# sibozhang/Text2Video

Hardware: AMD Instinct MI355X
Metric: frames/sec 512x512 pose->RGB (vid2vid generator) (higher is better)
Workload: dtype f32; 1 GPU; configs[1]: fadg0 openpose_only 512x512, 282-frame synthetic pose seq per GPU, generator-only inference, ngf128 n_down3 n_blocks9, flow branch + flow-warp compositor ON; frames_per_gpu=282, parallelism=sequence-chunk dp1, collectives=none (single process), world_size=1

## Files before the change

include/t2v.h:

```cpp
#ifndef T2V_H_
#define T2V_H_

#include <stddef.h>
#include <stdint.h>

#ifdef __cplusplus
extern "C" {
#endif

#define T2V_ABI_VERSION 18

typedef enum {
    T2V_OK = 0,
    T2V_ERR_INVALID = -1,
    T2V_ERR_HIP = -2,
    T2V_ERR_WORKSPACE = -3,
    T2V_ERR_HANDOVER = -4
} t2v_status;

enum { T2V_PAD_ZERO = 0, T2V_PAD_REFLECT = 1 };
enum { T2V_ACT_NONE = 0, T2V_ACT_TANH = 1, T2V_ACT_FLOW_W = 2 ,
       T2V_ACT_LRELU = 3  };

enum { T2V_ALGO_DIRECT = 0, T2V_ALGO_WINOGRAD = 1, T2V_ALGO_WINOGRAD_F4 = 2, T2V_ALGO_POLYPHASE = 3 };

typedef struct t2v_ctx t2v_ctx;

int t2v_abi_version(void);
const char* t2v_last_error(void);
int t2v_create(t2v_ctx** out, int device);
int t2v_destroy(t2v_ctx* ctx);
void t2v_reload_env(void);
int t2v_check_async_errors(void);
int t2v_fixed_grid_enabled(void);
int t2v_set_overlap_hint(int on);
void t2v_debug_async_error(int raise);

typedef struct {
    int H, W;
    int Cin, Cout;
    int kH, kW;
    int stride;
    int pad;
    int pad_mode;
    int transposed;
    int act;
    float act_scale;
    int output_padding;
    int algo;
} t2v_conv_desc;

int t2v_conv_out_dims(const t2v_conv_desc* d, int* Hout, int* Wout);
size_t t2v_conv_packed_weight_floats(const t2v_conv_desc* d, int x_cs);
int t2v_conv_pack_weight(t2v_ctx* ctx, void* stream, const t2v_conv_desc* d, int x_cs,
                         const float* w_torch_dev, float* packed_dev);
int t2v_conv_pack_weight_adjoint(t2v_ctx* ctx, void* stream, const t2v_conv_desc* d, int x_cs,
                                 const float* w_forward_torch_dev, float* packed_dev);
size_t t2v_conv_stats_floats(const t2v_conv_desc* d);
int t2v_conv2d_forward(t2v_ctx* ctx, void* stream, const t2v_conv_desc* d, const float* x, int x_cs,
                       const float* w_packed, const float* bias, float* y, int y_cs,
                       float* stats_partial);
int t2v_conv2d_forward_batch(t2v_ctx* ctx, void* stream, const t2v_conv_desc* d, int batch, const float* x, int x_cs,
                             const float* w_packed, const float* bias, float* y, int y_cs, float* stats_partial);

int t2v_conv_winograd_supported(const t2v_conv_desc* d, int x_cs);
int t2v_conv_polyphase_supported(const t2v_conv_desc* d, int x_cs);
int t2v_conv_best_algo(const t2v_conv_desc* d, int x_cs, int cap);
size_t t2v_conv_winograd_workspace_floats(const t2v_conv_desc* d, int x_cs);
size_t t2v_conv_winograd_batch_workspace_floats(const t2v_conv_desc* d, int x_cs, int nimg);
int t2v_conv_winograd_tile_rows(const t2v_conv_desc* d);
enum { T2V_GEMM_TILE_PER_BLOCK_64x64 = 0, T2V_GEMM_TILE_PER_BLOCK_128x128 = 1, T2V_GEMM_FIXED_GRID_128x128 = 2,
       T2V_GEMM_FIXED_GRID_192x64 = 3, T2V_GEMM_FIXED_GRID_160x128 = 4, T2V_GEMM_FIXED_GRID_RAGGED = 5,
       T2V_GEMM_FIXED_GRID_256x128 = 6 ,
       T2V_GEMM_FIXED_GRID_RAGGED_TALL = 7  };
int t2v_conv_winograd_gemm_form(const t2v_conv_desc* d, int nimg);
int t2v_conv2d_forward_winograd(t2v_ctx* ctx, void* stream, const t2v_conv_desc* d, const float* x, int x_cs,
                                const float* w_packed, const float* bias, float* y, int y_cs, float* stats_partial,
                                float* workspace);
int t2v_conv2d_forward_winograd_stages(t2v_ctx* ctx, void* stream, const t2v_conv_desc* d, const float* x, int x_cs,
                                       const float* w_packed, const float* bias, float* y, int y_cs,
                                       float* stats_partial, float* workspace, int stages);
int t2v_conv2d_forward_winograd_batch_stages(t2v_ctx* ctx, void* stream, const t2v_conv_desc* d, int nimg, const float* x,
                                             int x_cs, long img_stride, const float* w_packed, const float* bias, float* y,
                                             int y_cs, float* stats_partial, float* workspace, int stages,
                                             const float* mean_rstd, const float* gamma, const float* beta, int relu,
                                             const float* res, float* xout);

int t2v_instance_norm_finalize(t2v_ctx* ctx, void* stream, const t2v_conv_desc* producer,
                               const float* stats_partial, float eps, float* mean_rstd);
int t2v_batch_norm_finalize(t2v_ctx* ctx, void* stream, const t2v_conv_desc* producer, int batch,
                            const float* stats_partial, float eps, float* mean_rstd);
int t2v_batch_norm_update_running(t2v_ctx* ctx, void* stream, const float* mean_rstd, float* running_mean,
                                  float* running_var, long n, int C, float momentum, float eps);
int t2v_batch_norm_finalize_running(t2v_ctx* ctx, void* stream, const t2v_conv_desc* producer, int batch,
                                    const float* stats_partial, float eps, float* mean_rstd, float* running_mean,
                                    float* running_var, float momentum, int times);
int t2v_instance_norm_apply(t2v_ctx* ctx, void* stream, const float* x, const float* mean_rstd,
                            const float* gamma, const float* beta, const float* res1,
                            const float* res2, float* y, long npix, int C, int relu);

int t2v_flow_warp_composite(t2v_ctx* ctx, void* stream, const float* raw, const float* fw,
                            const float* prev, int prev_cs, int prev_c0, float* out, float* warp_out,
                            int H, int W);
int t2v_flow_warp_composite_backward(t2v_ctx* ctx, void* stream, const float* d_out, const float* d_warp,
                                     const float* raw, const float* fw, const float* prev, int prev_cs,
                                     int prev_c0, float* d_raw, float* d_fw, float* d_prev, int H, int W);

int t2v_avgpool3x3s2(t2v_ctx* ctx, void* stream, const float* x, float* y, int H, int W, int C);

size_t t2v_conv_backward_weight_workspace_floats(const t2v_conv_desc* d, int x_cs, int batch);
int t2v_conv2d_backward_weight(t2v_ctx* ctx, void* stream, const t2v_conv_desc* d, int batch, const float* x,
                               int x_cs, const float* dy, int dy_cs, float* dw_packed, int accumulate,
                               float* workspace );
int t2v_conv_backward_weight_strided_supported(const t2v_conv_desc* d, int x_cs, int dy_cs);
int t2v_conv2d_backward_weight_strided(t2v_ctx* ctx, void* stream, const t2v_conv_desc* d, int batch, const float* x,
                                       int x_cs, long x_img_stride, const float* dy, int dy_cs, long dy_img_stride,
                                       float* dw_packed, int accumulate, float* workspace);
int t2v_conv_backward_weight_winograd_supported(const t2v_conv_desc* d, int x_cs, int dy_cs);
size_t t2v_conv_backward_weight_winograd_workspace_floats(const t2v_conv_desc* d, int x_cs, int batch);
int t2v_conv2d_backward_weight_winograd(t2v_ctx* ctx, void* stream, const t2v_conv_desc* d, int batch, const float* x,
                                        int x_cs, const float* dy, int dy_cs, float* dw_torch, int accumulate,
                                        float* workspace);
int t2v_conv2d_backward_weight_winograd_stages(t2v_ctx* ctx, void* stream, const t2v_conv_desc* d, int batch, int b0,
                                               int nb, const float* x, int x_cs, const float* dy, int dy_cs,
                                               float* dw_torch, int accumulate, float* workspace, int stages);
int t2v_conv2d_backward_weight_winograd_dy_norm(t2v_ctx* ctx, void* stream, const t2v_conv_desc* d, int batch, int slot,
                                                int x_cs, const float* conv_out, const float* dy, const float* mean_rstd,
                                                const float* gamma, const float* beta, int relu, const float* sums,
                                                float* workspace);
int t2v_conv2d_forward_winograd_keep_v(t2v_ctx* ctx, void* stream, const t2v_conv_desc* d, const float* x, int x_cs,
                                       const float* w_packed, const float* bias, float* y, int y_cs, float* stats_partial,
                                       float* workspace, float* wgrad_workspace, int batch, int slot);

int t2v_conv_backward_data_winograd_supported(const t2v_conv_desc* d, int x_cs, int dy_cs);
size_t t2v_conv_backward_data_winograd_weight_floats(const t2v_conv_desc* d, int x_cs);
size_t t2v_conv_backward_data_winograd_scratch_floats(const t2v_conv_desc* d, int x_cs);
int t2v_conv_pack_weight_transposed(t2v_ctx* ctx, void* stream, const t2v_conv_desc* d, int x_cs, const float* w_forward_dev,
                                    float* packed_dev);
int t2v_conv2d_backward_data_winograd(t2v_ctx* ctx, void* stream, const t2v_conv_desc* d, int batch, int slot,
                                      const float* wgrad_workspace, int x_cs, const float* ut_packed, float* scratch, float* dx);
int t2v_conv_backward_data_winograd_takes_forward_weights(const t2v_conv_desc* d, int x_cs, int dy_cs);
int t2v_conv2d_backward_data_winograd_fw(t2v_ctx* ctx, void* stream, const t2v_conv_desc* d, int batch, int slot,
                                         const float* wgrad_workspace, int x_cs, const float* u_forward_packed, float* scratch,
                                         float* dx);

int t2v_conv_unpack_weight(t2v_ctx* ctx, void* stream, const t2v_conv_desc* d, int x_cs, const float* packed_dev,
                           float* w_torch_dev);
int t2v_conv_unpack_weight_into(t2v_ctx* ctx, void* stream, const t2v_conv_desc* d, int x_cs, const float* packed_dev,
                                float* w_torch_dev, int accumulate);
int t2v_accumulate(t2v_ctx* ctx, void* stream, float* dst, const float* src, long n, int overwrite);
int t2v_scale(t2v_ctx* ctx, void* stream, float* x, long n, float s);
int t2v_zero(t2v_ctx* ctx, void* stream, void* ptr, size_t bytes);
int t2v_unzip2(t2v_ctx* ctx, void* stream, const float* src, float* dst0, float* dst1, int C, int overwrite);
int t2v_channel_sum(t2v_ctx* ctx, void* stream, const float* x, long npix, int C, int cs,
                    float* scratch , float* out);
int t2v_reflect_pad_backward(t2v_ctx* ctx, void* stream, const float* dxp, float* dx, int H, int W, int C, int pad);
int t2v_instance_norm_backward(t2v_ctx* ctx, void* stream, const float* x, const float* dy, const float* mean_rstd,
                               const float* gamma, const float* beta, int relu, long npix, int C, float* scratch,
                               float* dx, float* dbeta_dgamma);
int t2v_instance_norm_backward_affine(t2v_ctx* ctx, void* stream, const float* x, const float* dy, const float* mean_rstd,
                                      const float* gamma, const float* beta, int relu, long npix, int C, float* scratch,
                                      float* dx, float* dbeta_dgamma, float* d_beta, float* d_gamma, int overwrite);
int t2v_act_backward(t2v_ctx* ctx, void* stream, const float* dy, const float* y, int act, float slope, long n,
                     float* dpre);
int t2v_avgpool3x3s2_backward(t2v_ctx* ctx, void* stream, const float* dy, float* dx, int H, int W, int C);
int t2v_maxpool2x2(t2v_ctx* ctx, void* stream, const float* x, float* y, int H, int W, int C);
int t2v_maxpool2x2_backward(t2v_ctx* ctx, void* stream, const float* x, const float* dy, float* dx, int H, int W, int C);
int t2v_sum_sq_diff_const_backward(t2v_ctx* ctx, void* stream, const float* x, float c, float scale, long n, float* dx);
int t2v_sum_abs_diff_backward(t2v_ctx* ctx, void* stream, const float* a, const float* b, float scale, long n, float* da);

int t2v_sum_sq_diff_const(t2v_ctx* ctx, void* stream, const float* x, float c, long n, float* scratch, float* out);
int t2v_sum_abs_diff(t2v_ctx* ctx, void* stream, const float* a, const float* b, long n, float* scratch, float* out);
int t2v_sum_abs_diff_masked(t2v_ctx* ctx, void* stream, const float* a, const float* b, const float* mask, long npix,
                            int c0, int C, int cs, float* scratch, float* out);
int t2v_sum_abs_diff_masked_backward(t2v_ctx* ctx, void* stream, const float* a, const float* b, const float* mask,
                                     float scale, long npix, int c0, int C, int cs, float* da);
int t2v_loss_terms(t2v_ctx* ctx, void* stream, const int64_t* term_ptrs, const int32_t* term_ints, const float* term_floats,
                   const int32_t* chunk_term, const int64_t* chunk_off, const int32_t* term_chunk0, int nterms, int nchunks,
                   int chunk, float* partials, float* out);
int t2v_adam_step(t2v_ctx* ctx, void* stream, float* param, const float* grad, float* exp_avg, float* exp_avg_sq,
                  long n, double lr, double beta1, double beta2, double eps, int step);

int t2v_adam_step_multi(t2v_ctx* ctx, void* stream, const int64_t* ptrs, const int64_t* nelem, const float* step_size,
                        const int32_t* chunk_tensor, const int64_t* chunk_off, int nchunks, int chunk, double beta1,
                        double beta2, double eps);

int t2v_nchw_to_nhwc(t2v_ctx* ctx, void* stream, const float* src, float* dst, int C, int H, int W, int dst_cs);
int t2v_nhwc_to_nchw(t2v_ctx* ctx, void* stream, const float* src, float* dst, int C, int H, int W, int src_cs);
int t2v_pose_u8_to_f32(t2v_ctx* ctx, void* stream, const uint8_t* src_hwc3, float* dst, long npix, int dst_cs, int c0);
int t2v_tensor2im_u8(t2v_ctx* ctx, void* stream, const float* x, uint8_t* y, long n);
int t2v_copy_channels(t2v_ctx* ctx, void* stream, const float* src, int src_cs, int src_c0, float* dst,
                      int dst_cs, int dst_c0, int nc, long npix);

typedef struct {
    int H, W;
    int input_nc;
    int prev_nc;
    int output_nc;
    int ngf;
    int n_downsample;
    int n_blocks;
    int no_flow;
    int norm_affine;
    int is_local;
    float flow_multiplier;
    float eps;
    int conv_algo;
} t2v_gen_desc;

typedef struct {
    const float* w;
    const float* bias;
    const float* gamma;
    const float* beta;
} t2v_layer;

// ... 44 lines not shown
```

text2video_amd/_lib.py:

```python
import ctypes
import os
from ctypes import POINTER, Structure, c_char_p, c_double, c_float, c_int, c_long, c_size_t, c_void_p

_HERE = os.path.dirname(os.path.abspath(__file__))
LIB_PATH = os.environ.get("T2V_LIBRARY") or os.path.join(_HERE, "lib", "libt2v_hip.so")

T2V_OK = 0
PAD_ZERO, PAD_REFLECT = 0, 1
ACT_NONE, ACT_TANH, ACT_FLOW_W, ACT_LRELU = 0, 1, 2, 3
ABI_VERSION = 18
MAX_BATCH = 8
ALGO_DIRECT, ALGO_WINOGRAD, ALGO_WINOGRAD_F4, ALGO_POLYPHASE = 0, 1, 2, 3


class ConvDesc(Structure):
    _fields_ = [("H", c_int), ("W", c_int), ("Cin", c_int), ("Cout", c_int), ("kH", c_int), ("kW", c_int),
                ("stride", c_int), ("pad", c_int), ("pad_mode", c_int), ("transposed", c_int), ("act", c_int),
                ("act_scale", c_float), ("output_padding", c_int), ("algo", c_int)]


class GenDesc(Structure):
    _fields_ = [("H", c_int), ("W", c_int), ("input_nc", c_int), ("prev_nc", c_int), ("output_nc", c_int),
                ("ngf", c_int), ("n_downsample", c_int), ("n_blocks", c_int), ("no_flow", c_int),
                ("norm_affine", c_int), ("is_local", c_int), ("flow_multiplier", c_float), ("eps", c_float),
                ("conv_algo", c_int)]


class Layer(Structure):
    _fields_ = [("w", c_void_p), ("bias", c_void_p), ("gamma", c_void_p), ("beta", c_void_p)]


class GenIO(Structure):
    _fields_ = [("pose", c_void_p), ("prev", c_void_p), ("coarse_img_feat", c_void_p),
                ("coarse_flow_feat", c_void_p), ("use_raw_only", c_int), ("out", c_void_p), ("raw", c_void_p),
                ("flow_w", c_void_p), ("img_feat", c_void_p), ("flow_feat", c_void_p)]


SIGNATURES = {
    "t2v_abi_version": (c_int, []),
    "t2v_last_error": (c_char_p, []),
    "t2v_create": (c_int, [POINTER(c_void_p), c_int]),
    "t2v_destroy": (c_int, [c_void_p]),
    "t2v_reload_env": (None, []),
    "t2v_set_overlap_hint": (c_int, [c_int]),
    "t2v_check_async_errors": (c_int, []),
    "t2v_fixed_grid_enabled": (c_int, []),
    "t2v_debug_async_error": (None, [c_int]),
    "t2v_conv_out_dims": (c_int, [POINTER(ConvDesc), POINTER(c_int), POINTER(c_int)]),
    "t2v_conv_packed_weight_floats": (c_size_t, [POINTER(ConvDesc), c_int]),
    "t2v_conv_pack_weight": (c_int, [c_void_p, c_void_p, POINTER(ConvDesc), c_int, c_void_p, c_void_p]),
    "t2v_conv_pack_weight_adjoint": (c_int, [c_void_p, c_void_p, POINTER(ConvDesc), c_int, c_void_p, c_void_p]),
    "t2v_conv_stats_floats": (c_size_t, [POINTER(ConvDesc)]),
    "t2v_conv2d_forward": (c_int, [c_void_p, c_void_p, POINTER(ConvDesc), c_void_p, c_int, c_void_p, c_void_p,
                                   c_void_p, c_int, c_void_p]),
    "t2v_conv2d_forward_batch": (c_int, [c_void_p, c_void_p, POINTER(ConvDesc), c_int, c_void_p, c_int, c_void_p, c_void_p,
                                         c_void_p, c_int, c_void_p]),
    "t2v_conv_winograd_supported": (c_int, [POINTER(ConvDesc), c_int]),
    "t2v_conv_polyphase_supported": (c_int, [POINTER(ConvDesc), c_int]),
    "t2v_conv_best_algo": (c_int, [POINTER(ConvDesc), c_int, c_int]),
    "t2v_conv_winograd_workspace_floats": (c_size_t, [POINTER(ConvDesc), c_int]),
    "t2v_conv_winograd_batch_workspace_floats": (c_size_t, [POINTER(ConvDesc), c_int, c_int]),
    "t2v_conv_winograd_tile_rows": (c_int, [POINTER(ConvDesc)]),
    "t2v_conv_winograd_gemm_form": (c_int, [POINTER(ConvDesc), c_int]),
    "t2v_conv2d_forward_winograd": (c_int, [c_void_p, c_void_p, POINTER(ConvDesc), c_void_p, c_int, c_void_p, c_void_p,
                                            c_void_p, c_int, c_void_p, c_void_p]),
    "t2v_conv2d_forward_winograd_stages": (c_int, [c_void_p, c_void_p, POINTER(ConvDesc), c_void_p, c_int, c_void_p,
                                                   c_void_p, c_void_p, c_int, c_void_p, c_void_p, c_int]),
    "t2v_conv2d_backward_weight_winograd_dy_norm": (c_int, [c_void_p, c_void_p, POINTER(ConvDesc), c_int, c_int, c_int, c_void_p,
                                                            c_void_p, c_void_p, c_void_p, c_void_p, c_int, c_void_p, c_void_p]),
    "t2v_conv2d_forward_winograd_batch_stages": (c_int, [c_void_p, c_void_p, POINTER(ConvDesc), c_int, c_void_p, c_int, c_long,
                                                         c_void_p, c_void_p, c_void_p, c_int, c_void_p, c_void_p, c_int,
                                                         c_void_p, c_void_p, c_void_p, c_int, c_void_p, c_void_p]),
    "t2v_conv2d_forward_winograd_keep_v": (c_int, [c_void_p, c_void_p, POINTER(ConvDesc), c_void_p, c_int, c_void_p,
                                                   c_void_p, c_void_p, c_int, c_void_p, c_void_p, c_void_p, c_int, c_int]),
    "t2v_instance_norm_finalize": (c_int, [c_void_p, c_void_p, POINTER(ConvDesc), c_void_p, c_float, c_void_p]),
    "t2v_batch_norm_finalize": (c_int, [c_void_p, c_void_p, POINTER(ConvDesc), c_int, c_void_p, c_float, c_void_p]),
    "t2v_batch_norm_finalize_running": (c_int, [c_void_p, c_void_p, POINTER(ConvDesc), c_int, c_void_p, c_float, c_void_p,
                                                c_void_p, c_void_p, c_float, c_int]),
    "t2v_conv_backward_weight_workspace_floats": (c_size_t, [POINTER(ConvDesc), c_int, c_int]),
    "t2v_conv_backward_weight_winograd_supported": (c_int, [POINTER(ConvDesc), c_int, c_int]),
    "t2v_conv_backward_weight_winograd_workspace_floats": (c_size_t, [POINTER(ConvDesc), c_int, c_int]),
    "t2v_conv2d_backward_weight_winograd": (c_int, [c_void_p, c_void_p, POINTER(ConvDesc), c_int, c_void_p, c_int,
                                                    c_void_p, c_int, c_void_p, c_int, c_void_p]),
    "t2v_conv2d_backward_weight_winograd_stages": (c_int, [c_void_p, c_void_p, POINTER(ConvDesc), c_int, c_int, c_int,
                                                           c_void_p, c_int, c_void_p, c_int, c_void_p, c_int, c_void_p,
                                                           c_int]),
    "t2v_conv2d_backward_weight": (c_int, [c_void_p, c_void_p, POINTER(ConvDesc), c_int, c_void_p, c_int, c_void_p,
                                           c_int, c_void_p, c_int, c_void_p]),
    "t2v_conv_backward_weight_strided_supported": (c_int, [POINTER(ConvDesc), c_int, c_int]),
    "t2v_conv2d_backward_weight_strided": (c_int, [c_void_p, c_void_p, POINTER(ConvDesc), c_int, c_void_p, c_int, c_long, c_void_p,
                                                   c_int, c_long, c_void_p, c_int, c_void_p]),
    "t2v_conv_unpack_weight": (c_int, [c_void_p, c_void_p, POINTER(ConvDesc), c_int, c_void_p, c_void_p]),
    "t2v_conv_backward_data_winograd_supported": (c_int, [POINTER(ConvDesc), c_int, c_int]),
    "t2v_conv_backward_data_winograd_weight_floats": (c_size_t, [POINTER(ConvDesc), c_int]),
    "t2v_conv_backward_data_winograd_scratch_floats": (c_size_t, [POINTER(ConvDesc), c_int]),
    "t2v_conv_pack_weight_transposed": (c_int, [c_void_p, c_void_p, POINTER(ConvDesc), c_int, c_void_p, c_void_p]),
    "t2v_conv2d_backward_data_winograd": (c_int, [c_void_p, c_void_p, POINTER(ConvDesc), c_int, c_int, c_void_p, c_int, c_void_p,
                                                  c_void_p, c_void_p]),
    "t2v_conv_backward_data_winograd_takes_forward_weights": (c_int, [POINTER(ConvDesc), c_int, c_int]),
    "t2v_conv2d_backward_data_winograd_fw": (c_int, [c_void_p, c_void_p, POINTER(ConvDesc), c_int, c_int, c_void_p, c_int, c_void_p,
                                                     c_void_p, c_void_p]),
    "t2v_conv_unpack_weight_into": (c_int, [c_void_p, c_void_p, POINTER(ConvDesc), c_int, c_void_p, c_void_p, c_int]),
    "t2v_accumulate": (c_int, [c_void_p, c_void_p, c_void_p, c_void_p, c_long, c_int]),
    "t2v_scale": (c_int, [c_void_p, c_void_p, c_void_p, c_long, c_float]),
    "t2v_zero": (c_int, [c_void_p, c_void_p, c_void_p, c_size_t]),
    "t2v_unzip2": (c_int, [c_void_p, c_void_p, c_void_p, c_void_p, c_void_p, c_int, c_int]),
    "t2v_channel_sum": (c_int, [c_void_p, c_void_p, c_void_p, c_long, c_int, c_int, c_void_p, c_void_p]),
    "t2v_reflect_pad_backward": (c_int, [c_void_p, c_void_p, c_void_p, c_void_p, c_int, c_int, c_int, c_int]),
    "t2v_instance_norm_backward": (c_int, [c_void_p, c_void_p, c_void_p, c_void_p, c_void_p, c_void_p, c_void_p, c_int,
                                           c_long, c_int, c_void_p, c_void_p, c_void_p]),
    "t2v_instance_norm_backward_affine": (c_int, [c_void_p, c_void_p, c_void_p, c_void_p, c_void_p, c_void_p, c_void_p, c_int,
                                           c_long, c_int, c_void_p, c_void_p, c_void_p, c_void_p, c_void_p, c_int]),
    "t2v_act_backward": (c_int, [c_void_p, c_void_p, c_void_p, c_void_p, c_int, c_float, c_long, c_void_p]),
    "t2v_avgpool3x3s2_backward": (c_int, [c_void_p, c_void_p, c_void_p, c_void_p, c_int, c_int, c_int]),
    "t2v_sum_sq_diff_const_backward": (c_int, [c_void_p, c_void_p, c_void_p, c_float, c_float, c_long, c_void_p]),
    "t2v_sum_abs_diff_backward": (c_int, [c_void_p, c_void_p, c_void_p, c_void_p, c_float, c_long, c_void_p]),
    "t2v_sum_sq_diff_const": (c_int, [c_void_p, c_void_p, c_void_p, c_float, c_long, c_void_p, c_void_p]),
    "t2v_sum_abs_diff": (c_int, [c_void_p, c_void_p, c_void_p, c_void_p, c_long, c_void_p, c_void_p]),
    "t2v_sum_abs_diff_masked": (c_int, [c_void_p, c_void_p, c_void_p, c_void_p, c_void_p, c_long, c_int, c_int, c_int,
                                        c_void_p, c_void_p]),
    "t2v_sum_abs_diff_masked_backward": (c_int, [c_void_p, c_void_p, c_void_p, c_void_p, c_void_p, c_float, c_long, c_int,
                                                 c_int, c_int, c_void_p]),
    "t2v_loss_terms": (c_int, [c_void_p, c_void_p, c_void_p, c_void_p, c_void_p, c_void_p, c_void_p, c_void_p, c_int, c_int,
                               c_int, c_void_p, c_void_p]),
    "t2v_adam_step": (c_int, [c_void_p, c_void_p, c_void_p, c_void_p, c_void_p, c_void_p, c_long, c_double, c_double,
                              c_double, c_double, c_int]),
    "t2v_adam_step_multi": (c_int, [c_void_p, c_void_p, c_void_p, c_void_p, c_void_p, c_void_p, c_void_p, c_int, c_int,
                                    c_double, c_double, c_double]),
    "t2v_batch_norm_update_running": (c_int, [c_void_p, c_void_p, c_void_p, c_void_p, c_void_p, c_long, c_int, c_float,
                                              c_float]),
    "t2v_instance_norm_apply": (c_int, [c_void_p, c_void_p, c_void_p, c_void_p, c_void_p, c_void_p, c_void_p,
                                        c_void_p, c_void_p, c_long, c_int, c_int]),
    "t2v_flow_warp_composite": (c_int, [c_void_p, c_void_p, c_void_p, c_void_p, c_void_p, c_int, c_int, c_void_p,
                                        c_void_p, c_int, c_int]),
    "t2v_flow_warp_composite_backward": (c_int, [c_void_p, c_void_p, c_void_p, c_void_p, c_void_p, c_void_p, c_void_p,
                                                 c_int, c_int, c_void_p, c_void_p, c_void_p, c_int, c_int]),
    "t2v_avgpool3x3s2": (c_int, [c_void_p, c_void_p, c_void_p, c_void_p, c_int, c_int, c_int]),
    "t2v_maxpool2x2": (c_int, [c_void_p, c_void_p, c_void_p, c_void_p, c_int, c_int, c_int]),
    "t2v_maxpool2x2_backward": (c_int, [c_void_p, c_void_p, c_void_p, c_void_p, c_void_p, c_int, c_int, c_int]),
    "t2v_nchw_to_nhwc": (c_int, [c_void_p, c_void_p, c_void_p, c_void_p, c_int, c_int, c_int, c_int]),
    "t2v_nhwc_to_nchw": (c_int, [c_void_p, c_void_p, c_void_p, c_void_p, c_int, c_int, c_int, c_int]),
    "t2v_pose_u8_to_f32": (c_int, [c_void_p, c_void_p, c_void_p, c_void_p, c_long, c_int, c_int]),
    "t2v_tensor2im_u8": (c_int, [c_void_p, c_void_p, c_void_p, c_void_p, c_long]),
    "t2v_copy_channels": (c_int, [c_void_p, c_void_p, c_void_p, c_int, c_int, c_void_p, c_int, c_int, c_int,
                                  c_long]),
    "t2v_generator_num_layers": (c_int, [POINTER(GenDesc)]),
    "t2v_generator_layer_desc": (c_int, [POINTER(GenDesc), c_int, POINTER(ConvDesc), POINTER(c_int)]),
    "t2v_generator_workspace_bytes": (c_size_t, [POINTER(GenDesc)]),
    "t2v_generator_forward": (c_int, [c_void_p, c_void_p, POINTER(GenDesc), POINTER(Layer), c_int, POINTER(GenIO),
                                      c_void_p, c_size_t]),
    "t2v_generator_workspace_bytes_batch": (c_size_t, [POINTER(GenDesc), c_int]),
    "t2v_generator_forward_batch": (c_int, [c_void_p, c_void_p, POINTER(GenDesc), POINTER(Layer), c_int, POINTER(GenIO),
                                            c_int, c_void_p, c_size_t]),
    "t2v_device_malloc": (c_int, [c_void_p, c_size_t, POINTER(c_void_p)]),
    "t2v_device_free": (c_int, [c_void_p, c_void_p]),
    "t2v_host_malloc": (c_int, [c_void_p, c_size_t, POINTER(c_void_p)]),
    "t2v_host_free": (c_int, [c_void_p, c_void_p]),
    "t2v_memcpy": (c_int, [c_void_p, c_void_p, c_void_p, c_void_p, c_size_t, c_int]),
    "t2v_stream_create": (c_int, [c_void_p, POINTER(c_void_p)]),
    "t2v_stream_destroy": (c_int, [c_void_p, c_void_p]),
    "t2v_stream_synchronize": (c_int, [c_void_p, c_void_p]),
    "t2v_event_create": (c_int, [c_void_p, POINTER(c_void_p)]),
    "t2v_event_record": (c_int, [c_void_p, c_void_p, c_void_p]),
    "t2v_event_synchronize": (c_int, [c_void_p, c_void_p]),
    "t2v_event_destroy": (c_int, [c_void_p, c_void_p]),
    "t2v_device_synchronize": (c_int, [c_void_p]),
}
COPY_H2D, COPY_D2H, COPY_D2D = 1, 2, 3

_lib = None
_load_lock = __import__("threading").RLock()


def load():
    if _lib is not None:
        return _lib
    with _load_lock:
        return _load_locked()


def _load_locked():
    global _lib
    if _lib is not None:
        return _lib
    if not os.path.exists(LIB_PATH):
        raise RuntimeError(
            "libt2v_hip.so not found at %s: the HIP extension is required (no CPU fallback). "
            "Build it with `python __graft_entry__.py` or `make -C text2video_amd/csrc`." % LIB_PATH)
    from ._xp import LEAN
    if not LEAN:
        import torch
        hip_rt = os.path.join(os.path.dirname(torch.__file__), "lib", "libamdhip64.so")
        if os.path.exists(hip_rt):
            ctypes.CDLL(hip_rt, mode=ctypes.RTLD_GLOBAL)
    elif os.environ.get("T2V_HIP_RUNTIME", "torch") != "system":
        import importlib.util
        spec = importlib.util.find_spec("torch")
        hip_rt = os.path.join(os.path.dirname(spec.origin), "lib", "libamdhip64.so") if spec and spec.origin else ""
        if os.path.exists(hip_rt):
            ctypes.CDLL(hip_rt, mode=ctypes.RTLD_GLOBAL)
    lib = ctypes.CDLL(LIB_PATH)
    for name, (res, args) in SIGNATURES.items():
        fn = getattr(lib, name)
        fn.restype = res
        fn.argtypes = args
    if lib.t2v_abi_version() != ABI_VERSION:
        raise RuntimeError("libt2v_hip.so ABI %d != binding ABI %d" % (lib.t2v_abi_version(), ABI_VERSION))
    _lib = lib
    return lib
# ... 31 lines not shown
```

text2video_amd/csrc/capi.hip:

```cpp
#include <stdarg.h>
#include <stdio.h>
#include <stdlib.h>
#include <string.h>

#include <algorithm>
#include <atomic>
#include <mutex>
#include <utility>
#include <vector>

#include "conv_plan.h"

namespace t2v {

static thread_local char g_err[512] = "";
void set_error(const char* fmt, ...) {
    va_list ap;
    va_start(ap, fmt);
    vsnprintf(g_err, sizeof(g_err), fmt, ap);
    va_end(ap);
}

static inline int round_up(int v, int m) { return (v + m - 1) / m * m; }

// ... 170 lines not shown
        k.ostride = 2;
        k.pad_mode = T2V_PAD_ZERO;
        k.nphases = 4;
        k.KW = 3;
        k.pad = 0;
        int tap0 = 0;
        long woff = 0;
        for (int p = 0; p < 4; ++p) {
            int nt, kh[4], kw[4], dy[4], dx[4], a, b;
            convT_phase_taps_host(p, d->kH, d->pad, &nt, kh, kw, dy, dx, &a, &b);
            ConvPhase& ph = k.ph[p];
            ph.ntaps = nt;
            ph.tap0 = tap0;
            ph.Kp = round_up(nt * x_cs, kBK);
            ph.nk = ph.Kp / kBK;
            ph.w_off = woff;
            ph.oy0 = a;
            ph.ox0 = b;
            for (int t = 0; t < nt; ++t) {
                k.tdy[tap0 + t] = dy[t];
                k.tdx[tap0 + t] = dx[t];
            }
            tap0 += nt;
            woff += (long)pl.Cout_p * ph.Kp;
        }
        pl.wfloats = (size_t)woff;
    }
    k.group_mtiles = 1 << 30;
    k.group_w_stride = 0;
    k.Wm = Wm;
    k.M = Hm * Wm;
    k.Wout = pl.Wout;
    k.Hout = pl.Hout;
    k.mtiles = (k.M + pl.BM - 1) / pl.BM;
    if (pl.tile == kTileL) {
        const long nb = (long)k.mtiles * k.ntiles * k.nphases;
        const double fill = (double)nb / (double)(((nb + 255) / 256) * 256);
        const long nbq = 4 * nb;
        const double fillq = (double)nbq / (double)(((nbq + 255) / 256) * 256);
        const int force = options().conv_tile;
        if (force == 2 || (force != 1 && ((fill < 0.8 && nb < 1024) || (k.nphases > 1 && nb <= 512) || (fillq - fill >= 0.1 && nb < 2048)))) {
            pl.tile = kTileQ;
            conv_tile_dims(pl.tile, &pl.BM, &pl.BN);
            k.ntiles = (d->Cout + pl.BN - 1) / pl.BN;
            k.mtiles = (k.M + pl.BM - 1) / pl.BM;
        }
    }
    if (need_stats && !d->transposed && d->kH == 7 && d->kW == 7 && d->stride == 1 && d->pad == 3 &&
        d->pad_mode == T2V_PAD_REFLECT && d->act == T2V_ACT_NONE && conv_stem7x7_supported(d->H, d->W, x_cs, d->Cout)) {
        pl.tile = kTileStem;
        pl.BM = 256;
        pl.BN = d->Cout;
        k.mtiles = ((d->H + 15) / 16) * ((d->W + 15) / 16);
        k.ntiles = 1;
    }
    pl.nparts = k.nphases * k.mtiles;
    T2V_REQUIRE((long)k.mtiles * k.ntiles * k.nphases < (1L << 31), "conv: grid too large");
    T2V_REQUIRE((long)d->H * d->W * x_cs * 4 < 0x7fff0000L, "conv: input tensor too large for 32-bit buffer offsets");
    for (int ph = 0; ph < k.nphases; ++ph)
        T2V_REQUIRE((long)pl.Cout_p * k.ph[ph].Kp * 4 < 0x7fff0000L, "conv: weight too large for 32-bit buffer offsets");
    return T2V_OK;
}

bool winograd_supported(const t2v_conv_desc* d, int x_cs, int algo) {
    if (!d || !is_winograd(algo)) return false;
    if (d->transposed || d->kH != 3 || d->kW != 3 || d->stride != 1) return false;
    if (d->pad_mode == T2V_PAD_REFLECT ? d->pad != 1 : (d->pad < 0 || d->pad > 2)) return false;
    if (wino_out_h(d) < 1 || wino_out_w(d) < 1) return false;
    if (d->Cin % 32 != 0 || x_cs != d->Cin || d->Cout % 4 != 0 || d->H < 2 || d->W < 2) return false;
    return d->act == T2V_ACT_NONE || (algo == T2V_ALGO_WINOGRAD_F4 && d->act == T2V_ACT_LRELU);
}

int best_conv_algo(const t2v_conv_desc* d, int x_cs, int cap) {
    const bool f4 = cap == 0 && winograd_supported(d, x_cs, T2V_ALGO_WINOGRAD_F4);
    const bool f2 = (cap == 0 || cap == 2) && winograd_supported(d, x_cs, T2V_ALGO_WINOGRAD);
    const long direct_rows = 9L * wino_out_h(d) * wino_out_w(d);
    if (f4 && (!f2 || wino_gemm_rows(d, T2V_ALGO_WINOGRAD_F4) <= wino_gemm_rows(d, T2V_ALGO_WINOGRAD)) &&
        wino_gemm_rows(d, T2V_ALGO_WINOGRAD_F4) < direct_rows)
        return T2V_ALGO_WINOGRAD_F4;
    if (f2 && wino_gemm_rows(d, T2V_ALGO_WINOGRAD) < direct_rows) return T2V_ALGO_WINOGRAD;
    return T2V_ALGO_DIRECT;
}

struct PositionGemm {
    int groups = 0;
    int rows = 0;
    int T = 0, K = 0, N = 0;
    int a_pitch = 0;
    bool has_scratch = true;
    bool b_kn = false;
};

static int build_position_gemm_plan(const PositionGemm& g, ConvPlan* pl) {
    t2v_conv_desc d;
    memset(&d, 0, sizeof(d));
    d.H = g.groups; d.W = g.T; d.Cin = g.K; d.Cout = g.N; d.kH = d.kW = 1; d.stride = 1; d.pad = 0;
    d.pad_mode = T2V_PAD_ZERO; d.act = T2V_ACT_NONE; d.act_scale = 1.f;
    T2V_TRY(build_conv_plan(&d, g.K,  true, pl));
    if (g.T % pl->BM != 0 && pl->tile == kTileL) {
        pl->tile = kTileQ;
        conv_tile_dims(pl->tile, &pl->BM, &pl->BN);
        pl->kp.ntiles = (d.Cout + pl->BN - 1) / pl->BN;
        pl->kp.mtiles = (pl->kp.M + pl->BM - 1) / pl->BM;
        pl->nparts = pl->kp.nphases * pl->kp.mtiles;
    }
    T2V_REQUIRE(g.T % pl->BM == 0, "position gemm: tile rows %d do not divide %d", pl->BM, g.T);
    pl->kp.group_mtiles = g.T / pl->BM;
    pl->kp.group_w_stride = (long)pl->Cout_p * g.K;
    if (g.a_pitch) {
        T2V_REQUIRE((long)g.groups * g.a_pitch * g.K * 4 < 0x7fff0000L, "position gemm: A too large for 32-bit buffer offsets");
        pl->kp.Win = g.a_pitch;
    }
    return T2V_OK;
}

static int position_gemm_form(const PositionGemm& g, ConvPlan* plan = nullptr) {
    if (g.b_kn) return T2V_GEMM_FIXED_GRID_128x128;
    if (g.has_scratch) {
        if (wino_gemm_skt_ok(g.groups, g.rows, g.T, g.K, g.N, g.N)) return T2V_GEMM_FIXED_GRID_RAGGED_TALL;
        if (wino_gemm_skr_ok(g.groups, g.rows, g.T, g.K, g.N, g.N)) return T2V_GEMM_FIXED_GRID_RAGGED;
        if (wino_gemm_sk_ok(g.groups, g.T, g.K, g.N, g.N, g.rows))
            switch (wino_gemm_sk_tall_rows(g.groups, g.rows, g.T, g.N)) {
                case 160: return T2V_GEMM_FIXED_GRID_160x128;
                case 256: return T2V_GEMM_FIXED_GRID_256x128;
                default: return g.T % 128 == 0 ? T2V_GEMM_FIXED_GRID_128x128 : T2V_GEMM_FIXED_GRID_192x64;
            }
    }
    ConvPlan local;
    ConvPlan* pl = plan ? plan : &local;
    if (build_position_gemm_plan(g, pl) != T2V_OK) return -1;
    return pl->tile == kTileL ? T2V_GEMM_TILE_PER_BLOCK_128x128 : T2V_GEMM_TILE_PER_BLOCK_64x64;
}

static int run_position_gemm(t2v_ctx* ctx, hipStream_t s, const PositionGemm& g, const float* a, const float* b, float* c,
                             float* scratch) {
    T2V_REQUIRE(a && b && c && (scratch || !g.has_scratch), "position gemm: null pointer");
    ConvPlan pl;
    const int form = position_gemm_form(g, &pl);
    if (form < 0) return T2V_ERR_INVALID;
    if (form == T2V_GEMM_TILE_PER_BLOCK_128x128 || form == T2V_GEMM_TILE_PER_BLOCK_64x64)
        return run_conv(ctx, s, pl, a, b, nullptr, c, g.N, nullptr);
    SkGemm k;
    k.a = a; k.b = b; k.c = c; k.scratch = scratch;
    k.err = async_error_word();
    k.rows = g.rows;
    k.a_group_stride = (long)(g.a_pitch ? g.a_pitch : g.T) * g.K;
    k.groups = g.groups; k.T = g.T; k.K = g.K; k.N = g.N; k.c_cs = g.N;
    k.b_kn = g.b_kn;
    if (form == T2V_GEMM_FIXED_GRID_RAGGED_TALL) return launch_wino_gemm_skt(s, k, g.rows);
    if (form == T2V_GEMM_FIXED_GRID_RAGGED) return launch_wino_gemm_skr(s, k, g.rows);
    return launch_wino_gemm_sk(s, k);
}

int run_conv_batch(t2v_ctx* ctx, hipStream_t s, const ConvPlan& pl, int batch, const float* x, long x_stride, const float* w,
                   const float* bias, float* y, int y_cs, long y_stride, float* stats, long stats_stride) {
    T2V_REQUIRE(ctx && x && w && y, "conv: null pointer");
    T2V_REQUIRE(batch >= 1 && batch <= 65535, "conv: batch %d", batch);
    T2V_REQUIRE(y_cs >= pl.kp.Cout && y_cs <= pl.Cout_p, "conv: output channel storage %d out of range [%d,%d]", y_cs,
                pl.kp.Cout, pl.Cout_p);
    T2V_REQUIRE((long)pl.Hout * pl.Wout * y_cs * 4 < 0x7fff0000L, "conv: output tensor too large for 32-bit buffer offsets");
    {
        const ConvKParams& q = pl.kp;
        if (!stats && q.nphases == 1 && q.ph[0].ntaps == 49 && q.KW == 7 && q.pad == 3 && q.stride == 1 &&
            q.pad_mode == T2V_PAD_REFLECT && q.Cout <= 3 && q.Cin_s % 16 == 0 && q.Hin >= 4 && q.Win >= 4) {
            for (int b = 0; b < batch; ++b) {
                HeadParams h;
                h.x = x + b * x_stride; h.w = w; h.bias = bias; h.y = y + b * y_stride;
                h.H = q.Hin; h.W = q.Win; h.Cin_s = q.Cin_s; h.Kp = q.ph[0].Kp; h.Cout = q.Cout; h.Cout_s = y_cs;
                h.act = q.act; h.act_scale = q.act_scale;
                T2V_TRY(launch_conv_head7x7(s, h));
            }
            return T2V_OK;
        }
    }
    {
        const ConvKParams& q = pl.kp;
        if (!stats && q.nphases == 1 && q.Cout == 1 && q.pad_mode == T2V_PAD_ZERO && q.ostride == 1 &&
            q.ph[0].ntaps == q.KW * q.KW && conv_cout1_supported(q.KW, q.Cin_s) &&
            (q.act == T2V_ACT_NONE || q.act == T2V_ACT_LRELU)) {
            for (int b = 0; b < batch; ++b) {
                Cout1Params c;
                c.x = x + b * x_stride; c.w = w; c.bias = bias; c.y = y + b * y_stride;
                c.H = q.Hin; c.W = q.Win; c.Cin_s = q.Cin_s; c.ksize = q.KW; c.stride = q.stride; c.pad = q.pad;
                c.Hout = pl.Hout; c.Wout = pl.Wout; c.Cout_s = y_cs; c.act = q.act; c.act_scale = q.act_scale;
                T2V_TRY(launch_conv_cout1(s, c));
            }
            return T2V_OK;
        }
    }
    if (pl.tile == kTileStem && stats) {
        for (int b = 0; b < batch; ++b) {
            StemParams sp;
            sp.x = x + b * x_stride; sp.w = w; sp.bias = bias; sp.y = y + b * y_stride; sp.stats = stats + b * stats_stride;
            sp.H = pl.kp.Hin; sp.W = pl.kp.Win; sp.Cin_s = pl.kp.Cin_s; sp.Kp = pl.kp.ph[0].Kp; sp.Cout = pl.kp.Cout; sp.Cout_s = y_cs;
            sp.Cin = pl.Cin;
            T2V_TRY(launch_conv_stem7x7(s, sp));
        }
        return T2V_OK;
    }
    T2V_REQUIRE(pl.tile != kTileStem, "conv: the stem plan needs a statistics buffer");
    ConvKParams k = pl.kp;
    k.x = x;
    k.w = w;
    k.bias = bias;
    k.y = y;
    k.Cout_s = y_cs;
    k.stats = stats;
    k.batch = batch;
    k.x_img_stride = batch > 1 ? x_stride : 0;
    k.y_img_stride = batch > 1 ? y_stride : 0;
    k.stats_img_stride = (batch > 1 && stats) ? stats_stride : 0;
    return launch_conv_igemm(s, k, pl.tile);
}

int run_conv(t2v_ctx* ctx, hipStream_t s, const ConvPlan& pl, const float* x, const float* w, const float* bias,
             float* y, int y_cs, float* stats) {
    return run_conv_batch(ctx, s, pl, 1, x, 0, w, bias, y, y_cs, 0, stats, 0);
}

int winograd_forward(t2v_ctx* ctx, hipStream_t s, const t2v_conv_desc* d, const float* x, const float* w_packed,
                     const float* bias, float* y, float* stats_partial, float* workspace, int stages,
                     const WinoBatch* batch) {
    const WinoBatch one;
    const WinoBatch& wb = batch ? *batch : one;
    const int nimg = wb.nimg;
    const bool f4 = d->algo == T2V_ALGO_WINOGRAD_F4;
    if (f4) T2V_TRY(check_async_errors());
    T2V_REQUIRE(nimg >= 1 && (f4 || nimg == 1), "winograd: batches are F(4x4,3x3) only");
    const size_t T = (size_t)wino_rows_batch(d, d->algo, nimg);
    const bool keep = wb.keep_v != nullptr;
    T2V_REQUIRE(!keep || (f4 && nimg == 1 && wb.keep_slot >= 0 && wb.keep_slot < wb.keep_total),
                "winograd: V is kept for the weight gradient of single F(4x4,3x3) images only");
    float* V = keep ? wb.keep_v + (size_t)wb.keep_slot * T * d->Cin : workspace;
    float* Mm = workspace + wino_pos(d->algo) * T * d->Cin;
    if (stages & 1) {
        const int reflect = d->pad_mode == T2V_PAD_REFLECT;
        if (keep) T2V_TRY(launch_winograd4_input(s, x, wb.keep_v, d->H, d->W, d->Cin, d->pad, reflect, wb.keep_total, wb.keep_slot));
        else
        T2V_TRY(f4 ? launch_winograd4_input(s, x, V, d->H, d->W, d->Cin, d->pad, reflect, nimg, 0, nimg, wb.img_stride_x)
                   : launch_winograd_input(s, x, V, d->H, d->W, d->Cin, d->pad, reflect));
    }
    if (stages & 2) {
        PositionGemm g;
        g.has_scratch = f4;
        g.groups = wino_pos(d->algo);
        g.rows = nimg * wino_tiles_real(d, d->algo);
        g.T = (int)T; g.K = d->Cin; g.N = d->Cout;
        if (keep) g.a_pitch = wb.keep_total * (int)T;
        T2V_TRY(run_position_gemm(ctx, s, g, V, w_packed, Mm, f4 ? workspace + winograd_vm_floats(d, nimg) : nullptr));
    }
    if (stages & 4) {
        T2V_REQUIRE(d->act == T2V_ACT_NONE || !stats_partial, "winograd: an activation and norm statistics do not combine");
        if (f4)
            T2V_TRY(launch_winograd4_output(s, Mm, bias, y, stats_partial, wino_out_h(d), wino_out_w(d), d->Cout,
                                            d->act == T2V_ACT_LRELU, d->act_scale, nimg));
        else
            T2V_TRY(launch_winograd_output(s, Mm, bias, y, stats_partial, wino_out_h(d), wino_out_w(d), d->Cout));
    }
    return T2V_OK;
}

bool polyphase_supported(const t2v_conv_desc* d, int x_cs) {
    if (!d || d->kH != 3 || d->kW != 3 || d->stride != 2 || d->pad != 1 || d->pad_mode != T2V_PAD_ZERO) return false;
    if (d->act != T2V_ACT_NONE || d->Cin % 32 != 0 || x_cs != d->Cin || d->Cout % 128 != 0) return false;
    if (d->transposed) return d->output_padding == 1 && d->H >= 2 && d->W >= 2;
    return d->H >= 4 && d->W >= 4 && d->H % 2 == 0 && d->W % 2 == 0;
}

bool polyphase_pays(const t2v_conv_desc* d, int x_cs) {
    return polyphase_supported(d, x_cs) && d->Cin >= 256 && d->Cout >= 256 && poly_tiles_real(d) >= 128;
}

int polyphase_forward(t2v_ctx* ctx, hipStream_t s, const t2v_conv_desc* d, const float* x, const float* w_packed,
                      const float* bias, float* y, float* stats_partial, float* workspace, int stages,
                      const LazyNorm* lazy) {
    T2V_TRY(check_async_errors());
    const int up = d->transposed ? 1 : 0;
    const int T = poly_tiles_padded(d), rows = poly_tiles_real(d);
    float* V = workspace;
    float* Mm = workspace + (size_t)81 * T * d->Cin;
    if (stages & 1) T2V_TRY(launch_polyphase_input(s, x, V, d->H, d->W, d->Cin, up, T, lazy));
    if (stages & 2) {
        PositionGemm g;
        g.groups = 81; g.rows = rows; g.T = T; g.K = d->Cin; g.N = d->Cout;
        T2V_TRY(run_position_gemm(ctx, s, g, V, w_packed, Mm, workspace + (size_t)81 * T * ((size_t)d->Cin + d->Cout)));
    }
    if (stages & 4)
        T2V_TRY(launch_polyphase_output(s, Mm, bias, y, stats_partial, poly_out_h(d), poly_out_w(d), d->Cout, up, T));
    return T2V_OK;
}

}

using namespace t2v;

extern "C" {

int t2v_abi_version(void) { return T2V_ABI_VERSION; }
const char* t2v_last_error(void) { return g_err; }

int t2v_create(t2v_ctx** out, int device) {
    T2V_REQUIRE(out, "t2v_create: null out");
    int n = 0;
    T2V_HIP_CHECK(hipGetDeviceCount(&n));
    T2V_REQUIRE(device >= 0 && device < n, "t2v_create: device %d out of range (%d visible)", device, n);
    T2V_HIP_CHECK(hipSetDevice(device));
    hipDeviceProp_t prop;
    T2V_HIP_CHECK(hipGetDeviceProperties(&prop, device));
    T2V_REQUIRE(strncmp(prop.gcnArchName, "gfx950", 6) == 0,
                "libt2v_hip is built for gfx950 (MI355X) only; device %d is %s", device, prop.gcnArchName);
    t2v_ctx* c = new t2v_ctx();
    c->device = device;
    c->side = nullptr;
    c->ev_fork = c->ev_join = nullptr;
    if (hipStreamCreateWithFlags(&c->side, hipStreamNonBlocking) != hipSuccess ||
        hipEventCreateWithFlags(&c->ev_fork, hipEventDisableTiming) != hipSuccess ||
        hipEventCreateWithFlags(&c->ev_join, hipEventDisableTiming) != hipSuccess) {
        t2v_destroy(c);
        set_error("t2v_create: cannot create the side stream / events");
        return T2V_ERR_HIP;
    }
    (void)options();
    {
        static std::once_flag once;
        int st = T2V_OK;
        std::call_once(once, [&]() {
            void* w = nullptr;
            if (hipHostMalloc(&w, 64, hipHostMallocMapped | hipHostMallocPortable) != hipSuccess) {
                fixed_grid_disable("no pinned error word");
                return;
            }
            memset(w, 0, 64);
            g_err_word = static_cast<unsigned*>(w);
            st = fixed_grid_selftest();
        });
        if (st != T2V_OK) {
            t2v_destroy(c);
            return st;
        }
    }
    *out = c;
    return T2V_OK;
}

void t2v_reload_env(void) { options_reload(); }
int t2v_set_overlap_hint(int on) { return set_overlap_hint(on); }
int t2v_check_async_errors(void) { return check_async_errors(); }
int t2v_fixed_grid_enabled(void) { return fixed_grid_enabled() ? 1 : 0; }
void t2v_debug_async_error(int raise) {
    if (!g_err_word) return;
    if (raise) {
        *reinterpret_cast<volatile unsigned*>(g_err_word) = 1u;
    } else {
        *reinterpret_cast<volatile unsigned*>(g_err_word) = 0u;
        g_fixed_grid_on.store(1);
    }
}

int t2v_destroy(t2v_ctx* ctx) {
    if (!ctx) return T2V_OK;
    if (ctx->ev_fork) (void)hipEventDestroy(ctx->ev_fork);
    if (ctx->ev_join) (void)hipEventDestroy(ctx->ev_join);
    if (ctx->side) (void)hipStreamDestroy(ctx->side);
    delete ctx;
    return T2V_OK;
}

int t2v_conv_out_dims(const t2v_conv_desc* d, int* Hout, int* Wout) {
    ConvPlan pl;
    T2V_TRY(build_conv_plan(d, round_up(d ? d->Cin : 0, 4), false, &pl));
    if (Hout) *Hout = pl.Hout;
    if (Wout) *Wout = pl.Wout;
    return T2V_OK;
}

size_t t2v_conv_packed_weight_floats(const t2v_conv_desc* d, int x_cs) {
    ConvPlan pl;
    if (build_conv_plan(d, x_cs, false, &pl) != T2V_OK) return 0;
    if (is_winograd(d->algo)) return winograd_supported(d, x_cs, d->algo) ? (size_t)wino_pos(d->algo) * pl.Cout_p * x_cs : 0;
    if (d->algo == T2V_ALGO_POLYPHASE) return polyphase_supported(d, x_cs) ? (size_t)81 * pl.Cout_p * x_cs : 0;
    return pl.wfloats;
}
int t2v_conv_polyphase_supported(const t2v_conv_desc* d, int x_cs) {
    return (polyphase_supported(d, x_cs) ? 1 : 0) | (polyphase_pays(d, x_cs) ? 2 : 0);
}

int t2v_conv_winograd_supported(const t2v_conv_desc* d, int x_cs) {
    return (winograd_supported(d, x_cs, T2V_ALGO_WINOGRAD) ? 1 : 0) | (winograd_supported(d, x_cs, T2V_ALGO_WINOGRAD_F4) ? 2 : 0);
}

int t2v_conv_best_algo(const t2v_conv_desc* d, int x_cs, int cap) { return d ? best_conv_algo(d, x_cs, cap) : T2V_ALGO_DIRECT; }

size_t t2v_conv_winograd_workspace_floats(const t2v_conv_desc* d, int x_cs) {
    if (d && d->algo == T2V_ALGO_POLYPHASE) return polyphase_supported(d, x_cs) ? polyphase_workspace_floats(d) : 0;
    if (!d || !winograd_supported(d, x_cs, d->algo)) return 0;
    return winograd_workspace_floats(d);
}

size_t t2v_conv_winograd_batch_workspace_floats(const t2v_conv_desc* d, int x_cs, int nimg) {
    if (!d || nimg < 1) return 0;
    if (d->algo == T2V_ALGO_POLYPHASE) return nimg == 1 && polyphase_supported(d, x_cs) ? polyphase_workspace_floats(d) : 0;
    if (!winograd_supported(d, x_cs, d->algo) || (nimg > 1 && d->algo != T2V_ALGO_WINOGRAD_F4)) return 0;
    return winograd_workspace_floats(d, nimg);
}

int t2v_conv2d_forward_winograd_stages(t2v_ctx* ctx, void* stream, const t2v_conv_desc* d, const float* x, int x_cs,
                                       const float* w_packed, const float* bias, float* y, int y_cs,
                                       float* stats_partial, float* workspace, int stages) {
    T2V_REQUIRE(ctx && d && x && w_packed && y && workspace, "winograd forward: null pointer");
    if (d->algo == T2V_ALGO_POLYPHASE) {
        T2V_REQUIRE(polyphase_supported(d, x_cs), "polyphase forward: shape not supported (t2v_conv_polyphase_supported)");
        T2V_REQUIRE(y_cs == d->Cout, "polyphase forward: output channel storage must equal Cout");
        return polyphase_forward(ctx, (hipStream_t)stream, d, x, w_packed, bias, y, stats_partial, workspace, stages);
    }
    T2V_REQUIRE(winograd_supported(d, x_cs, d->algo),
                "winograd forward: shape/algo not supported (t2v_conv_winograd_supported)");
    T2V_REQUIRE(y_cs == d->Cout, "winograd forward: output channel storage must equal Cout");
    return winograd_forward(ctx, (hipStream_t)stream, d, x, w_packed, bias, y, stats_partial, workspace, stages);
}

int t2v_conv2d_forward_winograd_batch_stages(t2v_ctx* ctx, void* stream, const t2v_conv_desc* d, int nimg, const float* x,
                                             int x_cs, long img_stride, const float* w_packed, const float* bias, float* y,
                                             int y_cs, float* stats_partial, float* workspace, int stages,
                                             const float* mean_rstd, const float* gamma, const float* beta, int relu,
                                             const float* res, float* xout) {
    T2V_REQUIRE(ctx && d && x && w_packed && y && workspace, "winograd batch forward: null pointer");
    T2V_REQUIRE(stages >= 0 && stages <= 7, "winograd batch forward: stages mask %d", stages);
    T2V_REQUIRE(nimg >= 1 && nimg <= 65535, "winograd batch forward: nimg %d", nimg);
    T2V_REQUIRE(nimg == 1 || img_stride >= (long)d->H * d->W * x_cs, "winograd batch forward: image stride %ld below one map",
                img_stride);
    T2V_REQUIRE(mean_rstd || (!gamma && !beta && !res && !xout && relu == 0),
                "winograd batch forward: gamma, beta, relu, res and xout need mean_rstd");
    hipStream_t s = (hipStream_t)stream;
    if (d->algo == T2V_ALGO_POLYPHASE) {
        T2V_REQUIRE(polyphase_supported(d, x_cs), "polyphase forward: shape not supported (t2v_conv_polyphase_supported)");
        T2V_REQUIRE(y_cs == d->Cout, "polyphase forward: output channel storage must equal Cout");
        T2V_REQUIRE(nimg == 1 && !res && !xout, "polyphase batch forward: one image, no residual");
        const LazyNorm ln{mean_rstd, gamma, beta, relu};
        return polyphase_forward(ctx, s, d, x, w_packed, bias, y, stats_partial, workspace, stages, mean_rstd ? &ln : nullptr);
    }
    T2V_REQUIRE(winograd_supported(d, x_cs, d->algo), "winograd forward: shape/algo not supported (t2v_conv_winograd_supported)");
    T2V_REQUIRE(y_cs == d->Cout, "winograd forward: output channel storage must equal Cout");
    T2V_REQUIRE(d->algo == T2V_ALGO_WINOGRAD_F4 || (nimg == 1 && !mean_rstd),
                "winograd batch forward: batches and the lazy norm are F(4x4,3x3) only");
    if (mean_rstd && (stages & 1)) {
        T2V_REQUIRE(relu == 0 || relu == 1, "winograd batch forward: relu %d", relu);
        const LazyNorm ln{mean_rstd, gamma, beta, relu, res, xout};
        T2V_TRY(launch_winograd4_input(s, x, workspace, d->H, d->W, d->Cin, d->pad, d->pad_mode == T2V_PAD_REFLECT, nimg, 0, nimg,
                                       img_stride, &ln));
        stages &= ~1;
    }
    WinoBatch wb;
    wb.nimg = nimg;
    wb.img_stride_x = img_stride;
    return winograd_forward(ctx, s, d, x, w_packed, bias, y, stats_partial, workspace, stages, &wb);
}

static bool wgrad_winograd_ok(const t2v_conv_desc* d, int x_cs, int dy_cs);
int t2v_conv2d_forward_winograd_keep_v(t2v_ctx* ctx, void* stream, const t2v_conv_desc* d, const float* x, int x_cs,
                                       const float* w_packed, const float* bias, float* y, int y_cs, float* stats_partial,
                                       float* workspace, float* wgrad_workspace, int batch, int slot) {
    T2V_REQUIRE(ctx && d && x && w_packed && y && workspace && wgrad_workspace, "winograd forward (V kept): null pointer");
    T2V_REQUIRE(d->algo == T2V_ALGO_WINOGRAD_F4 && winograd_supported(d, x_cs, d->algo) && x_cs == d->Cin &&
                    wgrad_winograd_ok(d, x_cs, d->Cout),
                "winograd forward (V kept): F(4x4,3x3) layers with a Winograd-domain weight gradient only "
                "(t2v_conv_backward_weight_winograd_supported)");
    T2V_REQUIRE(y_cs == d->Cout, "winograd forward: output channel storage must equal Cout");
    T2V_REQUIRE(batch >= 1 && slot >= 0 && slot < batch, "winograd forward (V kept): slot %d of %d", slot, batch);
    T2V_REQUIRE((long)36 * batch * wino_tiles_padded(d, d->algo) * x_cs * 4 < 0x7fff0000L,
                "winograd forward (V kept): batch-wide V too large for 32-bit buffer offsets");
    WinoBatch wb;
    wb.keep_v = wgrad_workspace;
    wb.keep_total = batch;
    wb.keep_slot = slot;
    return winograd_forward(ctx, (hipStream_t)stream, d, x, w_packed, bias, y, stats_partial, workspace, 7, &wb);
}

int t2v_conv2d_forward_winograd(t2v_ctx* ctx, void* stream, const t2v_conv_desc* d, const float* x, int x_cs,
                                const float* w_packed, const float* bias, float* y, int y_cs, float* stats_partial,
                                float* workspace) {
    return t2v_conv2d_forward_winograd_stages(ctx, stream, d, x, x_cs, w_packed, bias, y, y_cs, stats_partial, workspace, 7);
}

static int pack_weight(t2v_ctx* ctx, void* stream, const t2v_conv_desc* d, int x_cs, const float* w_torch_dev,
                       float* packed_dev, int adjoint) {
    T2V_REQUIRE(ctx && w_torch_dev && packed_dev, "pack_weight: null pointer");
    ConvPlan pl;
    T2V_TRY(build_conv_plan(d, x_cs, false, &pl));
    hipStream_t s = (hipStream_t)stream;
    if (d->algo == T2V_ALGO_POLYPHASE) {
        T2V_REQUIRE(polyphase_supported(d, x_cs) && !adjoint, "pack_weight: polyphase form not supported for this shape");
        return launch_polyphase_weight(s, w_torch_dev, packed_dev, d->Cout, d->Cin, pl.Cout_p, x_cs, d->transposed ? 1 : 0);
    }
    if (is_winograd(d->algo)) {
        T2V_REQUIRE(winograd_supported(d, x_cs, d->algo), "pack_weight: Winograd not supported for this shape");
        return (d->algo == T2V_ALGO_WINOGRAD_F4 ? launch_winograd4_weight : launch_winograd_weight)(
            s, w_torch_dev, packed_dev, d->Cout, d->Cin, pl.Cout_p, x_cs, adjoint);
    }
    if (!d->transposed)
        return launch_pack_conv_weight(s, w_torch_dev, packed_dev, d->Cout, d->Cin, d->kH, d->kW, x_cs, pl.kp.ph[0].Kp,
                                       pl.Cout_p, adjoint);
    T2V_REQUIRE(!adjoint, "pack_weight_adjoint: stride-1 convolutions only (a transposed conv's data gradient reuses its weight)");
    return launch_pack_convT_weight(s, w_torch_dev, packed_dev, d->Cin, d->Cout, x_cs, pl.Cout_p, d->kH, d->pad);
}
int t2v_conv_pack_weight(t2v_ctx* ctx, void* stream, const t2v_conv_desc* d, int x_cs, const float* w_torch_dev,
                         float* packed_dev) {
    return pack_weight(ctx, stream, d, x_cs, w_torch_dev, packed_dev, 0);
}
int t2v_conv_pack_weight_adjoint(t2v_ctx* ctx, void* stream, const t2v_conv_desc* d, int x_cs, const float* w_forward_dev,
                                 float* packed_dev) {
    T2V_REQUIRE(d && !d->transposed && d->stride == 1, "pack_weight_adjoint: `d` must be a stride-1 (data-gradient) conv");
    return pack_weight(ctx, stream, d, x_cs, w_forward_dev, packed_dev, 1);
}

size_t t2v_conv_stats_floats(const t2v_conv_desc* d) {
    if (d && is_winograd(d->algo))
        return (size_t)(wino_tiles_padded(d, d->algo) * wino_m(d->algo) * wino_m(d->algo) / 128) * d->Cout * 2;
    if (d && d->algo == T2V_ALGO_POLYPHASE) return (size_t)(poly_tiles_padded(d) * poly_m(d) * poly_m(d) / 128) * d->Cout * 2;
    ConvPlan pl;
    if (!d || build_conv_plan(d, round_up(d->Cin, 4), true, &pl) != T2V_OK) return 0;
    return (size_t)pl.nparts * d->Cout * 2;
}

int t2v_conv2d_forward(t2v_ctx* ctx, void* stream, const t2v_conv_desc* d, const float* x, int x_cs,
                       const float* w_packed, const float* bias, float* y, int y_cs, float* stats_partial) {
    T2V_REQUIRE(d && d->algo == T2V_ALGO_DIRECT, "conv2d_forward: use t2v_conv2d_forward_winograd for algo=WINOGRAD");
    ConvPlan pl;
    T2V_TRY(build_conv_plan(d, x_cs, stats_partial != nullptr, &pl));
    return run_conv(ctx, (hipStream_t)stream, pl, x, w_packed, bias, y, y_cs, stats_partial);
}

int t2v_conv2d_forward_batch(t2v_ctx* ctx, void* stream, const t2v_conv_desc* d, int batch, const float* x, int x_cs,
                             const float* w_packed, const float* bias, float* y, int y_cs, float* stats_partial) {
    T2V_REQUIRE(d && d->algo == T2V_ALGO_DIRECT, "conv2d_forward_batch: direct convolutions only");
    T2V_REQUIRE(batch >= 1, "conv2d_forward_batch: batch %d", batch);
    ConvPlan pl;
    T2V_TRY(build_conv_plan(d, x_cs, stats_partial != nullptr, &pl));
    return run_conv_batch(ctx, (hipStream_t)stream, pl, batch, x, (long)d->H * d->W * x_cs, w_packed, bias, y, y_cs,
                          (long)pl.Hout * pl.Wout * y_cs, stats_partial, (long)t2v_conv_stats_floats(d));
}

int t2v_instance_norm_finalize(t2v_ctx* ctx, void* stream, const t2v_conv_desc* producer, const float* stats_partial,
                               float eps, float* mean_rstd) {
    T2V_REQUIRE(ctx && stats_partial && mean_rstd, "inorm_finalize: null pointer");
    if (producer && is_winograd(producer->algo)) {
        return launch_inorm_finalize_winograd((hipStream_t)stream, stats_partial, wino_m(producer->algo),
                                              wino_out_h(producer), wino_out_w(producer), producer->Cout, eps, mean_rstd, 1);
    }
    if (producer && producer->algo == T2V_ALGO_POLYPHASE)
        return launch_inorm_finalize_winograd((hipStream_t)stream, stats_partial, poly_m(producer), poly_out_h(producer),
                                              poly_out_w(producer), producer->Cout, eps, mean_rstd, 1);
    ConvPlan pl;
    T2V_TRY(build_conv_plan(producer, round_up(producer ? producer->Cin : 0, 4), true, &pl));
    if (pl.tile == kTileStem)
        return launch_inorm_finalize_tiles((hipStream_t)stream, stats_partial, 16, producer->H, producer->W, producer->Cout, eps,
                                           mean_rstd, 1);
    return launch_inorm_finalize((hipStream_t)stream, stats_partial, pl.nparts, pl.kp.mtiles, pl.BM, pl.kp.M,
                                 producer->Cout, eps, mean_rstd);
}

static int batch_norm_finalize(hipStream_t s, const t2v_conv_desc* producer, int batch, const float* stats_partial, float eps,
                               float* mean_rstd, const RunningUpdate* ru) {
    if (producer && is_winograd(producer->algo))
        return launch_inorm_finalize_winograd(s, stats_partial, wino_m(producer->algo), wino_out_h(producer),
                                              wino_out_w(producer), producer->Cout, eps, mean_rstd, batch, nullptr, ru);
    if (producer && producer->algo == T2V_ALGO_POLYPHASE)
        return launch_inorm_finalize_winograd(s, stats_partial, poly_m(producer), poly_out_h(producer), poly_out_w(producer),
                                              producer->Cout, eps, mean_rstd, batch, nullptr, ru);
    ConvPlan pl;
    T2V_TRY(build_conv_plan(producer, round_up(producer ? producer->Cin : 0, 4), true, &pl));
    if (pl.tile == kTileStem)
        return launch_inorm_finalize_tiles(s, stats_partial, 16, producer->H, producer->W, producer->Cout, eps, mean_rstd, batch,
                                           nullptr, ru);
    return launch_inorm_finalize(s, stats_partial, batch * pl.nparts, pl.kp.mtiles, pl.BM, pl.kp.M, producer->Cout, eps,
                                 mean_rstd, nullptr, ru);
}
int t2v_batch_norm_finalize(t2v_ctx* ctx, void* stream, const t2v_conv_desc* producer, int batch,
                            const float* stats_partial, float eps, float* mean_rstd) {
    T2V_REQUIRE(ctx && stats_partial && mean_rstd && batch >= 1, "batch_norm_finalize: bad arguments");
    return batch_norm_finalize((hipStream_t)stream, producer, batch, stats_partial, eps, mean_rstd, nullptr);
}
int t2v_batch_norm_finalize_running(t2v_ctx* ctx, void* stream, const t2v_conv_desc* producer, int batch,
                                    const float* stats_partial, float eps, float* mean_rstd, float* running_mean,
                                    float* running_var, float momentum, int times) {
    T2V_REQUIRE(ctx && producer && stats_partial && mean_rstd && running_mean && running_var && batch >= 1 && times >= 1,
                "batch_norm_finalize_running: bad arguments");
    int ho = 0, wo = 0;
    T2V_TRY(t2v_conv_out_dims(producer, &ho, &wo));
    const long n = (long)batch * ho * wo;
    T2V_REQUIRE(n >= 2, "batch_norm_finalize_running: the unbiased variance needs at least two values per channel");
    const RunningUpdate ru{running_mean, running_var, (float)n, momentum, times};
    return batch_norm_finalize((hipStream_t)stream, producer, batch, stats_partial, eps, mean_rstd, &ru);
}

static bool wgrad_fold(const t2v_conv_desc* d, int x_cs) {
    return !d->transposed && x_cs < 64 && d->kH * d->kW > 1;
}

static bool wgrad_fold_n(const t2v_conv_desc* d, int x_cs, int dy_cs) {
    return !d->transposed && d->stride == 1 && dy_cs <= 16 && x_cs >= 64 && d->kH * d->kW > 1 &&
           d->kH * d->kW <= kMaxTaps;
}
static size_t wgrad_padded_floats(const t2v_conv_desc* d, int x_cs, int batch) {
    return (size_t)batch * (d->H + 2 * d->pad) * (d->W + 2 * d->pad) * x_cs;
}

static int wgrad_splits(const t2v_conv_desc* d, int x_cs, int batch, const ConvPlan& pl) {
    int ntaps = 0;
    for (int ph = 0; ph < pl.kp.nphases; ++ph) ntaps += pl.kp.ph[ph].ntaps;
    const long blocks = wgrad_fold(d, x_cs) ? (long)((d->Cout + 127) / 128) * ((ntaps * x_cs + 127) / 128)
                                            : (long)ntaps * ((d->Cout + 127) / 128) * ((x_cs + 127) / 128);
    const long nk = ((long)batch * pl.kp.M + 31) / 32;
    long smax = nk / 8;
    if (smax > 256) smax = 256;
    if (smax < 1) smax = 1;
    long s = 1, best = -1;
    const long slots = 2 * 256;
    for (long c = 1; c <= smax; ++c) {
        const long rounds = (blocks * c + slots - 1) / slots;
        const long cost = rounds * ((nk + c - 1) / c + 3) + (c > 1 ? c * (long)pl.wfloats * 12 / 15000000 : 0);
        if (best < 0 || cost < best) { best = cost; s = c; }
        if (blocks * c >= 4096) break;
    }
    return s < 1 ? 1 : (int)s;
}

static size_t wgrad_ticket_floats(const t2v_conv_desc* d, int x_cs, const ConvPlan& pl) {
    int ntaps = 0;
    for (int ph = 0; ph < pl.kp.nphases; ++ph) ntaps += pl.kp.ph[ph].ntaps;
    const size_t tiles = wgrad_fold(d, x_cs) ? (size_t)((d->Cout + 127) / 128) * ((ntaps * x_cs + 127) / 128)
                                            : (size_t)ntaps * ((d->Cout + 127) / 128) * ((x_cs + 127) / 128);
    return (tiles + 255) / 256 * 256;
}
static int wgrad_combine_max_splits() { return options().wgrad_combine_max; }
static bool wgrad_combine_on() { return options().wgrad_combine != 0; }

size_t t2v_conv_backward_weight_workspace_floats(const t2v_conv_desc* d, int x_cs, int batch) {
    ConvPlan pl;
    if (!d || build_conv_plan(d, x_cs, true, &pl) != T2V_OK) return 0;
    const int dy_cs = round_up(d->Cout, 4);
    if (wgrad_fold_n(d, x_cs, dy_cs)) {
        const long nk = ((long)batch * (d->H + 2 * d->pad) * (d->W + 2 * d->pad) + 31) / 32;
        long s = nk / 16;
        if (s > 256) s = 256;
        if (s < 1) s = 1;
        return wgrad_padded_floats(d, x_cs, batch) + (size_t)s * d->Cout * pl.kp.ph[0].Kp;
    }
    const int s = wgrad_splits(d, x_cs, batch, pl);
    return s > 1 ? (size_t)s * pl.wfloats + wgrad_ticket_floats(d, x_cs, pl) : 0;
}

static int backward_weight_impl(t2v_ctx* ctx, void* stream, const t2v_conv_desc* d, int batch, const float* x,
                                int x_cs, long x_stride, const float* dy, int dy_cs, long dy_stride, float* dw_packed,
                                int accumulate, float* workspace) {
    T2V_REQUIRE(ctx && x && dy && dw_packed && batch >= 1, "backward_weight: bad arguments");
    ConvPlan pl;
    T2V_TRY(build_conv_plan(d, x_cs, true, &pl));
    T2V_REQUIRE(dy_cs >= d->Cout && dy_cs % 4 == 0, "backward_weight: dy channel storage %d", dy_cs);
    const ConvKParams& k = pl.kp;
    WgradParams w;
    memset(&w, 0, sizeof(w));
    w.x = x; w.dy = dy; w.dw = dw_packed;
    w.batch = batch; w.Hin = d->H; w.Win = d->W; w.Cin_s = x_cs;
    w.Wm = k.Wm; w.M = k.M;
    w.Hout = pl.Hout; w.Wout = pl.Wout; w.Cout = d->Cout; w.Cout_s = dy_cs;
    w.stride = k.stride; w.ostride = k.ostride;
    w.reflect = k.pad_mode == T2V_PAD_REFLECT; w.accumulate = accumulate;
    w.ntiles = (d->Cout + 127) / 128; w.ctiles = (x_cs + 127) / 128;
    int nt = 0;
    for (int ph = 0; ph < k.nphases; ++ph)
        for (int t = 0; t < k.ph[ph].ntaps; ++t, ++nt) {
            w.tdy[nt] = k.tdy[k.ph[ph].tap0 + t]; w.tdx[nt] = k.tdx[k.ph[ph].tap0 + t];
            w.toy[nt] = k.ph[ph].oy0; w.tox[nt] = k.ph[ph].ox0;
            w.tap_woff[nt] = k.ph[ph].w_off; w.tap_Kp[nt] = k.ph[ph].Kp; w.tap_kidx[nt] = t;
        }
    w.ntaps = nt;
    w.x_img_stride = (long)d->H * d->W * x_cs;
    w.dy_img_stride = (long)pl.Hout * pl.Wout * dy_cs;
    if (x_stride || dy_stride) {
        T2V_REQUIRE(!(wgrad_fold_n(d, x_cs, dy_cs) && dy_cs == round_up(d->Cout, 4)) && !wgrad_fold(d, x_cs) && conv_wgrad_strided_ok(w),
                    "backward_weight_strided: this shape keeps its images contiguous (t2v_conv_backward_weight_strided_supported)");
        if (x_stride) w.x_img_stride = x_stride;
// ... 529 lines not shown
```

text2video_amd/csrc/conv_head.hip:

```cpp
#include <stdlib.h>

#include "t2v_internal.h"

namespace t2v {

__device__ __forceinline__ void hd_dma16(const float* base, int nbytes, char* lds_dst, int voff, int soff) {
#if defined(__HIP_DEVICE_COMPILE__)
    const __amdgpu_buffer_rsrc_t srd = __builtin_amdgcn_make_buffer_rsrc(const_cast<float*>(base), 0, nbytes, 0x00020000);
    __builtin_amdgcn_raw_ptr_buffer_load_lds(srd, (__attribute__((address_space(3))) void*)lds_dst, 16, voff, soff, 0, 0);
#endif
}

constexpr int kHdTile = 16;
constexpr int kHdHalo = kHdTile + 6;
constexpr int kHsPitch = 23;
constexpr int kHsPlane = 512 * 16;
template <int CIN>
__global__ __launch_bounds__(256) void conv_head7x7_strip_kernel(const HeadParams p) {
    extern __shared__ __attribute__((aligned(16))) char smem[];
    const int tid = threadIdx.x, lane = tid & 63;
    const int wave = __builtin_amdgcn_readfirstlane(tid >> 6);
    const int cin_s = CIN ? CIN : p.Cin_s;
    int tile;
    {
        const int nb = gridDim.x, b = blockIdx.x;
        const int xcd = b & 7, idx = b >> 3;
        const int q = nb >> 3, r = nb & 7;
        tile = (xcd < r ? xcd * (q + 1) : r * (q + 1) + (xcd - r) * q) + idx;
    }
    const int tiles_x = (p.W + kHdTile - 1) / kHdTile;
    const int x0 = (tile % tiles_x) * kHdTile, y0 = (tile / tiles_x) * kHdTile;
    int voff[8];
#pragma unroll
    for (int i = 0; i < 8; ++i) {
        const int hp = i * 64 + lane;
        const int hy = hp / kHsPitch, hx = hp - hy * kHsPitch;
        int gy = y0 - 3 + hy, gx = x0 - 3 + hx;
        gy = gy < 0 ? -gy : gy;
        gx = gx < 0 ? -gx : gx;
        gy = min(gy, 2 * p.H - 2 - gy);
        gx = min(gx, 2 * p.W - 2 - gx);
        gy = max(gy, 0);
        gx = max(gx, 0);
        voff[i] = (hy < kHdHalo && hx < kHdHalo) ? (gy * p.W + gx) * cin_s * 4 : 0x7fff0000;
    }
    const int x_bytes = p.H * p.W * cin_s * 4;
    char* plane = smem + wave * kHsPlane;
    const int lq = (lane & 31) >> 2;
    const int ty = ((lq >> 1) << 2) | (lane & 3), sx = ((lane >> 5) << 1) | ((0x96 >> lq) & 1);
    const char* sb = plane + (ty * kHsPitch + sx * 4) * 16;

    typedef float f32x2 __attribute__((ext_vector_type(2)));
    f32x2 acc[3][4];
#pragma unroll
    for (int o = 0; o < 3; ++o)
#pragma unroll
        for (int q = 0; q < 4; ++q) acc[o][q] = (f32x2){0.f, 0.f};
    const float* __restrict__ w0 = p.w;
    const float* __restrict__ w1 = p.w + p.Kp;
    const float* __restrict__ w2 = p.w + 2 * p.Kp;
    auto stage = [&](int c) {
#pragma unroll
        for (int i = 0; i < 8; ++i) hd_dma16(p.x, x_bytes, plane + i * 1024, voff[i], c * 4);
    };
    for (int c0 = wave * 4; c0 < cin_s; c0 += 16) {
        stage(c0);
        asm volatile("s_waitcnt vmcnt(0)" ::: "memory");
        typedef float f32x4 __attribute__((ext_vector_type(4)));
        typedef const __attribute__((address_space(4))) f32x4* cf4;
        f32x4 wa[3][3], wb[2][3], wc[2][3];
        float4 xv[2][10];
        const float* __restrict__ b0 = w0 + c0;
        const float* __restrict__ b1 = w1 + c0;
        const float* __restrict__ b2 = w2 + c0;
        auto load_w = [&](int kh, int kw, f32x4(&w)[3]) {
            const int kofs = (kh * 7 + kw) * cin_s;
            w[0] = *(cf4)(b0 + kofs);
            w[1] = *(cf4)(b1 + kofs);
            w[2] = *(cf4)(b2 + kofs);
        };
        auto load_x = [&](int kh, float4(&x)[10]) {
#pragma unroll
            for (int j = 0; j < 10; ++j) x[j] = *reinterpret_cast<const float4*>(sb + (kh * kHsPitch + j) * 16);
        };
        auto taps = [&](const float4(&x)[10], int kw, const f32x4(&w)[3]) {
#pragma unroll
            for (int q = 0; q < 4; ++q) {
                const f32x2 xlo = {x[q + kw].x, x[q + kw].y}, xhi = {x[q + kw].z, x[q + kw].w};
#pragma unroll
                for (int o = 0; o < 3; ++o) acc[o][q] = __builtin_elementwise_fma(xlo, (f32x2){w[o].x, w[o].y}, acc[o][q]);
#pragma unroll
                for (int o = 0; o < 3; ++o) acc[o][q] = __builtin_elementwise_fma(xhi, (f32x2){w[o].z, w[o].w}, acc[o][q]);
            }
        };
        if constexpr (CIN == 0) {
#pragma unroll 1
            for (int kh = 0; kh < 7; ++kh) {
                load_x(kh, xv[0]);
#pragma unroll
                for (int kw = 0; kw < 7; ++kw) {
                    load_w(kh, kw, wa[0]);
                    taps(xv[0], kw, wa[0]);
                }
            }
        } else {
        load_x(0, xv[0]);
#pragma unroll
        for (int t = 0; t < 3; ++t) load_w(0, t, wa[t]);
#pragma unroll
        for (int kh = 0; kh < 7; ++kh) {
            __builtin_amdgcn_sched_barrier(0);
#pragma unroll
            for (int t = 0; t < 2; ++t) load_w(kh, 3 + t, wb[t]);
            __builtin_amdgcn_sched_barrier(0);
#pragma unroll
            for (int t = 0; t < 3; ++t) taps(xv[kh & 1], t, wa[t]);
            __builtin_amdgcn_sched_barrier(0);
#pragma unroll
            for (int t = 0; t < 2; ++t) load_w(kh, 5 + t, wc[t]);
            __builtin_amdgcn_sched_barrier(0);
#pragma unroll
            for (int t = 0; t < 2; ++t) taps(xv[kh & 1], 3 + t, wb[t]);
            __builtin_amdgcn_sched_barrier(0);
            if (kh < 6) {
                load_x(kh + 1, xv[(kh + 1) & 1]);
#pragma unroll
                for (int t = 0; t < 3; ++t) load_w(kh + 1, t, wa[t]);
            }
            __builtin_amdgcn_sched_barrier(0);
#pragma unroll
            for (int t = 0; t < 2; ++t) taps(xv[kh & 1], 5 + t, wc[t]);
        }
        }
        __builtin_amdgcn_sched_barrier(0);
        asm volatile("s_waitcnt lgkmcnt(0)" ::: "memory");
    }
    float* red = reinterpret_cast<float*>(plane);
#pragma unroll
    for (int o = 0; o < 3; ++o)
#pragma unroll
        for (int q = 0; q < 4; ++q) red[(o * 4 + q) * 64 + lane] = acc[o][q].x + acc[o][q].y;
    __syncthreads();
    const int prow = tid >> 4, pcol = tid & 15;
    const int pq = pcol & 3, psx = pcol >> 2;
    const int src = ((psx >> 1) << 5) | ((((psx & 1) ? 0x7421 : 0x6530) >> (4 * (prow >> 2))) & 7) << 2 | (prow & 3);
    float v[3];
#pragma unroll
    for (int o = 0; o < 3; ++o) {
        float sum = 0.f;
#pragma unroll
        for (int w = 0; w < 4; ++w) sum += reinterpret_cast<const float*>(smem + w * kHsPlane)[(o * 4 + pq) * 64 + src];
        v[o] = sum;
    }
    const int oy = y0 + prow, ox = x0 + pcol;
    if (oy < p.H && ox < p.W) {
        float v0 = v[0] + (p.bias ? p.bias[0] : 0.f);
        float v1 = v[1] + (p.bias && p.Cout > 1 ? p.bias[1] : 0.f);
        float v2 = v[2] + (p.bias && p.Cout > 2 ? p.bias[2] : 0.f);
        if (p.act == T2V_ACT_TANH) {
            v0 = tanhf(v0); v1 = tanhf(v1); v2 = tanhf(v2);
        } else if (p.act == T2V_ACT_FLOW_W) {
            v0 *= p.act_scale; v1 *= p.act_scale; v2 = 1.f / (1.f + expf(-v2));
        } else if (p.act == T2V_ACT_LRELU) {
            v0 = v0 > 0.f ? v0 : v0 * p.act_scale; v1 = v1 > 0.f ? v1 : v1 * p.act_scale; v2 = v2 > 0.f ? v2 : v2 * p.act_scale;
        }
        if (p.Cout < 2) v1 = 0.f;
        if (p.Cout < 3) v2 = 0.f;
        float* dst = p.y + (size_t)(oy * p.W + ox) * p.Cout_s;
        if (p.Cout_s == 4) {
            *reinterpret_cast<float4*>(dst) = make_float4(v0, v1, v2, 0.f);
        } else {
            dst[0] = v0;
            if (p.Cout_s > 1) dst[1] = v1;
            if (p.Cout_s > 2) dst[2] = v2;
            for (int c = 3; c < p.Cout_s; ++c) dst[c] = 0.f;
        }
    }
}

int launch_conv_head7x7(hipStream_t s, const HeadParams& p) {
    constexpr int lds = 4 * kHsPlane;
    const dim3 grid(((p.W + kHdTile - 1) / kHdTile) * ((p.H + kHdTile - 1) / kHdTile));
    if (p.Cin_s == 128) hipLaunchKernelGGL(conv_head7x7_strip_kernel<128>, grid, dim3(256), lds, s, p);
    else if (p.Cin_s == 64) hipLaunchKernelGGL(conv_head7x7_strip_kernel<64>, grid, dim3(256), lds, s, p);
    else hipLaunchKernelGGL(conv_head7x7_strip_kernel<0>, grid, dim3(256), lds, s, p);
    T2V_HIP_CHECK(hipGetLastError());
    return T2V_OK;
}

constexpr int kC1Pix = 4;
template <int KS, int CPL>
__global__ __launch_bounds__(256) void conv_cout1_kernel(const Cout1Params p) {
    const int lane = threadIdx.x & 63;
    const int wave = blockIdx.x * 4 + (threadIdx.x >> 6);
    const int C4 = p.Cin_s >> 2;
    const float4* __restrict__ x4 = reinterpret_cast<const float4*>(p.x);
    const float4* __restrict__ w4 = reinterpret_cast<const float4*>(p.w);
    float4 wv[KS * KS][CPL];
#pragma unroll
    for (int t = 0; t < KS * KS; ++t)
#pragma unroll
        for (int h = 0; h < CPL; ++h) wv[t][h] = w4[t * C4 + h * 64 + lane];
    const float bv = p.bias ? p.bias[0] : 0.f;
    const int P = p.Hout * p.Wout;
    for (int i = 0; i < kC1Pix; ++i) {
        const int pix = wave * kC1Pix + i;
        if (pix >= P) return;
        const int oy = pix / p.Wout, ox = pix - oy * p.Wout;
        float4 acc = make_float4(0.f, 0.f, 0.f, 0.f);
#pragma unroll
        for (int kh = 0; kh < KS; ++kh)
#pragma unroll
            for (int kw = 0; kw < KS; ++kw) {
                const int iy = oy * p.stride - p.pad + kh, ix = ox * p.stride - p.pad + kw;
                const bool ok = (unsigned)iy < (unsigned)p.H && (unsigned)ix < (unsigned)p.W;
                const long base = ok ? ((long)iy * p.W + ix) * C4 : 0;
#pragma unroll
                for (int h = 0; h < CPL; ++h) {
                    float4 xv = x4[base + h * 64 + lane];
                    if (!ok) xv = make_float4(0.f, 0.f, 0.f, 0.f);
                    const float4 wq = wv[kh * KS + kw][h];
                    acc.x = fmaf(xv.x, wq.x, acc.x);
                    acc.y = fmaf(xv.y, wq.y, acc.y);
                    acc.z = fmaf(xv.z, wq.z, acc.z);
                    acc.w = fmaf(xv.w, wq.w, acc.w);
                }
            }
        float s = (acc.x + acc.y) + (acc.z + acc.w);
#pragma unroll
        for (int m = 32; m >= 1; m >>= 1) s += __shfl_xor(s, m);
        if (lane == 0) {
            float v = s + bv;
            if (p.act == T2V_ACT_LRELU) v = v > 0.f ? v : v * p.act_scale;
            float* dst = p.y + (size_t)pix * p.Cout_s;
            dst[0] = v;
            for (int c = 1; c < p.Cout_s; ++c) dst[c] = 0.f;
        }
    }
}
bool conv_cout1_supported(int ksize, int Cin_s) { return ksize == 4 && (Cin_s == 256 || Cin_s == 512); }
int launch_conv_cout1(hipStream_t s, const Cout1Params& p) {
    T2V_REQUIRE(conv_cout1_supported(p.ksize, p.Cin_s), "conv_cout1: k=%d Cin_s=%d not supported", p.ksize, p.Cin_s);
    const int P = p.Hout * p.Wout;
    const int blocks = (P + 4 * kC1Pix - 1) / (4 * kC1Pix);
    if (p.Cin_s == 512)
        hipLaunchKernelGGL((conv_cout1_kernel<4, 2>), dim3(blocks), dim3(256), 0, s, p);
    else
        hipLaunchKernelGGL((conv_cout1_kernel<4, 1>), dim3(blocks), dim3(256), 0, s, p);
    T2V_HIP_CHECK(hipGetLastError());
    return T2V_OK;
}

}
```

text2video_amd/csrc/conv_plan.h:

```cpp
#pragma once
#include "t2v_internal.h"

namespace t2v {

struct ConvPlan {
    ConvKParams kp;
    int tile;
    int BM, BN;
    int Hout, Wout;
    int Cout_p;
    int Cin;
    int nparts;
    size_t wfloats;
};

int build_conv_plan(const t2v_conv_desc* d, int x_cs, bool need_stats, ConvPlan* out);
inline bool is_winograd(int algo) { return algo == T2V_ALGO_WINOGRAD || algo == T2V_ALGO_WINOGRAD_F4; }
inline int wino_m(int algo) { return algo == T2V_ALGO_WINOGRAD_F4 ? 4 : 2; }
inline int wino_pos(int algo) { return (wino_m(algo) + 2) * (wino_m(algo) + 2); }
inline int wino_out_h(const t2v_conv_desc* d) { return d->H + 2 * d->pad - 2; }
inline int wino_out_w(const t2v_conv_desc* d) { return d->W + 2 * d->pad - 2; }
inline TileGrid wino_tile_grid(const t2v_conv_desc* d, int algo) { return tile_grid(wino_out_h(d), wino_out_w(d), wino_m(algo)); }
inline int wino_tiles_padded(const t2v_conv_desc* d, int algo) { return wino_tile_grid(d, algo).Tp; }
inline int wino_tiles_real(const t2v_conv_desc* d, int algo) { return wino_tile_grid(d, algo).T; }
inline int wino_rows_batch(const t2v_conv_desc* d, int algo, int nimg) {
    return (nimg > 1 && algo == T2V_ALGO_WINOGRAD_F4) ? wino_pad_tiles(nimg * wino_tiles_real(d, algo)) : wino_tiles_padded(d, algo);
}
inline size_t winograd_vm_floats(const t2v_conv_desc* d, int nimg = 1) {
    return (size_t)wino_pos(d->algo) * wino_rows_batch(d, d->algo, nimg) * ((size_t)d->Cin + d->Cout);
}
inline size_t winograd_workspace_floats(const t2v_conv_desc* d, int nimg = 1) {
    return winograd_vm_floats(d, nimg) + (d->algo == T2V_ALGO_WINOGRAD_F4 ? wino_gemm_sk_scratch_floats() : 0);
}
inline long wino_gemm_rows(const t2v_conv_desc* d, int algo) { return (long)wino_pos(algo) * wino_tiles_padded(d, algo); }
bool winograd_supported(const t2v_conv_desc* d, int x_cs, int algo);
bool polyphase_supported(const t2v_conv_desc* d, int x_cs);
bool polyphase_pays(const t2v_conv_desc* d, int x_cs);
inline TileGrid poly_tile_grid(const t2v_conv_desc* d) {
    return d->transposed ? tile_grid(d->H, d->W, 4) : tile_grid(d->H / 2, d->W / 2, 4);
}
inline int poly_tiles_real(const t2v_conv_desc* d) { return poly_tile_grid(d).T; }
inline int poly_tiles_padded(const t2v_conv_desc* d) { return poly_tile_grid(d).Tp; }
inline int poly_out_h(const t2v_conv_desc* d) { return d->transposed ? 2 * d->H : d->H / 2; }
inline int poly_out_w(const t2v_conv_desc* d) { return d->transposed ? 2 * d->W : d->W / 2; }
inline int poly_m(const t2v_conv_desc* d) { return d->transposed ? 8 : 4; }
inline size_t polyphase_workspace_floats(const t2v_conv_desc* d) {
    return (size_t)81 * poly_tiles_padded(d) * ((size_t)d->Cin + d->Cout) + wino_gemm_sk_scratch_floats();
}
int polyphase_forward(t2v_ctx* ctx, hipStream_t s, const t2v_conv_desc* d, const float* x, const float* w_packed,
                      const float* bias, float* y, float* stats_partial, float* workspace, int stages,
                      const LazyNorm* lazy = nullptr);
int best_conv_algo(const t2v_conv_desc* d, int x_cs, int cap);
struct WinoBatch {
    int nimg = 1;
    long img_stride_x = 0;
    float* keep_v = nullptr;
    int keep_total = 1, keep_slot = 0;
};
int winograd_forward(t2v_ctx* ctx, hipStream_t s, const t2v_conv_desc* d, const float* x, const float* w_packed,
                     const float* bias, float* y, float* stats_partial, float* workspace, int stages,
                     const WinoBatch* batch = nullptr);
int run_conv(t2v_ctx* ctx, hipStream_t s, const ConvPlan& pl, const float* x, const float* w, const float* bias,
             float* y, int y_cs, float* stats);
int run_conv_batch(t2v_ctx* ctx, hipStream_t s, const ConvPlan& pl, int batch, const float* x, long x_stride, const float* w,
                   const float* bias, float* y, int y_cs, long y_stride, float* stats, long stats_stride);

}
```

text2video_amd/csrc/elementwise.hip:

```cpp
#include <math.h>
#include <stdint.h>
#include <stdlib.h>

#include <algorithm>

#include "t2v_internal.h"
#include "norm_pool.h"
#include "transform_common.h"

namespace t2v {

static inline long gcd_l(long a, long b) {
    while (b) { const long t = a % b; a = b; b = t; }
    return a;
}
static inline int grid_for(long n, int block) {
    long g = (n + block - 1) / block;
    if (g > 2048) g = 2048;
    if (g < 1) g = 1;
    return (int)g;
}

__device__ __forceinline__ void running_update(const RunningUpdate& ru, int c, float2 mr, float eps) {
    if (ru.mean == nullptr) return;
    const float var = fmaxf(1.0f / (mr.y * mr.y) - eps, 0.f);
    const float unbiased = var * (ru.n / (ru.n - 1.0f));
    float rm = ru.mean[c], rv = ru.var[c];
    for (int t = 0; t < ru.times; ++t) {
        rm = (1.0f - ru.momentum) * rm + ru.momentum * mr.x;
        rv = (1.0f - ru.momentum) * rv + ru.momentum * unbiased;
    }
    ru.mean[c] = rm;
    ru.var[c] = rv;
}

__global__ __launch_bounds__(16 * kFinSlices) void inorm_finalize_kernel(const float2* __restrict__ stats, int nparts, int mtiles,
                                                             int BM, int M, int C, float eps,
                                                             float2* __restrict__ mean_rstd, int wm, int H, int W,
                                                             double* __restrict__ scratch, RunningUpdate ru) {
    __shared__ double sh[4][kFinSlices][17];
    const int cc = threadIdx.x & 15, sl = threadIdx.x >> 4;
    const int c = blockIdx.x * 16 + cc;
    double s0 = 0.0, s1 = 0.0, s2 = 0.0, sm2 = 0.0;
    float ref = 0.f;
    if (c < C) {
        ref = stats[c].x;
        const bool uniform = wm == 0 && M % BM == 0;
#pragma unroll 4
        for (int part = blockIdx.y * kFinSlices + sl; part < nparts; part += kFinSlices * gridDim.y) {
            const int nb = uniform ? BM : partial_pixels(part, mtiles, BM, M, wm, H, W);
            if (nb == 0) continue;
            const float2 v = stats[(size_t)part * C + c];
            const double d = (double)(v.x - ref), n = (double)nb;
            s0 += n;
            s1 += n * d;
            s2 += n * d * d;
            sm2 += (double)v.y;
        }
    }
    sh[0][sl][cc] = s0;
    sh[1][sl][cc] = s1;
    sh[2][sl][cc] = s2;
    sh[3][sl][cc] = sm2;
    __syncthreads();
    if (sl == 0 && c < C) {
        for (int s = 1; s < kFinSlices; ++s) {
            s0 += sh[0][s][cc];
            s1 += sh[1][s][cc];
            s2 += sh[2][s][cc];
            sm2 += sh[3][s][cc];
        }
        if (scratch != nullptr) {
            double* o = scratch + ((size_t)blockIdx.y * C + c) * 4;
            o[0] = s0; o[1] = s1; o[2] = s2; o[3] = sm2;
            return;
        }
        const double mean_d = s1 / s0;
        double m2 = sm2 + s2 - s1 * mean_d;
        m2 = m2 > 0.0 ? m2 : 0.0;
        const float var = (float)(m2 / s0);
        const float2 mr = make_float2(ref + (float)mean_d, 1.0f / sqrtf(var + eps));
        mean_rstd[c] = mr;
        running_update(ru, c, mr, eps);
    }
}

__global__ void inorm_finalize_merge_kernel(const float2* __restrict__ stats, const double* __restrict__ scratch, int groups,
                                            int C, float eps, float2* __restrict__ mean_rstd, RunningUpdate ru) {
    const int c = blockIdx.x * blockDim.x + threadIdx.x;
    if (c >= C) return;
    double s0 = 0.0, s1 = 0.0, s2 = 0.0, sm2 = 0.0;
    for (int g = 0; g < groups; ++g) {
        const double* o = scratch + ((size_t)g * C + c) * 4;
        s0 += o[0]; s1 += o[1]; s2 += o[2]; sm2 += o[3];
    }
    const double mean_d = s1 / s0;
    double m2 = sm2 + s2 - s1 * mean_d;
    m2 = m2 > 0.0 ? m2 : 0.0;
    const float2 mr = make_float2(stats[c].x + (float)mean_d, 1.0f / sqrtf((float)(m2 / s0) + eps));
    mean_rstd[c] = mr;
    running_update(ru, c, mr, eps);
}

static int finalize_groups(int nparts, int C, const double* scratch) {
    if (scratch == nullptr || nparts < 2048) return 1;
    int g = nparts / 512;
    const int want = 512 / ((C + 15) / 16);
    if (g > want) g = want;
    if (g > kFinalizeMaxGroups) g = kFinalizeMaxGroups;
    return g < 1 ? 1 : g;
}
static int run_finalize(hipStream_t s, const float* stats, int nparts, int mtiles, int BM, int M, int C, float eps,
                        float* mean_rstd, int wm, int H, int W, double* scratch, const RunningUpdate* ru) {
    const int groups = finalize_groups(nparts, C, scratch);
    const RunningUpdate none{nullptr, nullptr, 0.f, 0.f, 0};
    const RunningUpdate upd = ru ? *ru : none;
    hipLaunchKernelGGL(inorm_finalize_kernel, dim3((C + 15) / 16, groups), dim3(16 * kFinSlices), 0, s,
                       reinterpret_cast<const float2*>(stats), nparts, mtiles, BM, M, C, eps,
                       reinterpret_cast<float2*>(mean_rstd), wm, H, W, groups > 1 ? scratch : nullptr, groups > 1 ? none : upd);
    T2V_HIP_CHECK(hipGetLastError());
    if (groups > 1) {
        hipLaunchKernelGGL(inorm_finalize_merge_kernel, dim3((C + 255) / 256), dim3(256), 0, s,
                           reinterpret_cast<const float2*>(stats), scratch, groups, C, eps,
                           reinterpret_cast<float2*>(mean_rstd), upd);
        T2V_HIP_CHECK(hipGetLastError());
    }
    return T2V_OK;
}

int launch_inorm_finalize(hipStream_t s, const float* stats, int nparts, int mtiles, int BM, int M, int C,
                          float eps, float* mean_rstd, double* scratch, const RunningUpdate* ru) {
    return run_finalize(s, stats, nparts, mtiles, BM, M, C, eps, mean_rstd, 0, 0, 0, scratch, ru);
}
int launch_inorm_finalize_tiles(hipStream_t s, const float* stats, int edge, int H, int W, int C, float eps,
                                float* mean_rstd, int batch, double* scratch, const RunningUpdate* ru) {
    const int nparts = ((H + edge - 1) / edge) * ((W + edge - 1) / edge);
    return run_finalize(s, stats, batch * nparts, nparts, edge * edge, H * W, C, eps, mean_rstd, -edge, H, W, scratch, ru);
}

int launch_inorm_finalize_winograd(hipStream_t s, const float* stats, int wm, int H, int W, int C, float eps,
                                   float* mean_rstd, int batch, double* scratch, const RunningUpdate* ru) {
    const int T = ((H + wm - 1) / wm) * ((W + wm - 1) / wm), Tp = wino_pad_tiles(T);
    const int nparts = Tp / (128 / (wm * wm));
    return run_finalize(s, stats, batch * nparts, nparts, 0, H * W, C, eps, mean_rstd, wm, H, W, scratch, ru);
}

__global__ void bn_running_update_kernel(const float2* __restrict__ mean_rstd, float* __restrict__ running_mean,
                                         float* __restrict__ running_var, float n, float momentum, float eps, int C) {
    const int c = blockIdx.x * blockDim.x + threadIdx.x;
    if (c >= C) return;
    const float2 mr = mean_rstd[c];
    const float var = fmaxf(1.0f / (mr.y * mr.y) - eps, 0.f);
    const float unbiased = var * (n / (n - 1.0f));
    running_mean[c] = (1.0f - momentum) * running_mean[c] + momentum * mr.x;
    running_var[c] = (1.0f - momentum) * running_var[c] + momentum * unbiased;
}
int launch_bn_running_update(hipStream_t s, const float* mean_rstd, float* running_mean, float* running_var, long n,
                             float momentum, float eps, int C) {
    hipLaunchKernelGGL(bn_running_update_kernel, dim3((C + 255) / 256), dim3(256), 0, s,
                       reinterpret_cast<const float2*>(mean_rstd), running_mean, running_var, (float)n, momentum, eps, C);
    T2V_HIP_CHECK(hipGetLastError());
    return T2V_OK;
}

__global__ __launch_bounds__(256) void inorm_apply_kernel(const float4* __restrict__ x,
                                                          const float4* __restrict__ mean_rstd,
                                                          const float4* __restrict__ gamma,
                                                          const float4* __restrict__ beta,
                                                          const float4* __restrict__ res1,
                                                          const float4* __restrict__ res2, float4* __restrict__ y,
                                                          long n4, int C4, int relu) {
    {
        const long im = blockIdx.y;
        x += im * n4;
        y += im * n4;
        mean_rstd += im * 2 * C4;
        if (res1) res1 += im * n4;
        if (res2) res2 += im * n4;
    }
    const long stride = (long)gridDim.x * blockDim.x;
    for (long i = (long)blockIdx.x * blockDim.x + threadIdx.x; i < n4; i += stride) {
        const int c4 = (int)(i % C4);
        const float4 a = mean_rstd[2 * c4], b = mean_rstd[2 * c4 + 1];
        float4 v = x[i];
        v.x = norm_scale(v.x, a.x, a.y);
        v.y = norm_scale(v.y, a.z, a.w);
        v.z = norm_scale(v.z, b.x, b.y);
        v.w = norm_scale(v.w, b.z, b.w);
        if (gamma) {
            const float4 gm = gamma[c4], bt = beta[c4];
            v.x = norm_affine(v.x, gm.x, bt.x);
            v.y = norm_affine(v.y, gm.y, bt.y);
            v.z = norm_affine(v.z, gm.z, bt.z);
            v.w = norm_affine(v.w, gm.w, bt.w);
        }
        if (relu == 1) {
            v.x = norm_act(v.x, 1);
            v.y = norm_act(v.y, 1);
            v.z = norm_act(v.z, 1);
            v.w = norm_act(v.w, 1);
        } else if (relu == 2) {
            v.x = norm_act(v.x, 2);
            v.y = norm_act(v.y, 2);
            v.z = norm_act(v.z, 2);
            v.w = norm_act(v.w, 2);
        }
        if (res1) {
            const float4 r = res1[i];
            v.x += r.x; v.y += r.y; v.z += r.z; v.w += r.w;
        }
        if (res2) {
            const float4 r = res2[i];
            v.x += r.x; v.y += r.y; v.z += r.z; v.w += r.w;
        }
        y[i] = v;
    }
}

int launch_inorm_apply(hipStream_t s, const float* x, const float* mean_rstd, const float* gamma,
                       const float* beta, const float* res1, const float* res2, float* y, long npix, int C,
                       int relu, int nimg) {
    T2V_REQUIRE(C % 4 == 0, "inorm_apply: C=%d must be a multiple of 4", C);
    const long n4 = npix * (C / 4);
    hipLaunchKernelGGL(inorm_apply_kernel, dim3(grid_for(n4, 256), nimg), dim3(256), 0, s,
                       reinterpret_cast<const float4*>(x), reinterpret_cast<const float4*>(mean_rstd),
                       reinterpret_cast<const float4*>(gamma), reinterpret_cast<const float4*>(beta),
                       reinterpret_cast<const float4*>(res1), reinterpret_cast<const float4*>(res2),
                       reinterpret_cast<float4*>(y), n4, C / 4, relu);
    T2V_HIP_CHECK(hipGetLastError());
    return T2V_OK;
}

__global__ void add_kernel(const float4* __restrict__ a, const float4* __restrict__ b, float4* __restrict__ y,
                           long n4) {
    const long stride = (long)gridDim.x * blockDim.x;
    for (long i = (long)blockIdx.x * blockDim.x + threadIdx.x; i < n4; i += stride) {
        float4 u = a[i];
        const float4 v = b[i];
        u.x += v.x; u.y += v.y; u.z += v.z; u.w += v.w;
        y[i] = u;
    }
}
int launch_add(hipStream_t s, const float* a, const float* b, float* y, long n) {
    T2V_REQUIRE(n % 4 == 0, "add: n must be a multiple of 4");
    hipLaunchKernelGGL(add_kernel, dim3(grid_for(n / 4, 256)), dim3(256), 0, s,
                       reinterpret_cast<const float4*>(a), reinterpret_cast<const float4*>(b),
                       reinterpret_cast<float4*>(y), n / 4);
    T2V_HIP_CHECK(hipGetLastError());
    return T2V_OK;
}

__device__ __forceinline__ float block_sum(float v, float* sh) {
#pragma unroll
    for (int o = 32; o >= 1; o >>= 1) v += __shfl_xor(v, o);
    const int w = threadIdx.x >> 6, l = threadIdx.x & 63;
    if (l == 0) sh[w] = v;
    __syncthreads();
    float t = 0.f;
    if (threadIdx.x == 0)
        for (int i = 0; i < (int)(blockDim.x >> 6); ++i) t += sh[i];
    return t;
}
template <int OP>
__global__ __launch_bounds__(256) void reduce_partial_kernel(const float* __restrict__ a, const float* __restrict__ b,
                                                             float c, long n, float* __restrict__ part) {
    __shared__ float sh[4];
    float s = 0.f;
    const long stride = (long)gridDim.x * blockDim.x;
    for (long i = (long)blockIdx.x * blockDim.x + threadIdx.x; i < n; i += stride) {
        if (OP == 0) {
            const float d = a[i] - c;
            s += d * d;
        } else {
            s += fabsf(a[i] - b[i]);
        }
    }
    const float t = block_sum(s, sh);
    if (threadIdx.x == 0) part[blockIdx.x] = t;
}
__global__ __launch_bounds__(256) void reduce_final_kernel(const float* __restrict__ part, int np, float* out) {
    __shared__ float sh[4];
    float s = 0.f;
    for (int i = threadIdx.x; i < np; i += blockDim.x) s += part[i];
    const float t = block_sum(s, sh);
    if (threadIdx.x == 0) out[0] = t;
}
__global__ __launch_bounds__(256) void reduce_masked_l1_kernel(const float* __restrict__ a, const float* __restrict__ b,
                                                               const float* __restrict__ mask, long npix, int c0, int C,
                                                               int cs, float* __restrict__ part) {
    __shared__ float sh[4];
    float s = 0.f;
    const long n = npix * cs, stride = (long)gridDim.x * blockDim.x;
    for (long i = (long)blockIdx.x * blockDim.x + threadIdx.x; i < n; i += stride) {
        const long pix = i / cs;
        if ((unsigned)((int)(i - pix * cs) - c0) < (unsigned)C) {
            const float d = fabsf(a[i] - (b ? b[i] : 0.f));
            s += mask ? mask[pix] * d : d;
        }
    }
    const float t = block_sum(s, sh);
    if (threadIdx.x == 0) part[blockIdx.x] = t;
}
__global__ void masked_l1_backward_kernel(const float* __restrict__ a, const float* __restrict__ b,
                                          const float* __restrict__ mask, float scale, long npix, int c0, int C,
                                          int cs, float* __restrict__ da) {
    const long n = npix * cs, stride = (long)gridDim.x * blockDim.x;
    for (long i = (long)blockIdx.x * blockDim.x + threadIdx.x; i < n; i += stride) {
        const long pix = i / cs;
        float g = 0.f;
        if ((unsigned)((int)(i - pix * cs) - c0) < (unsigned)C) {
            const float d = a[i] - (b ? b[i] : 0.f);
            g = (d > 0.f ? scale : (d < 0.f ? -scale : 0.f)) * (mask ? mask[pix] : 1.f);
        }
        da[i] = g;
    }
}
int launch_masked_l1(hipStream_t s, const float* a, const float* b, const float* mask, long npix, int c0, int C, int cs,
                     float* scratch, float* out) {
    const int g = grid_for(npix * cs, 256);
    hipLaunchKernelGGL(reduce_masked_l1_kernel, dim3(g), dim3(256), 0, s, a, b, mask, npix, c0, C, cs, scratch);
    hipLaunchKernelGGL(reduce_final_kernel, dim3(1), dim3(256), 0, s, scratch, g, out);
    T2V_HIP_CHECK(hipGetLastError());
    return T2V_OK;
}
int launch_masked_l1_backward(hipStream_t s, const float* a, const float* b, const float* mask, float scale, long npix,
                              int c0, int C, int cs, float* da) {
    hipLaunchKernelGGL(masked_l1_backward_kernel, dim3(grid_for(npix * cs, 256)), dim3(256), 0, s, a, b, mask, scale,
                       npix, c0, C, cs, da);
    T2V_HIP_CHECK(hipGetLastError());
    return T2V_OK;
}
int launch_reduce(hipStream_t s, int op, const float* a, const float* b, float c, long n, float* scratch, float* out) {
    const int g = grid_for(n, 256);
    if (op == 0)
        hipLaunchKernelGGL(reduce_partial_kernel<0>, dim3(g), dim3(256), 0, s, a, b, c, n, scratch);
    else
        hipLaunchKernelGGL(reduce_partial_kernel<1>, dim3(g), dim3(256), 0, s, a, b, c, n, scratch);
    hipLaunchKernelGGL(reduce_final_kernel, dim3(1), dim3(256), 0, s, scratch, g, out);
    T2V_HIP_CHECK(hipGetLastError());
    return T2V_OK;
}

__global__ __launch_bounds__(256) void loss_terms_kernel(const long long* __restrict__ tp, const int* __restrict__ ti,
                                                         const float* __restrict__ tf, const int* __restrict__ chunk_term,
                                                         const long long* __restrict__ chunk_off, int chunk,
                                                         float* __restrict__ part) {
    __shared__ float sh[4];
    const int t = chunk_term[blockIdx.x];
    const long long off = chunk_off[blockIdx.x];
    const float* __restrict__ a = reinterpret_cast<const float*>(tp[4 * t]);
    const float* __restrict__ b = reinterpret_cast<const float*>(tp[4 * t + 1]);
    float* __restrict__ seed = reinterpret_cast<float*>(tp[4 * t + 2]);
    const long long end = min(tp[4 * t + 3], off + (long long)chunk);
    const int op = ti[2 * t], cs = ti[2 * t + 1];
    const float c = tf[3 * t], ss = tf[3 * t + 1];
    float s = 0.f;
    if (op == 0) {
        for (long long i = off + threadIdx.x; i < end; i += blockDim.x) {
            const float d = a[i * cs] - c;
            s += d * d;
            if (seed) {
                seed[i * cs] = 2.f * ss * d;
                for (int k = 1; k < cs; ++k) seed[i * cs + k] = 0.f;
            }
        }
    } else if (op == 1) {
        long long body = off;
        if ((((uintptr_t)a | (uintptr_t)b | (uintptr_t)seed) & 15) == 0) {
            const long long n4 = (end - off) >> 2;
            const float4* a4 = reinterpret_cast<const float4*>(a + off);
            const float4* b4 = reinterpret_cast<const float4*>(b + off);
            float4* s4 = seed ? reinterpret_cast<float4*>(seed + off) : nullptr;
            auto sg = [&](float d) { return d > 0.f ? ss : (d < 0.f ? -ss : 0.f); };
            for (long long i = threadIdx.x; i < n4; i += blockDim.x) {
                const float4 av = a4[i], bv = b4[i];
                const float d0 = av.x - bv.x, d1 = av.y - bv.y, d2 = av.z - bv.z, d3 = av.w - bv.w;
                s += (fabsf(d0) + fabsf(d1)) + (fabsf(d2) + fabsf(d3));
                if (s4) s4[i] = make_float4(sg(d0), sg(d1), sg(d2), sg(d3));
            }
            body = off + (n4 << 2);
        }
// ... 928 lines not shown
```

text2video_amd/csrc/generator.hip:

```cpp
#include <vector>

#include "conv_plan.h"

namespace t2v {
namespace {

inline int round_up(int v, int m) { return (v + m - 1) / m * m; }

struct Arena {
    char* base;
    size_t cap;
    size_t off = 0;
    bool overflow = false;
    float* alloc(size_t floats) {
        const size_t bytes = (floats * sizeof(float) + 255) / 256 * 256;
        float* p = reinterpret_cast<float*>(base + off);
        off += bytes;
        if (base && off > cap) overflow = true;
        return p;
    }
};

t2v_conv_desc mk_conv(int H, int W, int Cin, int Cout, int k, int stride, int pad, int pad_mode, int transposed,
                      int act = T2V_ACT_NONE, float act_scale = 1.f) {
    t2v_conv_desc d;
    d.H = H; d.W = W; d.Cin = Cin; d.Cout = Cout; d.kH = k; d.kW = k; d.stride = stride; d.pad = pad;
    d.pad_mode = pad_mode; d.transposed = transposed; d.act = act; d.act_scale = act_scale;
    d.output_padding = transposed ? 1 : 0;
    d.algo = T2V_ALGO_DIRECT;
    return d;
}

struct LayerSpec {
    t2v_conv_desc cd;
    int x_cs;
    bool has_norm;
};

void enumerate_layers(const t2v_gen_desc& g, std::vector<LayerSpec>& out) {
    const int G = g.ngf, n = g.is_local ? 1 : g.n_downsample;
    const int H = g.H, W = g.W;
    auto enc = [&](int in_nc) {
        out.push_back({mk_conv(H, W, in_nc, G, 7, 1, 3, T2V_PAD_REFLECT, 0), round_up(in_nc, 4), true});
        for (int i = 0; i < n; ++i) {
            t2v_conv_desc cd = mk_conv(H >> i, W >> i, G << i, G << (i + 1), 3, 2, 1, T2V_PAD_ZERO, 0);
            if (g.conv_algo == 0 && polyphase_pays(&cd, G << i)) cd.algo = T2V_ALGO_POLYPHASE;
            out.push_back({cd, G << i, true});
        }
    };
    auto rbs = [&](int count) {
        const int C = G << n;
        t2v_conv_desc cd = mk_conv(H >> n, W >> n, C, C, 3, 1, 1, T2V_PAD_REFLECT, 0);
        cd.algo = best_conv_algo(&cd, C, g.conv_algo);
        for (int i = 0; i < 2 * count; ++i) out.push_back({cd, C, true});
    };
    auto ups = [&]() {
        for (int i = 0; i < n; ++i) {
            const int l = n - i;
            t2v_conv_desc cd = mk_conv(H >> l, W >> l, G << l, G << (l - 1), 3, 2, 1, T2V_PAD_ZERO, 1);
            if (g.conv_algo == 0 && polyphase_pays(&cd, G << l)) cd.algo = T2V_ALGO_POLYPHASE;
            out.push_back({cd, G << l, true});
        }
    };
    const int nb_enc = g.is_local ? 0 : g.n_blocks - g.n_blocks / 2;
    const int nb_res = g.is_local ? g.n_blocks : g.n_blocks / 2;
    enc(g.input_nc); rbs(nb_enc);
    enc(g.prev_nc);  rbs(nb_enc);
    rbs(nb_res); ups();
    out.push_back({mk_conv(H, W, G, g.output_nc, 7, 1, 3, T2V_PAD_REFLECT, 0, T2V_ACT_TANH), G, false});
    if (!g.no_flow) {
        rbs(nb_res); ups();
        out.push_back({mk_conv(H, W, G, 3, 7, 1, 3, T2V_PAD_REFLECT, 0, T2V_ACT_FLOW_W, g.flow_multiplier), G, false});
    }
}

int check_desc(const t2v_gen_desc* g) {
    T2V_REQUIRE(g, "null generator descriptor");
    const int n = g->is_local ? 1 : g->n_downsample;
    T2V_REQUIRE(g->ngf > 0 && g->ngf % 4 == 0, "ngf=%d must be a positive multiple of 4", g->ngf);
    T2V_REQUIRE(n >= 1 && n <= 6, "n_downsample=%d out of range", n);
    T2V_REQUIRE(g->H > 0 && g->W > 0 && g->H % (1 << n) == 0 && g->W % (1 << n) == 0,
                "H=%d W=%d must be positive multiples of %d", g->H, g->W, 1 << n);
    T2V_REQUIRE((g->H >> n) >= 2 && (g->W >> n) >= 2, "bottleneck %dx%d too small for reflection pad 1", g->H >> n,
                g->W >> n);
    T2V_REQUIRE(g->output_nc == 3, "output_nc=%d: only RGB output is on the path", g->output_nc);
    T2V_REQUIRE(g->input_nc > 0 && g->prev_nc >= 3, "bad input_nc/prev_nc");
    T2V_REQUIRE(g->n_blocks >= 0, "bad n_blocks");
    return T2V_OK;
}

constexpr int kMaxBatch = T2V_MAX_BATCH;

struct Buffers {
    float *encA[8], *encB[8];
    float* bt[4];
    float* bt2[4];
    float* d;
    float *dimg, *dflow;
    float *decI[8], *decF[8];
    float *raw, *fw;
    size_t lvl[8];
    size_t bott;
    float* stats[2];
    float* mean_rstd[2];
    float* wino[2];
    double* fin[2];
    size_t stats_stride, mr_stride, fin_stride;
};

void plan_buffers(const t2v_gen_desc& g, const std::vector<LayerSpec>& layers, int nimg, Arena& a, Buffers& b) {
    const int G = g.ngf, n = g.is_local ? 1 : g.n_downsample;
    auto lvl = [&](int l) { return (size_t)(g.H >> l) * (g.W >> l) * (G << l); };
    const size_t N = (size_t)nimg;
    for (int l = 0; l <= n; ++l) {
        b.lvl[l] = lvl(l);
        b.encA[l] = a.alloc(N * lvl(l));
        b.encB[l] = a.alloc(N * lvl(l));
    }
    b.bott = lvl(n);
    for (int i = 0; i < 4; ++i) b.bt[i] = a.alloc(N * lvl(n));
    for (int i = 0; i < 4; ++i) b.bt2[i] = a.alloc(N * lvl(n));
    b.d = a.alloc(N * lvl(n));
    b.dimg = a.alloc(N * lvl(n));
    b.dflow = a.alloc(N * lvl(n));
    for (int l = 0; l < n; ++l) {
        b.decI[l] = a.alloc(N * lvl(l));
        b.decF[l] = g.no_flow ? nullptr : a.alloc(N * lvl(l));
    }
    b.raw = a.alloc(N * g.H * g.W * 4);
    b.fw = a.alloc(N * g.H * g.W * 4);
    size_t max_stats = 0;
    int max_c = 4;
    for (const LayerSpec& L : layers) {
        ConvPlan pl;
        if (L.has_norm && is_winograd(L.cd.algo)) {
            const int m = wino_m(L.cd.algo);
            const size_t s = (size_t)(wino_tiles_padded(&L.cd, L.cd.algo) * m * m / 128) * L.cd.Cout * 2;
            if (s > max_stats) max_stats = s;
        } else if (L.has_norm && L.cd.algo == T2V_ALGO_POLYPHASE) {
            const size_t s = (size_t)(poly_tiles_padded(&L.cd) * poly_m(&L.cd) * poly_m(&L.cd) / 128) * L.cd.Cout * 2;
            if (s > max_stats) max_stats = s;
        } else if (L.has_norm && build_conv_plan(&L.cd, L.x_cs, true, &pl) == T2V_OK) {
            const size_t s = (size_t)pl.nparts * L.cd.Cout * 2;
            if (s > max_stats) max_stats = s;
        }
        if (L.cd.Cout > max_c) max_c = L.cd.Cout;
    }
    b.stats_stride = (max_stats + 63) / 64 * 64;
    b.mr_stride = (size_t)max_c * 2;
    b.fin_stride = (size_t)kFinalizeMaxGroups * max_c * 4;
    for (int k = 0; k < 2; ++k) {
        b.stats[k] = a.alloc(N * b.stats_stride);
        b.mean_rstd[k] = a.alloc(N * b.mr_stride);
        b.fin[k] = reinterpret_cast<double*>(a.alloc(N * b.fin_stride * 2));
    }
    size_t max_wino = 0;
    for (const LayerSpec& L : layers)
        if (is_winograd(L.cd.algo)) {
            const size_t w = winograd_workspace_floats(&L.cd, L.cd.algo == T2V_ALGO_WINOGRAD_F4 ? nimg : 1);
            if (w > max_wino) max_wino = w;
        } else if (L.cd.algo == T2V_ALGO_POLYPHASE) {
            const size_t w = polyphase_workspace_floats(&L.cd);
            if (w > max_wino) max_wino = w;
        }
    for (int k = 0; k < 2; ++k) b.wino[k] = max_wino ? a.alloc(max_wino) : nullptr;
}

struct Ptrs {
    const float* p[kMaxBatch];
};
struct MutPtrs {
    float* p[kMaxBatch];
    operator Ptrs() const {
        Ptrs q;
        for (int i = 0; i < kMaxBatch; ++i) q.p[i] = p[i];
        return q;
    }
};

struct Runner {
    t2v_ctx* ctx;
    hipStream_t s;
    const t2v_gen_desc& g;
    const std::vector<LayerSpec>& specs;
    const t2v_layer* layers;
    Buffers& b;
    int nimg;
    int li = 0;
    int sc = 0;

    Ptrs at(const float* base, size_t stride) const {
        Ptrs q{};
        for (int i = 0; i < nimg; ++i) q.p[i] = base ? base + (size_t)i * stride : nullptr;
        return q;
    }
    MutPtrs at(float* base, size_t stride) const {
        MutPtrs q{};
        for (int i = 0; i < nimg; ++i) q.p[i] = base ? base + (size_t)i * stride : nullptr;
        return q;
    }
    float* stats_of(int im) const { return b.stats[sc] + (size_t)im * b.stats_stride; }
    float* mr_of(int im) const { return b.mean_rstd[sc] + (size_t)im * b.mr_stride; }
    double* fin_of(int im) const { return b.fin[sc] + (size_t)im * b.fin_stride; }
    int conv_norm_one(int l, int im, const float* x, float* y, int relu, const float* res1, const float* res2,
                      bool lazy_in = false, bool lazy_out = false) {
        const LayerSpec& L = specs[l];
        const t2v_layer& w = layers[l];
        ConvPlan pl;
        const int Cout = L.cd.Cout;
        float* stats = stats_of(im);
        float* mr = mr_of(im);
        const float* gam = g.norm_affine ? w.gamma : nullptr;
        const float* bet = g.norm_affine ? w.beta : nullptr;
        if (g.norm_affine) T2V_REQUIRE(gam && bet, "layer %d: norm_affine=1 but gamma/beta missing", l);
        if (is_winograd(L.cd.algo)) {
            const int M = L.cd.H * L.cd.W;
            const int wm = wino_m(L.cd.algo);
            WinoBatch wb;
            T2V_TRY(winograd_forward(ctx, s, &L.cd, x, w.w, w.bias, y, stats, b.wino[sc], 7, &wb));
            T2V_TRY(launch_inorm_finalize_winograd(s, stats, wm, L.cd.H, L.cd.W, Cout, g.eps, mr, 1, fin_of(im)));
            return launch_inorm_apply(s, y, mr, gam, bet, res1, res2, y, (long)M, Cout, relu);
        }
        T2V_REQUIRE(!lazy_out || (relu == 1 && !res1 && !res2), "internal: a lazy output carries a plain norm + ReLU");
        if (L.cd.algo == T2V_ALGO_POLYPHASE) {
            const int Ho = poly_out_h(&L.cd), Wo = poly_out_w(&L.cd);
            const LazyNorm ln{mr, g.norm_affine ? layers[l - 1].gamma : nullptr, g.norm_affine ? layers[l - 1].beta : nullptr, 1};
            T2V_TRY(polyphase_forward(ctx, s, &L.cd, x, w.w, w.bias, y, stats, b.wino[sc], 7, lazy_in ? &ln : nullptr));
            T2V_TRY(launch_inorm_finalize_winograd(s, stats, poly_m(&L.cd), Ho, Wo, Cout, g.eps, mr, 1, fin_of(im)));
            if (lazy_out) return T2V_OK;
            return launch_inorm_apply(s, y, mr, gam, bet, res1, res2, y, (long)Ho * Wo, Cout, relu);
        }
        T2V_REQUIRE(!lazy_in, "internal: only the polyphase input transform applies a pending norm");
        T2V_TRY(build_conv_plan(&L.cd, L.x_cs, true, &pl));
        T2V_TRY(run_conv(ctx, s, pl, x, w.w, w.bias, y, Cout, stats));
        if (pl.tile == kTileStem)
            T2V_TRY(launch_inorm_finalize_tiles(s, stats, 16, L.cd.H, L.cd.W, Cout, g.eps, mr, 1, fin_of(im)));
        else
            T2V_TRY(launch_inorm_finalize(s, stats, pl.nparts, pl.kp.mtiles, pl.BM, pl.kp.M, Cout, g.eps, mr, fin_of(im)));
        if (lazy_out) return T2V_OK;
        return launch_inorm_apply(s, y, mr, gam, bet, res1, res2, y, (long)pl.Hout * pl.Wout, Cout, relu);
    }
    int conv_norm(const Ptrs& x, const MutPtrs& y, int relu, const Ptrs& res1, bool lazy_in = false, bool lazy_out = false) {
        for (int im = 0; im < nimg; ++im)
            T2V_TRY(conv_norm_one(li, im, x.p[im], y.p[im], relu, res1.p[im], nullptr, lazy_in, lazy_out));
        ++li;
        return T2V_OK;
    }
    bool next_takes_raw() const { return options().chain_lazy && specs[li + 1].cd.algo == T2V_ALGO_POLYPHASE; }

    int head(const Ptrs& x, const MutPtrs& y) {
        const LayerSpec& L = specs[li];
        const t2v_layer& w = layers[li];
        ++li;
        ConvPlan pl;
        T2V_TRY(build_conv_plan(&L.cd, L.x_cs, false, &pl));
        for (int im = 0; im < nimg; ++im) T2V_TRY(run_conv(ctx, s, pl, x.p[im], w.w, w.bias, y.p[im], 4, nullptr));
        return T2V_OK;
    }

    int resblock(const Ptrs& x, const MutPtrs& t, const MutPtrs& y) {
        T2V_TRY(conv_norm(x, t, 1, Ptrs{}));
        return conv_norm(t, y, 0, x);
    }

    struct LazyIn {
        const t2v_layer* norm;
        int relu;
        const float* res;
        float* xout;
    };
    int wino4_conv_stats(const float* x, const LazyIn* lz, float* y_raw) {
        const LayerSpec& L = specs[li];
        const t2v_layer& w = layers[li];
        ++li;
        const t2v_conv_desc& cd = L.cd;
        if (g.norm_affine) T2V_REQUIRE(w.gamma && w.beta, "layer %d: norm_affine=1 but gamma/beta missing", li - 1);
        T2V_REQUIRE(b.mr_stride == (size_t)2 * cd.Cout, "internal: chain scratch layout");
        if (lz) {
            const LazyNorm ln{b.mean_rstd[sc], g.norm_affine ? lz->norm->gamma : nullptr, g.norm_affine ? lz->norm->beta : nullptr,
                              lz->relu, lz->res, lz->xout};
            T2V_TRY(launch_winograd4_input(s, x, b.wino[sc], cd.H, cd.W, cd.Cin, cd.pad, cd.pad_mode == T2V_PAD_REFLECT, nimg, 0,
                                           nimg, (long)b.bott, &ln));
        }
        WinoBatch wb;
        wb.nimg = nimg;
        wb.img_stride_x = (long)b.bott;
        T2V_TRY(winograd_forward(ctx, s, &cd, x, w.w, w.bias, y_raw, b.stats[sc], b.wino[sc], lz ? 6 : 7, &wb));
        const size_t per_img = (size_t)(wino_tiles_padded(&cd, cd.algo) / 8) * cd.Cout * 2;
        for (int im = 0; im < nimg; ++im)
            T2V_TRY(launch_inorm_finalize_winograd(s, b.stats[sc] + im * per_img, 4, cd.H, cd.W, cd.Cout, g.eps, mr_of(im), 1,
                                                   fin_of(im)));
        return T2V_OK;
    }

    int res_chain_lazy(const float* x, int count, float* tmp[4], const float** out) {
        const float* cur = x;
        const t2v_layer* pend = nullptr;
        for (int i = 0; i < count; ++i) {
            if (i == 0) {
                T2V_TRY(wino4_conv_stats(x, nullptr, tmp[0]));
            } else {
                float* xi = tmp[2 + (i & 1)];
                const LazyIn in{pend, 0, cur, xi};
                T2V_TRY(wino4_conv_stats(tmp[1], &in, tmp[0]));
                cur = xi;
            }
            const LazyIn mid{&layers[li - 1], 1, nullptr, nullptr};
            T2V_TRY(wino4_conv_stats(tmp[0], &mid, tmp[1]));
            pend = &layers[li - 1];
        }
        const LayerSpec& L = specs[li - 1];
        T2V_TRY(launch_inorm_apply(s, tmp[1], b.mean_rstd[sc], g.norm_affine ? pend->gamma : nullptr,
                                   g.norm_affine ? pend->beta : nullptr, cur, nullptr, tmp[1], (long)L.cd.H * L.cd.W,
                                   L.cd.Cout, 0, nimg));
        *out = tmp[1];
        return T2V_OK;
    }

    int res_chain(const float* x, int count, float* tmp[4], const float** out) {
        if (options().chain_lazy && count > 0 && specs[li].cd.algo == T2V_ALGO_WINOGRAD_F4 && b.mr_stride == (size_t)2 * specs[li].cd.Cout)
            return res_chain_lazy(x, count, tmp, out);
        const float* cur = x;
        for (int i = 0; i < count; ++i) {
            float* t = tmp[0];
            float* y = (cur == tmp[1]) ? tmp[2] : tmp[1];
            T2V_TRY(resblock(at(cur, b.bott), at(t, b.bott), at(y, b.bott)));
            cur = y;
        }
        *out = cur;
        return T2V_OK;
    }

    int encoder(const Ptrs& x, float** act, int nb, float* tmp[4], const float** out) {
        const int n = g.is_local ? 1 : g.n_downsample;
        bool raw = n > 0 && next_takes_raw();
        T2V_TRY(conv_norm(x, at(act[0], b.lvl[0]), 1, Ptrs{}, false, raw));
        for (int i = 0; i < n; ++i) {
            const bool raw_out = i + 1 < n && next_takes_raw();
            T2V_TRY(conv_norm(at(act[i], b.lvl[i]), at(act[i + 1], b.lvl[i + 1]), 1, Ptrs{}, raw, raw_out));
            raw = raw_out;
        }
        if (nb == 0) {
            *out = act[n];
            return T2V_OK;
        }
        return res_chain(act[n], nb, tmp, out);
    }

    int decoder(const float* x, float** dec, const float** out) {
        const int n = g.is_local ? 1 : g.n_downsample;
        const float* cur = x;
        size_t cur_stride = b.bott;
        bool raw = false;
        for (int i = 0; i < n; ++i) {
            const int l = n - 1 - i;
            float* y = dec[l];
            const bool raw_out = i + 1 < n && next_takes_raw();
            T2V_TRY(conv_norm(at(cur, cur_stride), at(y, b.lvl[l]), 1, Ptrs{}, raw, raw_out));
            raw = raw_out;
            cur = y;
            cur_stride = b.lvl[l];
        }
        *out = cur;
        return T2V_OK;
    }
};

}
}

using namespace t2v;

extern "C" {

int t2v_generator_num_layers(const t2v_gen_desc* d) {
    if (check_desc(d) != T2V_OK) return -1;
    std::vector<LayerSpec> L;
    enumerate_layers(*d, L);
    return (int)L.size();
}

int t2v_generator_layer_desc(const t2v_gen_desc* d, int i, t2v_conv_desc* out, int* x_cs) {
    T2V_TRY(check_desc(d));
    std::vector<LayerSpec> L;
    enumerate_layers(*d, L);
    T2V_REQUIRE(i >= 0 && i < (int)L.size() && out, "layer index %d out of range", i);
    *out = L[i].cd;
    if (x_cs) *x_cs = L[i].x_cs;
    return T2V_OK;
}

size_t t2v_generator_workspace_bytes_batch(const t2v_gen_desc* d, int batch) {
    if (check_desc(d) != T2V_OK || batch < 1 || batch > kMaxBatch) return 0;
    std::vector<LayerSpec> L;
    enumerate_layers(*d, L);
    Arena a{nullptr, 0};
    Buffers b;
    plan_buffers(*d, L, batch, a, b);
    return a.off;
}
size_t t2v_generator_workspace_bytes(const t2v_gen_desc* d) { return t2v_generator_workspace_bytes_batch(d, 1); }

int t2v_generator_forward_batch(t2v_ctx* ctx, void* stream, const t2v_gen_desc* d, const t2v_layer* layers, int n_layers,
                                const t2v_gen_io* ios, int batch, void* workspace, size_t ws_bytes) {
    T2V_REQUIRE(ctx && layers && ios && workspace, "generator_forward: null pointer");
    T2V_REQUIRE(batch >= 1 && batch <= kMaxBatch, "generator_forward: batch %d out of range [1,%d]", batch, kMaxBatch);
    T2V_TRY(check_desc(d));
    T2V_TRY(check_async_errors());
    std::vector<LayerSpec> specs;
    enumerate_layers(*d, specs);
    T2V_REQUIRE(n_layers == (int)specs.size(), "generator_forward: expected %d layers, got %d", (int)specs.size(),
                n_layers);
    T2V_REQUIRE(((uintptr_t)workspace & 255) == 0, "workspace must be 256-byte aligned");
    for (int im = 0; im < batch; ++im) {
        const t2v_gen_io* io = ios + im;
        T2V_REQUIRE(io->pose && io->prev && io->out, "generator_forward: pose/prev/out must be set (image %d)", im);
        if (d->is_local) {
            T2V_REQUIRE(io->coarse_img_feat, "local generator needs coarse_img_feat");
            T2V_REQUIRE(d->no_flow || io->coarse_flow_feat, "local generator with flow needs coarse_flow_feat");
        }
    }
    for (int i = 0; i < n_layers; ++i)
        T2V_REQUIRE(layers[i].w && layers[i].bias, "layer %d: weight/bias pointer missing", i);
    Arena a{reinterpret_cast<char*>(workspace), ws_bytes};
    Buffers b;
    plan_buffers(*d, specs, batch, a, b);
    if (a.overflow) {
        set_error("generator_forward: workspace %zu bytes < required %zu", ws_bytes, a.off);
        return T2V_ERR_WORKSPACE;
    }
    hipStream_t s = (hipStream_t)stream;
    const int bott_tiles = ((d->H >> d->n_downsample) + 3) / 4 * (((d->W >> d->n_downsample) + 3) / 4);
    const bool two_streams = options().streams == 2 || (options().streams == 0 && (d->is_local || bott_tiles < 1024));
    const OverlapScope overlap(two_streams);
    hipStream_t s2 = two_streams ? ctx->side : s;
    auto fork = [&]() -> int {
        if (!two_streams) return T2V_OK;
        T2V_HIP_CHECK(hipEventRecord(ctx->ev_fork, s));
        T2V_HIP_CHECK(hipStreamWaitEvent(s2, ctx->ev_fork, 0));
        return T2V_OK;
    };
    auto join = [&]() -> int {
        if (!two_streams) return T2V_OK;
        T2V_HIP_CHECK(hipEventRecord(ctx->ev_join, s2));
        T2V_HIP_CHECK(hipStreamWaitEvent(s, ctx->ev_join, 0));
        return T2V_OK;
    };
    const int n = d->is_local ? 1 : d->n_downsample;
    const int G = d->ngf;
    const size_t bott = b.bott;
    const int nb_enc = d->is_local ? 0 : d->n_blocks - d->n_blocks / 2;
    const int nb_res = d->is_local ? d->n_blocks : d->n_blocks / 2;
    const int enc_layers = 1 + n + 2 * nb_enc;
    const int branch_layers = 2 * nb_res + n + 1;
    Runner r{ctx, s, *d, specs, layers, b, batch};
    Runner r2{ctx, s2, *d, specs, layers, b, batch};
    r2.sc = two_streams ? 1 : 0;

    Ptrs pose{}, prevp{};
    for (int im = 0; im < batch; ++im) {
        pose.p[im] = ios[im].pose;
        prevp.p[im] = ios[im].prev;
    }
    float* tmpA[4] = {b.bt[0], b.bt[1], b.bt[2], b.bt[3]};
    float* tmpB[4] = {b.bt2[0], b.bt2[1], b.bt2[2], b.bt2[3]};
    const float *segout, *imgout;
    T2V_TRY(fork());
    r2.li = enc_layers;
    T2V_TRY(r2.encoder(prevp, b.encB, nb_enc, tmpB, &imgout));
    T2V_TRY(r.encoder(pose, b.encA, nb_enc, tmpA, &segout));
    T2V_TRY(join());
    T2V_TRY(launch_add(s, imgout, segout, b.d, (long)(batch * bott)));
    const float* dsum = b.d;
    r.li = 2 * enc_layers;

    const float* img_in = dsum;
    const float* flow_in = dsum;
    if (d->is_local) {
        for (int im = 0; im < batch; ++im) {
            T2V_TRY(launch_add(s, dsum + im * bott, ios[im].coarse_img_feat, b.dimg + im * bott, (long)bott));
            if (!d->no_flow)
                T2V_TRY(launch_add(s, dsum + im * bott, ios[im].coarse_flow_feat, b.dflow + im * bott, (long)bott));
        }
        img_in = b.dimg;
        if (!d->no_flow) flow_in = b.dflow;
    }
    const size_t px4 = (size_t)d->H * d->W * 4, feat = (size_t)d->H * d->W * G;
    MutPtrs raw{}, fw{};
    bool blend[kMaxBatch];
    for (int im = 0; im < batch; ++im) {
        blend[im] = !(d->no_flow || ios[im].use_raw_only);
        raw.p[im] = ios[im].raw ? ios[im].raw : (blend[im] ? b.raw + im * px4 : ios[im].out);
        fw.p[im] = ios[im].flow_w ? ios[im].flow_w : b.fw + im * px4;
    }
    if (!d->no_flow) {
        T2V_TRY(fork());
        r2.li = 2 * enc_layers + branch_layers;
        const float *res_flow, *flow_feat;
        T2V_TRY(r2.res_chain(flow_in, nb_res, tmpB, &res_flow));
        T2V_TRY(r2.decoder(res_flow, b.decF, &flow_feat));
        T2V_TRY(r2.head(r2.at(flow_feat, feat), fw));
        for (int im = 0; im < batch; ++im)
            if (ios[im].flow_feat)
                T2V_HIP_CHECK(hipMemcpyAsync(ios[im].flow_feat, flow_feat + im * feat, feat * sizeof(float),
                                             hipMemcpyDeviceToDevice, s2));
    }
    const float *res_img, *img_feat;
    T2V_TRY(r.res_chain(img_in, nb_res, tmpA, &res_img));
    T2V_TRY(r.decoder(res_img, b.decI, &img_feat));
    T2V_TRY(r.head(r.at(img_feat, feat), raw));
    for (int im = 0; im < batch; ++im)
        if (ios[im].img_feat)
            T2V_HIP_CHECK(hipMemcpyAsync(ios[im].img_feat, img_feat + im * feat, feat * sizeof(float), hipMemcpyDeviceToDevice,
                                         s));
    if (!d->no_flow) {
        T2V_TRY(join());
        r.li += branch_layers;
        T2V_REQUIRE(r2.li == n_layers, "internal: flow branch consumed up to layer %d of %d", r2.li, n_layers);
        const int prev_cs = round_up(d->prev_nc, 4);
        for (int im = 0; im < batch; ++im)
            if (blend[im])
                T2V_TRY(launch_warp_composite(s, raw.p[im], fw.p[im], ios[im].prev, prev_cs, d->prev_nc - 3, ios[im].out,
                                              nullptr, d->H, d->W));
    }
    for (int im = 0; im < batch; ++im)
        if (!blend[im] && raw.p[im] != ios[im].out)
            T2V_HIP_CHECK(hipMemcpyAsync(ios[im].out, raw.p[im], px4 * sizeof(float), hipMemcpyDeviceToDevice, s));
    T2V_REQUIRE(r.li == n_layers, "internal: consumed %d of %d layers", r.li, n_layers);
    return T2V_OK;
}

int t2v_generator_forward(t2v_ctx* ctx, void* stream, const t2v_gen_desc* d, const t2v_layer* layers, int n_layers,
                          const t2v_gen_io* io, void* workspace, size_t ws_bytes) {
    return t2v_generator_forward_batch(ctx, stream, d, layers, n_layers, io, 1, workspace, ws_bytes);
}

}
```

text2video_amd/csrc/polyphase.hip:

```cpp
#include "t2v_internal.h"
#include "norm_pool.h"
#include "polyphase_consts.h"
#include "transform_common.h"

namespace t2v {

static inline int pp_grid(long n, int block) { return capped_grid(n, block, 65535L * 16); }


template <bool UP>
__global__ void polyphase_weight_kernel(const float* __restrict__ w, float* __restrict__ U, int Cout, int Cin, int Cout_p,
                                        int Cin_s) {
    const long total = (long)Cout_p * Cin_s;
    const long stride = (long)gridDim.x * blockDim.x;
    for (long i = (long)blockIdx.x * blockDim.x + threadIdx.x; i < total; i += stride) {
        const int n = (int)(i / Cin_s), c = (int)(i - (long)n * Cin_s);
        double g[3][3];
#pragma unroll
        for (int a = 0; a < 3; ++a)
#pragma unroll
            for (int b = 0; b < 3; ++b) {
                const size_t at = UP ? (((size_t)c * Cout + n) * 3 + a) * 3 + b : (((size_t)n * Cin + c) * 3 + a) * 3 + b;
                g[a][b] = (n < Cout && c < Cin) ? (double)w[at] : 0.0;
            }
        double t[9][3];
#pragma unroll
        for (int p = 0; p < 9; ++p)
#pragma unroll
            for (int b = 0; b < 3; ++b) {
                const double(&G)[9][3] = UP ? pp::kGU : pp::kGD;
                t[p][b] = G[p][0] * g[0][b] + G[p][1] * g[1][b] + G[p][2] * g[2][b];
            }
#pragma unroll
        for (int p = 0; p < 9; ++p)
#pragma unroll
            for (int q = 0; q < 9; ++q) {
                const double(&G)[9][3] = UP ? pp::kGU : pp::kGD;
                const double u = t[p][0] * G[q][0] + t[p][1] * G[q][1] + t[p][2] * G[q][2];
                U[(size_t)(p * 9 + q) * Cout_p * Cin_s + (size_t)n * Cin_s + c] = (float)u;
            }
    }
}
int launch_polyphase_weight(hipStream_t s, const float* w, float* U, int Cout, int Cin, int Cout_p, int Cin_s, int up) {
    const int grid = pp_grid((long)Cout_p * Cin_s, 256);
    if (up)
        hipLaunchKernelGGL(polyphase_weight_kernel<true>, dim3(grid), dim3(256), 0, s, w, U, Cout, Cin, Cout_p, Cin_s);
    else
        hipLaunchKernelGGL(polyphase_weight_kernel<false>, dim3(grid), dim3(256), 0, s, w, U, Cout, Cin, Cout_p, Cin_s);
    T2V_HIP_CHECK(hipGetLastError());
    return T2V_OK;
}

template <bool UP, bool NORM>
__global__ __launch_bounds__(256) void polyphase_input_kernel(const float2* __restrict__ x, float2* __restrict__ V, int H, int W,
                                                             int C2, int TW, int T, int Tt,
                                                             const float2* __restrict__ mean_rstd,
                                                             const float2* __restrict__ gamma,
                                                             const float2* __restrict__ beta, int relu) {
    const long total = (long)Tt * C2;
    const long stride = (long)gridDim.x * blockDim.x;
    for (long i = (long)blockIdx.x * blockDim.x + threadIdx.x; i < total; i += stride) {
        const long tile = i / C2;
        const int c2 = (int)(i - tile * C2);
        if (tile >= T) {
#pragma unroll 1
            for (int pos = 0; pos < 81; ++pos) V[((long)pos * Tt + tile) * C2 + c2] = make_float2(0.f, 0.f);
            continue;
        }
        const int ty = (int)(tile / TW), tx = (int)(tile - (long)ty * TW);
        auto wrow = [&](int k, int t) { return UP ? 4 * t + k : 8 * t - 1 + 2 * k; };
        auto prow = [&](int k, int t) { return UP ? 4 * t + k : 8 * t + 2 * k; };
        float2 mr0 = make_float2(0.f, 1.f), mr1 = make_float2(0.f, 1.f), gm = make_float2(1.f, 1.f), bt = make_float2(0.f, 0.f);
        if (NORM) {
            mr0 = mean_rstd[2 * c2];
            mr1 = mean_rstd[2 * c2 + 1];
            if (gamma) {
                gm = gamma[c2];
                bt = beta[c2];
            }
        }
        auto load = [&](int yy, int xx) {
            if (!((unsigned)yy < (unsigned)H && (unsigned)xx < (unsigned)W)) return make_float2(0.f, 0.f);
            float2 v = x[((long)yy * W + xx) * C2 + c2];
            if (NORM) {
                v.x = norm_apply(v.x, mr0.x, mr0.y, gamma != nullptr, gm.x, bt.x, relu == 1);
                v.y = norm_apply(v.y, mr1.x, mr1.y, gamma != nullptr, gm.y, bt.y, relu == 1);
            }
            return v;
        };
        auto store = [&](int pr, int pc, float vx, float vy) { V[((long)(pr * 9 + pc) * Tt + tile) * C2 + c2] = make_float2(vx, vy); };
        {
            float rx[5][5], ry[5][5];
#pragma unroll
            for (int a = 0; a < 5; ++a) {
                float dx[5], dy[5];
#pragma unroll
                for (int b = 0; b < 5; ++b) {
                    const float2 v = load(wrow(a, ty), wrow(b, tx));
                    dx[b] = v.x;
                    dy[b] = v.y;
                }
#pragma unroll
                for (int q = 0; q < 5; ++q) {
                    rx[a][q] = cdot<5>(pp::kBU[q], dx);
                    ry[a][q] = cdot<5>(pp::kBU[q], dy);
                }
            }
#pragma unroll
            for (int q = 0; q < 5; ++q) {
                float cx[5], cy[5];
#pragma unroll
                for (int a = 0; a < 5; ++a) {
                    cx[a] = rx[a][q];
                    cy[a] = ry[a][q];
                }
#pragma unroll
                for (int p = 0; p < 5; ++p) store(p, q, cdot<5>(pp::kBU[p], cx), cdot<5>(pp::kBU[p], cy));
            }
        }
#pragma unroll
        for (int b = 0; b < 4; ++b) {
            float cx[5], cy[5];
#pragma unroll
            for (int a = 0; a < 5; ++a) {
                const float2 v = load(wrow(a, ty), prow(b, tx));
                cx[a] = v.x;
                cy[a] = v.y;
            }
#pragma unroll
            for (int p = 0; p < 5; ++p) store(p, 5 + b, cdot<5>(pp::kBU[p], cx), cdot<5>(pp::kBU[p], cy));
        }
#pragma unroll
        for (int a = 0; a < 4; ++a) {
            float dx[5], dy[5];
#pragma unroll
            for (int b = 0; b < 5; ++b) {
                const float2 v = load(prow(a, ty), wrow(b, tx));
                dx[b] = v.x;
                dy[b] = v.y;
            }
#pragma unroll
            for (int q = 0; q < 5; ++q) store(5 + a, q, cdot<5>(pp::kBU[q], dx), cdot<5>(pp::kBU[q], dy));
        }
#pragma unroll
        for (int a = 0; a < 4; ++a)
#pragma unroll
            for (int b = 0; b < 4; ++b) {
                const float2 v = load(prow(a, ty), prow(b, tx));
                store(5 + a, 5 + b, v.x, v.y);
            }
    }
}
int launch_polyphase_input(hipStream_t s, const float* x, float* V, int H, int W, int C, int up, int Tt, const LazyNorm* lazy) {
    const LazyNorm none{};
    const LazyNorm& ln = lazy ? *lazy : none;
    T2V_REQUIRE((ln.gamma == nullptr) == (ln.beta == nullptr) && (ln.relu == 0 || ln.relu == 1) && !ln.res && !ln.xout,
                "polyphase_input: bad norm arguments");
    const TileGrid tg = up ? tile_grid(H, W, 4) : tile_grid(H / 2, W / 2, 4);
    const int grid = pp_grid((long)Tt * (C / 2), 256);
    auto kern = up ? (ln.mean_rstd ? polyphase_input_kernel<true, true> : polyphase_input_kernel<true, false>)
                   : (ln.mean_rstd ? polyphase_input_kernel<false, true> : polyphase_input_kernel<false, false>);
    hipLaunchKernelGGL(kern, dim3(grid), dim3(256), 0, s, reinterpret_cast<const float2*>(x), reinterpret_cast<float2*>(V), H, W,
                       C / 2, tg.TW, tg.T, Tt, reinterpret_cast<const float2*>(ln.mean_rstd),
                       reinterpret_cast<const float2*>(ln.gamma), reinterpret_cast<const float2*>(ln.beta), ln.relu);
    T2V_HIP_CHECK(hipGetLastError());
    return T2V_OK;
}

__global__ __launch_bounds__(256) void polyphase_output_down_kernel(const float* __restrict__ Mm, const float* __restrict__ bias,
                                                                    float* __restrict__ y, float2* __restrict__ stats, int Ho,
                                                                    int Wo, int N, int TW, int T, int Tt) {
    __shared__ float sh[4][64];
    output_transform_4x4<9>(pp::kAD, Mm, bias, y, stats, Ho, Wo, N, TW, T, Tt, sh, [](float v) { return v; });
}

__global__ __launch_bounds__(256) void polyphase_output_up_kernel(const float* __restrict__ Mm, const float* __restrict__ bias,
                                                                  float* __restrict__ y, float2* __restrict__ stats, int Ho,
                                                                  int Wo, int N, int TW, int T, int Tt) {
    __shared__ float sh[4][64];
    const int cl = threadIdx.x & 63, tl = threadIdx.x >> 6;
    const int n = blockIdx.y * 64 + cl;
    const bool ok = n < N;
    const float bv = (ok && bias) ? bias[n] : 0.f;
    const long tile = (long)blockIdx.x * 2 + (tl >> 1);
    const int half = tl & 1;
    const bool tv = tile < T;
    float r[4][9];
#pragma unroll
    for (int pc = 0; pc < 9; ++pc) {
        float m[5];
#pragma unroll
        for (int pr = 0; pr < 5; ++pr) m[pr] = (ok && tv) ? Mm[((long)(pr * 9 + pc) * Tt + tile) * N + n] : 0.f;
#pragma unroll
        for (int k = 0; k < 2; ++k) {
            const int q = 2 * half + k;
            r[2 * k][pc] = (ok && tv) ? Mm[((long)((5 + q) * 9 + pc) * Tt + tile) * N + n] : 0.f;
            r[2 * k + 1][pc] = half ? (k ? cdot<5>(pp::kAD[3], m) : cdot<5>(pp::kAD[2], m)) : (k ? cdot<5>(pp::kAD[1], m) : cdot<5>(pp::kAD[0], m));
        }
    }
    const int ty = (int)(tile / TW), tx = (int)(tile - (long)ty * TW);
    float out[32];
    unsigned mask = 0;
#pragma unroll
    for (int i2 = 0; i2 < 4; ++i2)
#pragma unroll
        for (int j2 = 0; j2 < 8; ++j2) {
            const float v = cdot<9>(pp::kAU[j2], r[i2]) + bv;
            out[i2 * 8 + j2] = v;
            const int oy = 8 * ty + 4 * half + i2, ox = 8 * tx + j2;
            if (tv && oy < Ho && ox < Wo) {
                mask |= 1u << (i2 * 8 + j2);
                if (ok) y[((long)oy * Wo + ox) * N + n] = v;
            }
        }
    block_stats_128(out, mask, sh, tl, cl, ok, stats, N, n);
}
int launch_polyphase_output(hipStream_t s, const float* Mm, const float* bias, float* y, float* stats, int Ho, int Wo, int N,
                            int up, int Tt) {
    const TileGrid tg = tile_grid(Ho, Wo, up ? 8 : 4);
    const int TW = tg.TW, T = tg.T, Tp = tg.Tp;
    if (up)
        hipLaunchKernelGGL(polyphase_output_up_kernel, dim3(Tp / 2, (N + 63) / 64), dim3(256), 0, s, Mm, bias, y,
                           reinterpret_cast<float2*>(stats), Ho, Wo, N, TW, T, Tt);
    else
        hipLaunchKernelGGL(polyphase_output_down_kernel, dim3(Tp / 8, (N + 63) / 64), dim3(256), 0, s, Mm, bias, y,
                           reinterpret_cast<float2*>(stats), Ho, Wo, N, TW, T, Tt);
    T2V_HIP_CHECK(hipGetLastError());
    return T2V_OK;
}

}
```

text2video_amd/csrc/t2v_internal.h:

```cpp
#pragma once
#include <hip/hip_runtime.h>
#include <stddef.h>
#include <stdint.h>
#include "../../include/t2v.h"

namespace t2v {

void set_error(const char* fmt, ...);
#define T2V_HIP_CHECK(expr)                                                            \
    do {                                                                               \
        hipError_t _e = (expr);                                                        \
        if (_e != hipSuccess) {                                                        \
            ::t2v::set_error("%s:%d: %s -> %s", __FILE__, __LINE__, #expr,             \
                             hipGetErrorString(_e));                                   \
            return T2V_ERR_HIP;                                                        \
        }                                                                              \
    } while (0)
#define T2V_REQUIRE(cond, ...)                                                         \
    do {                                                                               \
        if (!(cond)) {                                                                 \
            ::t2v::set_error(__VA_ARGS__);                                             \
            return T2V_ERR_INVALID;                                                    \
        }                                                                              \
    } while (0)
// ... 11 lines not shown
    int wgrad_sk;
    int wgrad_combine;
    int wgrad_combine_max;
    int chain_lazy;
    int conv_tile;
    int streams;
    int sk_blocks_per_cu;
    int xcd_slices;
};
const Options& options();
bool overlap_hint();
int set_overlap_hint(int on);
struct OverlapScope {
    int prev;
    explicit OverlapScope(bool on) : prev(set_overlap_hint(on ? 1 : 0)) {}
    ~OverlapScope() { set_overlap_hint(prev); }
};
void options_reload();

unsigned* async_error_word();
bool fixed_grid_enabled();
void fixed_grid_disable(const char* why);
int check_async_errors();

constexpr int kMaxTaps = 52;
constexpr int kMaxPhases = 4;
constexpr int kBK = 32;

struct ConvPhase {
    int ntaps;
    int tap0;
    int nk;
    int Kp;
    long w_off;
    int oy0, ox0;
};

struct ConvKParams {
    const float* x;
    const float* w;
    const float* bias;
    float* y;
    float* stats;
    int Hin, Win, Cin_s;
    int Wm, M;
    int Cout, Cout_s, Wout, Hout;
    int stride, ostride;
    int pad_mode, act;
    float act_scale;
    int mtiles, ntiles, nphases;
    int group_mtiles;
    long group_w_stride;
    int KW, pad;
    int batch;
    long x_img_stride, y_img_stride, stats_img_stride;
    ConvPhase ph[kMaxPhases];
    int tdy[kMaxTaps];
    int tdx[kMaxTaps];
};

struct WgradParams {
    const float* x;
    const float* dy;
    float* dw;
    int batch, Hin, Win, Cin_s;
    long x_img_stride, dy_img_stride;
    int Wm, M;
    int Hout, Wout, Cout, Cout_s;
    int stride, ostride;
    int ntaps, ntiles, ctiles;
    int reflect, accumulate;
    int fold, fold_taps, KW, pad;
    int splits;
    long dw_floats;
    float* dw_final;
    int* tickets;
    int tdy[kMaxTaps], tdx[kMaxTaps];
    int toy[kMaxTaps], tox[kMaxTaps];
    long tap_woff[kMaxTaps];
    int tap_Kp[kMaxTaps];
    int tap_kidx[kMaxTaps];
};
int launch_conv_wgrad(hipStream_t s, const WgradParams& p);
bool conv_wgrad_strided_ok(const WgradParams& p);
int launch_wgrad_reduce(hipStream_t s, const float* partial, int splits, long n, float* dw, int accumulate);
int launch_unpack_conv_weight(hipStream_t s, const float* packed, float* w, int Cout, int Cin, int KH, int KW, int Cin_s,
                              int Kp, int accumulate = 0);
int launch_unpack_convT_weight(hipStream_t s, const float* packed, float* w, int Cin, int Cout, int Cin_s, int Cout_p,
                               int K, int pad, int accumulate = 0);
int launch_accumulate(hipStream_t s, float* dst, const float* src, long n, int overwrite);
int launch_scale(hipStream_t s, float* x, long n, float sc);
int launch_unzip2(hipStream_t s, const float* src, float* dst0, float* dst1, int C, int overwrite);
int launch_pad_copy(hipStream_t s, const float* x, float* xp, int batch, int H, int W, int C, int pad, int reflect);
int launch_reflect_pad_backward(hipStream_t s, const float* dxp, float* dx, int H, int W, int C, int p);
int launch_inorm_backward(hipStream_t s, const float* x, const float* dy, const float* mean_rstd, const float* gamma,
                          const float* beta, int relu, long npix, int C, float* scratch, float* dx, float* sums,
                          float* d_beta = nullptr, float* d_gamma = nullptr, int overwrite = 0);
int launch_act_backward(hipStream_t s, const float* dy, const float* y, int mode, float slope, long n, float* dpre);
int launch_avgpool3s2_backward(hipStream_t s, const float* dy, float* dx, int H, int W, int C);
int launch_maxpool2x2(hipStream_t s, const float* x, float* y, int H, int W, int C);
int launch_maxpool2x2_backward(hipStream_t s, const float* x, const float* dy, float* dx, int H, int W, int C);
int launch_loss_backward(hipStream_t s, int op, const float* a, const float* b, float c, float scale, long n, float* da);
inline int wino_pad_tiles(int T) {
    const int a = (T + 63) / 64 * 64, b = (T + 127) / 128 * 128;
    return (b - a) * 8 >= b ? a : b;
}
struct TileGrid {
    int TW, T, Tp;
};
inline TileGrid tile_grid(int Ho, int Wo, int edge) {
    const int TW = (Wo + edge - 1) / edge, T = ((Ho + edge - 1) / edge) * TW;
    return {TW, T, wino_pad_tiles(T)};
}
inline int capped_grid(long n, int block, long cap) {
    const long g = (n + block - 1) / block;
    return (int)(g > cap ? cap : g < 1 ? 1 : g);
}
struct LazyNorm {
    const float* mean_rstd = nullptr;
    const float* gamma = nullptr;
    const float* beta = nullptr;
    int relu = 0;
    const float* res = nullptr;
    float* xout = nullptr;
};
int launch_winograd_weight(hipStream_t s, const float* w, float* U, int Cout, int Cin, int Cout_p, int Cin_s, int adjoint = 0);
int launch_winograd_input(hipStream_t s, const float* x, float* V, int H, int W, int C, int pad, int reflect);
int launch_winograd_output(hipStream_t s, const float* Mm, const float* bias, float* y, float* stats, int H, int W, int N);
int launch_winograd4_weight(hipStream_t s, const float* w, float* U, int Cout, int Cin, int Cout_p, int Cin_s, int adjoint = 0);
int launch_winograd4_input(hipStream_t s, const float* x, float* V, int H, int W, int C, int pad, int reflect, int batch = 1,
                           int image = 0, int nimg = 0, long img_stride = 0, const LazyNorm* lazy = nullptr);
int launch_winograd4_dgrad_output(hipStream_t s, const float* dV, float* dxp, int H, int W, int C);
int launch_polyphase_weight(hipStream_t s, const float* w, float* U, int Cout, int Cin, int Cout_p, int Cin_s, int up);
int launch_polyphase_input(hipStream_t s, const float* x, float* V, int H, int W, int C, int up, int Tt,
                           const LazyNorm* lazy = nullptr);
int launch_polyphase_output(hipStream_t s, const float* Mm, const float* bias, float* y, float* stats, int Ho, int Wo, int N,
                            int up, int Tt);
int launch_winograd4_dy(hipStream_t s, const float* dy, float* Md, int Ho, int Wo, int N, int dy_cs, int batch, int image);
int launch_winograd4_dy_norm(hipStream_t s, const float* dy, const float* x, const float* mean_rstd, const float* gamma,
                             const float* beta, int relu, const float* sums, float* Md, int Ho, int Wo, int N, int batch,
                             int image);
int launch_winograd4_dw(hipStream_t s, const float* dU, float* dw, int Cout, int Cin, int Cout_p, int Kp, int accumulate);
int launch_winograd4_output(hipStream_t s, const float* Mm, const float* bias, float* y, float* stats, int H, int W, int N,
                            int lrelu, float slope, int nimg = 1);
int launch_channel_sum(hipStream_t s, const float* x, long npix, int C, int cs, float* scratch, float* out);

struct HeadParams {
    const float* x;
    const float* w;
    const float* bias;
    float* y;
    int H, W, Cin_s, Kp, Cout, Cout_s, act;
    float act_scale;
};
int launch_conv_head7x7(hipStream_t s, const HeadParams& p);

struct Cout1Params {
    const float* x;
    const float* w;
    const float* bias;
    float* y;
    int H, W, Cin_s, ksize, stride, pad, Hout, Wout, Cout_s, act;
    float act_scale;
};
bool conv_cout1_supported(int ksize, int Cin_s);
int launch_conv_cout1(hipStream_t s, const Cout1Params& p);

struct StemParams {
    const float* x;
    const float* w;
    const float* bias;
    float* y;
    float* stats;
    int H, W, Cin_s, Kp, Cout, Cout_s;
    int Cin;
};
bool conv_stem7x7_supported(int H, int W, int Cin_s, int Cout);
int launch_conv_stem7x7(hipStream_t s, const StemParams& p);

enum ConvTile { kTileL = 0 , kTileS = 1 , kTileQ = 2 ,
                kTileStem = 3  };
int conv_tile_for(int Cout);
void conv_tile_dims(int tile, int* BM, int* BN);
int launch_conv_igemm(hipStream_t s, const ConvKParams& p, int tile);

struct SkGemm {
    const float* a;
    const float* b;
    float* c;
    float* scratch;
    unsigned* err;
    int rows = 0;
    long a_group_stride;
    int groups, T, K, N, c_cs;
    bool b_kn = false;
};
size_t wino_gemm_sk_scratch_floats();
bool wino_gemm_sk_ok(int groups, int T, int K, int N, int c_cs, int rows = 0);
bool wino_gemm_sk_bkn_ok(int groups, int T, int K, int N, int c_cs);
int wino_gemm_sk_tall_rows(int groups, int rows, int T, int N);
int launch_wino_gemm_sk(hipStream_t s, const SkGemm& g);
bool wino_gemm_skr_ok(int groups, int rows, int Tp, int K, int N, int c_cs);
int launch_wino_gemm_skr(hipStream_t s, const SkGemm& g, int rows);
bool wino_gemm_skt_ok(int groups, int rows, int Tp, int K, int N, int c_cs);
int launch_wino_gemm_skt(hipStream_t s, const SkGemm& g, int rows);
int wino_gemm_sk_grid_blocks();
int sk_launch_blocks();
constexpr int kSkExclusiveLds = 96 * 1024;
int sk_exclusive_lds(int own_bytes);
unsigned long long wino_gemm_sk_next_tag();
bool wino_wgrad_sk_ok(int Tt, int Cin, int Cout);
int launch_wino_wgrad_sk(hipStream_t s, const float* V, const float* Md, float* dU, float* scratch, int Tt, int Cin, int Cout,
                         int Cout_p, int Kp);

constexpr int kFinalizeMaxGroups = 64;
struct RunningUpdate {
    float* mean;
    float* var;
    float n;
    float momentum;
    int times;
};
int launch_inorm_finalize_winograd(hipStream_t s, const float* stats, int wm, int H, int W, int C, float eps,
                                   float* mean_rstd, int batch, double* scratch = nullptr, const RunningUpdate* ru = nullptr);
int launch_inorm_finalize_tiles(hipStream_t s, const float* stats, int edge, int H, int W, int C, float eps,
                                float* mean_rstd, int batch, double* scratch = nullptr, const RunningUpdate* ru = nullptr);
int launch_inorm_finalize(hipStream_t s, const float* stats, int nparts, int mtiles, int BM, int M, int C,
                          float eps, float* mean_rstd, double* scratch = nullptr, const RunningUpdate* ru = nullptr);
int launch_inorm_apply(hipStream_t s, const float* x, const float* mean_rstd, const float* gamma,
                       const float* beta, const float* res1, const float* res2, float* y, long npix, int C,
                       int relu, int nimg = 1);
int launch_bn_running_update(hipStream_t s, const float* mean_rstd, float* running_mean, float* running_var, long n,
                             float momentum, float eps, int C);
int launch_pack_conv_weight(hipStream_t s, const float* w, float* packed, int Cout, int Cin, int KH, int KW,
                            int Cin_s, int Kp, int Cout_p, int adjoint = 0);
int launch_pack_convT_weight(hipStream_t s, const float* w, float* packed, int Cin, int Cout, int Cin_s, int Cout_p,
                             int K, int pad);
void convT_phase_taps_host(int phase, int k, int pad, int* ntaps, int kh[4], int kw[4], int dy[4], int dx[4], int* a,
                           int* b);
int launch_nchw_to_nhwc(hipStream_t s, const float* src, float* dst, int C, int H, int W, int Cs);
int launch_nhwc_to_nchw(hipStream_t s, const float* src, float* dst, int C, int H, int W, int Cs);
int launch_reduce(hipStream_t s, int op, const float* a, const float* b, float c, long n, float* scratch, float* out);
int launch_loss_terms(hipStream_t s, const long long* tp, const int* ti, const float* tf, const int* chunk_term,
                      const long long* chunk_off, const int* term_chunk0, int nterms, int nchunks, int chunk, float* part,
                      float* out);
int launch_adam(hipStream_t s, float* p, const float* g, float* m, float* v, long n, double lr, double b1, double b2,
                double eps, int step);
int launch_adam_multi(hipStream_t s, const long long* ptrs, const long long* nelem, const float* step_size,
                      const int* chunk_tensor, const long long* chunk_off, int nchunks, int chunk, double b1, double b2,
                      double eps);
int launch_masked_l1(hipStream_t s, const float* a, const float* b, const float* mask, long npix, int c0, int C, int cs,
                     float* scratch, float* out);
int launch_masked_l1_backward(hipStream_t s, const float* a, const float* b, const float* mask, float scale, long npix,
                              int c0, int C, int cs, float* da);
int launch_add(hipStream_t s, const float* a, const float* b, float* y, long n);
int launch_warp_composite(hipStream_t s, const float* raw, const float* fw, const float* prev, int prev_cs,
                          int prev_c0, float* out, float* warp_out, int H, int W);
int launch_warp_composite_backward(hipStream_t s, const float* d_out, const float* d_warp, const float* raw,
                                   const float* fw, const float* prev, int prev_cs, int prev_c0, float* d_raw,
                                   float* d_fw, float* d_prev, int H, int W);
int launch_avgpool3s2(hipStream_t s, const float* x, float* y, int H, int W, int C);
int launch_to_u8(hipStream_t s, const float* x, uint8_t* y, long n);
int launch_u8_pose_to_f32(hipStream_t s, const uint8_t* src, float* dst, long npix, int Cs, int c0);
int launch_copy_channels(hipStream_t s, const float* src, int src_cs, int src_c0, float* dst, int dst_cs,
                         int dst_c0, int nc, long npix);

}

struct t2v_ctx {
    int device;
    hipStream_t side;
    hipEvent_t ev_fork, ev_join;
};
```

text2video_amd/ops.py:

```python
import ctypes

from ._xp import torch

from . import _lib
from ._lib import (ACT_FLOW_W, ACT_LRELU, ACT_NONE, ACT_TANH, ALGO_DIRECT, ALGO_WINOGRAD,
                   ALGO_POLYPHASE, ALGO_WINOGRAD_F4, PAD_REFLECT, PAD_ZERO, ConvDesc, check)

_contexts = {}


def context(device=None):
    if not torch.cuda.is_available():
        raise RuntimeError("text2video_amd: no HIP device visible; the frame-synthesis path has no CPU fallback")
    dev = torch.cuda.current_device() if device is None else torch.device(device).index or 0
    c = _contexts.get(dev)
    if c is None:
        with torch.cuda.device(dev):
            c = _lib.Context(dev)
        _contexts[dev] = c
    return c


def reload_env():
    _lib.load().t2v_reload_env()
# ... 21 lines not shown

def _chk(t, name):
    if not (t.is_cuda and t.dtype == torch.float32 and t.is_contiguous()):
        raise ValueError("%s must be a contiguous fp32 device tensor" % name)


def round_up(v, m):
    return (v + m - 1) // m * m


def conv_desc(H, W, Cin, Cout, k, stride=1, pad=0, pad_mode=PAD_ZERO, transposed=False, act=ACT_NONE,
              act_scale=1.0, output_padding=None, algo=0):
    if output_padding is None:
        output_padding = 1 if transposed else 0
    return ConvDesc(H, W, Cin, Cout, k, k, stride, pad, pad_mode, int(transposed), act, act_scale, output_padding,
                    algo)


def winograd_supported(desc, x_cs=None, algo=None):
    x_cs = round_up(desc.Cin, 4) if x_cs is None else x_cs
    algo = (desc.algo or ALGO_WINOGRAD) if algo is None else algo
    mask = _lib.load().t2v_conv_winograd_supported(ctypes.byref(desc), x_cs)
    return bool(mask & (2 if algo == ALGO_WINOGRAD_F4 else 1))


def polyphase_supported(desc, x_cs=None):
    x_cs = round_up(desc.Cin, 4) if x_cs is None else x_cs
    return bool(_lib.load().t2v_conv_polyphase_supported(ctypes.byref(desc), x_cs) & 1)


def polyphase_pays(desc, x_cs=None):
    x_cs = round_up(desc.Cin, 4) if x_cs is None else x_cs
    return bool(_lib.load().t2v_conv_polyphase_supported(ctypes.byref(desc), x_cs) & 2)


def best_conv_algo(desc, x_cs=None, cap=0):
    x_cs = round_up(desc.Cin, 4) if x_cs is None else x_cs
    return _lib.load().t2v_conv_best_algo(ctypes.byref(desc), x_cs, cap)


def conv2d_auto(x, packed_w, bias, desc, y_cs=None, stats=None, out=None):
    if desc.algo in (ALGO_WINOGRAD, ALGO_WINOGRAD_F4, ALGO_POLYPHASE):
        assert y_cs is None or y_cs == desc.Cout
        return conv2d_winograd(x, packed_w, bias, desc, stats=stats, out=out)
    return conv2d(x, packed_w, bias, desc, y_cs=y_cs, stats=stats, out=out)


def with_algo(desc, algo):
    return ConvDesc(desc.H, desc.W, desc.Cin, desc.Cout, desc.kH, desc.kW, desc.stride, desc.pad, desc.pad_mode,
                    desc.transposed, desc.act, desc.act_scale, desc.output_padding, algo)


GEMM_FORMS = {0: "conv_igemm_kernel<64x64 tiles, one block per tile>", 1: "conv_igemm_kernel<128x128 tiles, one block per tile>",
              2: "wino_gemm_sk_kernel<128x128 tiles on a fixed grid of 2 blocks per CU>",
              3: "wino_gemm_sk_kernel<192x64 tiles on a fixed grid of 2 blocks per CU>",
              4: "wino_gemm_sk_kernel<160x128 tiles on a fixed grid of 1 block per CU>",
              5: "wino_gemm_skr_kernel<ragged 128/96/64/32 x 128 tiles on a fixed grid of 2 blocks per CU>",
              6: "wino_gemm_sk_kernel<256x128 tiles on a fixed grid of 1 block per CU>",
              7: "wino_gemm_skt_kernel<ragged 96..192 x 128 tiles on a fixed grid of 1 block per CU>"}


def winograd_gemm_form(desc, nimg=1):
    return GEMM_FORMS.get(_lib.load().t2v_conv_winograd_gemm_form(ctypes.byref(desc), nimg), "?")


def winograd_tile_rows(desc):
    return _lib.load().t2v_conv_winograd_tile_rows(ctypes.byref(desc))


def winograd_workspace(desc, x_cs, device):
    n = _lib.load().t2v_conv_winograd_workspace_floats(ctypes.byref(desc), x_cs)
    if n == 0:
        raise RuntimeError("winograd_workspace: shape not supported")
    return torch.empty(n, dtype=torch.float32, device=device)


def conv2d_winograd(x, packed_u, bias, desc, stats=None, out=None, workspace=None, stages=7, keep_v=None):
    c = context()
    _chk(x, "x")
    x_cs = x.shape[-1]
    ws = workspace if workspace is not None else winograd_workspace(desc, x_cs, x.device)
    ho, wo = conv_out_dims(desc)
    y = out if out is not None else torch.empty(ho, wo, desc.Cout, dtype=torch.float32, device=x.device)
    if keep_v is not None:
        assert stages == 7
        wg, batch, slot = keep_v
        check(c.lib.t2v_conv2d_forward_winograd_keep_v(c.handle, _stream(), ctypes.byref(desc), _p(x), x_cs, _p(packed_u), _p(bias),
                                                       _p(y), desc.Cout, _p(stats), _p(ws), _p(wg), batch, slot),
              "conv2d_forward_winograd_keep_v")
        return y
    check(c.lib.t2v_conv2d_forward_winograd_stages(c.handle, _stream(), ctypes.byref(desc), _p(x), x_cs, _p(packed_u),
                                                   _p(bias), _p(y), desc.Cout, _p(stats), _p(ws), stages),
          "conv2d_forward_winograd")
    return y


def winograd_batch_workspace(desc, x_cs, nimg, device):
    n = _lib.load().t2v_conv_winograd_batch_workspace_floats(ctypes.byref(desc), x_cs, nimg)
    if n == 0:
        raise RuntimeError("winograd_batch_workspace: shape not supported")
    return torch.empty(n, dtype=torch.float32, device=device)


def conv2d_winograd_batch(x, packed_u, bias, desc, workspace, stats=None, out=None, stages=7, mean_rstd=None, gamma=None,
                          beta=None, relu=0, res=None, xout=None):
    c = context()
    if x.dim() == 3:
        x = x.unsqueeze(0)
    _chk(x, "x")
    nimg, x_cs = x.shape[0], x.shape[-1]
    ho, wo = conv_out_dims(desc)
    y = out if out is not None else torch.empty(nimg, ho, wo, desc.Cout, dtype=torch.float32, device=x.device)
    check(c.lib.t2v_conv2d_forward_winograd_batch_stages(c.handle, _stream(), ctypes.byref(desc), nimg, _p(x), x_cs,
                                                         x[0].numel(), _p(packed_u), _p(bias), _p(y), desc.Cout, _p(stats),
                                                         _p(workspace), stages, _p(mean_rstd), _p(gamma), _p(beta), int(relu),
                                                         _p(res), _p(xout)),
          "conv2d_forward_winograd_batch_stages")
    return y


def conv_out_dims(desc):
    h, w = ctypes.c_int(), ctypes.c_int()
    check(_lib.load().t2v_conv_out_dims(ctypes.byref(desc), ctypes.byref(h), ctypes.byref(w)), "conv_out_dims")
    return h.value, w.value


def pack_conv_weight(weight, desc, x_cs=None, adjoint=False):
    c = context()
    _chk(weight, "weight")
    x_cs = round_up(desc.Cin, 4) if x_cs is None else x_cs
    n = c.lib.t2v_conv_packed_weight_floats(ctypes.byref(desc), x_cs)
    if n == 0:
        raise RuntimeError("pack_conv_weight: %s" % c.lib.t2v_last_error().decode())
    packed = torch.empty(n, dtype=torch.float32, device=weight.device)
    fn = c.lib.t2v_conv_pack_weight_adjoint if adjoint else c.lib.t2v_conv_pack_weight
    check(fn(c.handle, _stream(), ctypes.byref(desc), x_cs, _p(weight), _p(packed)), "conv_pack_weight")
    return packed


def conv_stats_buffer(desc, device):
    n = _lib.load().t2v_conv_stats_floats(ctypes.byref(desc))
    return torch.empty(max(n, 1), dtype=torch.float32, device=device)


def conv2d(x, packed_w, bias, desc, y_cs=None, stats=None, out=None):
    c = context()
    _chk(x, "x")
    x_cs = x.shape[-1]
    ho, wo = conv_out_dims(desc)
    y_cs = round_up(desc.Cout, 4) if y_cs is None else y_cs
    y = out if out is not None else torch.empty(ho, wo, y_cs, dtype=torch.float32, device=x.device)
    check(c.lib.t2v_conv2d_forward(c.handle, _stream(), ctypes.byref(desc), _p(x), x_cs, _p(packed_w), _p(bias),
                                   _p(y), y_cs, _p(stats)), "conv2d_forward")
    return y


def conv2d_batch(x, packed_w, bias, desc, y_cs=None, stats=None, out=None):
    c = context()
    _chk(x, "x")
    B, x_cs = x.shape[0], x.shape[-1]
    ho, wo = conv_out_dims(desc)
    y_cs = round_up(desc.Cout, 4) if y_cs is None else y_cs
    y = out if out is not None else torch.empty(B, ho, wo, y_cs, dtype=torch.float32, device=x.device)
    if out is not None:
        _chk(out, "out")
    check(c.lib.t2v_conv2d_forward_batch(c.handle, _stream(), ctypes.byref(desc), B, _p(x), x_cs, _p(packed_w), _p(bias),
                                         _p(y), y_cs, _p(stats)), "conv2d_forward_batch")
    return y


def conv2d_auto_batch(x, packed_w, bias, desc, y_cs=None, stats=None, out=None):
    B = x.shape[0]
    if out is None:
        ho, wo = conv_out_dims(desc)
        out = torch.empty(B, ho, wo, round_up(desc.Cout, 4) if y_cs is None else y_cs, dtype=torch.float32, device=x.device)
    if desc.algo == ALGO_DIRECT and B > 1 and x.is_contiguous() and out.is_contiguous() and \
            (stats is None or stats.is_contiguous()):
        return conv2d_batch(x, packed_w, bias, desc, y_cs=y_cs, stats=stats, out=out)
    n = stats.numel() // B if stats is not None else 0
    for i in range(B):
        conv2d_auto(x[i], packed_w, bias, desc, y_cs=y_cs, stats=stats[i * n:(i + 1) * n] if stats is not None else None, out=out[i])
    return out


def instance_norm_finalize(stats, desc, eps=1e-5, out=None, running=None):
    c = context()
    mr = out if out is not None else torch.empty(desc.Cout, 2, dtype=torch.float32, device=stats.device)
    if running is not None:
        rm, rv, momentum, times = running
        check(c.lib.t2v_batch_norm_finalize_running(c.handle, _stream(), ctypes.byref(desc), 1, _p(stats), eps, _p(mr), _p(rm), _p(rv),
                                                    momentum, int(times)), "batch_norm_finalize_running")
        return mr
    check(c.lib.t2v_instance_norm_finalize(c.handle, _stream(), ctypes.byref(desc), _p(stats), eps, _p(mr)),
          "instance_norm_finalize")
    return mr


def instance_norm_apply(x, mean_rstd, gamma=None, beta=None, res1=None, res2=None, relu=False, out=None):
    c = context()
    _chk(x, "x")
    C = x.shape[-1]
    npix = x.numel() // C
    y = out if out is not None else torch.empty_like(x)
    check(c.lib.t2v_instance_norm_apply(c.handle, _stream(), _p(x), _p(mean_rstd), _p(gamma), _p(beta), _p(res1),
                                        _p(res2), _p(y), npix, C, int(relu)), "instance_norm_apply")
    return y


def conv_norm_act(x, packed_w, bias, desc, gamma=None, beta=None, relu=True, res1=None, res2=None, eps=1e-5):
    stats = conv_stats_buffer(desc, x.device)
    y = conv2d(x, packed_w, bias, desc, y_cs=desc.Cout, stats=stats)
    mr = instance_norm_finalize(stats, desc, eps)
    return instance_norm_apply(y, mr, gamma, beta, res1, res2, relu, out=y)


def flow_warp_composite(raw, fw, prev, prev_c0, want_warp=False, out=None):
    c = context()
    H, W = raw.shape[0], raw.shape[1]
    out = torch.empty_like(raw) if out is None else out
    warp = torch.empty_like(raw) if want_warp else None
    check(c.lib.t2v_flow_warp_composite(c.handle, _stream(), _p(raw), _p(fw), _p(prev), prev.shape[-1], prev_c0,
                                        _p(out), _p(warp), H, W), "flow_warp_composite")
    return (out, warp) if want_warp else out


def flow_warp(fw, img, c0=0, out=None):
    c = context()
    H, W = fw.shape[0], fw.shape[1]
    out = torch.empty(H, W, 4, dtype=torch.float32, device=fw.device) if out is None else out
    check(c.lib.t2v_flow_warp_composite(c.handle, _stream(), None, _p(fw), _p(img), img.shape[-1], c0, None, _p(out),
                                        H, W), "flow_warp")
    return out


def flow_warp_composite_backward(d_out, d_warp, raw, fw, prev, prev_c0, want_d_prev=False):
    c = context()
    H, W = fw.shape[0], fw.shape[1]
    d_raw = torch.empty_like(fw) if d_out is not None else None
    d_fw = torch.empty_like(fw)
    d_prev = torch.zeros_like(prev) if want_d_prev else None
    check(c.lib.t2v_flow_warp_composite_backward(c.handle, _stream(), _p(d_out), _p(d_warp), _p(raw), _p(fw), _p(prev),
                                                 prev.shape[-1], prev_c0, _p(d_raw), _p(d_fw), _p(d_prev), H, W),
          "flow_warp_composite_backward")
    return d_raw, d_fw, d_prev


def avgpool3x3s2(x):
    c = context()
    _chk(x, "x")
    H, W, C = x.shape
    y = torch.empty((H + 2 - 3) // 2 + 1, (W + 2 - 3) // 2 + 1, C, dtype=torch.float32, device=x.device)
    check(c.lib.t2v_avgpool3x3s2(c.handle, _stream(), _p(x), _p(y), H, W, C), "avgpool3x3s2")
    return y


def nchw_to_nhwc(x, cs=None, out=None):
    c = context()
    _chk(x, "x")
    C, H, W = x.shape
    cs = round_up(C, 4) if cs is None else cs
    y = out if out is not None else torch.empty(H, W, cs, dtype=torch.float32, device=x.device)
    check(c.lib.t2v_nchw_to_nhwc(c.handle, _stream(), _p(x), _p(y), C, H, W, cs), "nchw_to_nhwc")
    return y


def nhwc_to_nchw(x, C=None):
    c = context()
    _chk(x, "x")
    H, W, cs = x.shape
    C = cs if C is None else C
    y = torch.empty(C, H, W, dtype=torch.float32, device=x.device)
    check(c.lib.t2v_nhwc_to_nchw(c.handle, _stream(), _p(x), _p(y), C, H, W, cs), "nhwc_to_nchw")
    return y


def pose_u8_to_f32(src_u8, dst, c0):
    c = context()
    H, W, _ = src_u8.shape
    check(c.lib.t2v_pose_u8_to_f32(c.handle, _stream(), _p(src_u8), _p(dst), H * W, dst.shape[-1], c0),
          "pose_u8_to_f32")
    return dst


def tensor2im_u8(x):
    c = context()
    _chk(x, "x")
    y = torch.empty(x.shape, dtype=torch.uint8, device=x.device)
    check(c.lib.t2v_tensor2im_u8(c.handle, _stream(), _p(x), _p(y), x.numel()), "tensor2im_u8")
    return y


def copy_channels(src, src_c0, dst, dst_c0, nc):
    c = context()
    npix = src.numel() // src.shape[-1]
    check(c.lib.t2v_copy_channels(c.handle, _stream(), _p(src), src.shape[-1], src_c0, _p(dst), dst.shape[-1],
                                  dst_c0, nc, npix), "copy_channels")
    return dst


def batch_norm_finalize(stats, desc, batch, eps=1e-5, running=None):
    c = context()
    mr = torch.empty(desc.Cout, 2, dtype=torch.float32, device=stats.device)
    if running is not None:
        rm, rv, momentum, times = running
        check(c.lib.t2v_batch_norm_finalize_running(c.handle, _stream(), ctypes.byref(desc), batch, _p(stats), eps, _p(mr), _p(rm),
                                                    _p(rv), momentum, int(times)), "batch_norm_finalize_running")
# ... 368 lines not shown
```

Baseline: 96.52 frames/s.

## Fuse pending norm into 7x7 head, share Winograd V across branches, join-norm bottleneck

Lets the 7x7 output head apply the decoder's last pending instance norm + ReLU on its LDS input plane, so the separate norm-apply pass over the full-resolution feature map is skipped. When the image and flow residual chains start from the same input, one F(4x4,3x3) Winograd input transform is computed once and reused by both branches. The two encoder outputs are normalized and summed in a single join kernel, and the polyphase input transform spreads its four sub-blocks across more threads. This adds coupling between layers and more parameters in the generator scheduler, and it risks more register and LDS pressure in the head kernel.

Result: faster. 98.11 frames/s, median of 6 (+1.6%).

```diff
diff --git a/include/t2v.h b/include/t2v.h
--- a/include/t2v.h
+++ b/include/t2v.h
@@ -8,7 +8,7 @@
 extern "C" {
 #endif
 
-#define T2V_ABI_VERSION 18
+#define T2V_ABI_VERSION 19
 
 typedef enum {
     T2V_OK = 0,
@@ -62,6 +62,9 @@
                        float* stats_partial);
 int t2v_conv2d_forward_batch(t2v_ctx* ctx, void* stream, const t2v_conv_desc* d, int batch, const float* x, int x_cs,
                              const float* w_packed, const float* bias, float* y, int y_cs, float* stats_partial);
+int t2v_conv2d_forward_head_norm(t2v_ctx* ctx, void* stream, const t2v_conv_desc* d, const float* x, int x_cs,
+                                 const float* w_packed, const float* bias, float* y, int y_cs, const float* mean_rstd,
+                                 const float* gamma, const float* beta, int relu);
 
 int t2v_conv_winograd_supported(const t2v_conv_desc* d, int x_cs);
 int t2v_conv_polyphase_supported(const t2v_conv_desc* d, int x_cs);
diff --git a/text2video_amd/_lib.py b/text2video_amd/_lib.py
--- a/text2video_amd/_lib.py
+++ b/text2video_amd/_lib.py
@@ -8,7 +8,7 @@
 T2V_OK = 0
 PAD_ZERO, PAD_REFLECT = 0, 1
 ACT_NONE, ACT_TANH, ACT_FLOW_W, ACT_LRELU = 0, 1, 2, 3
-ABI_VERSION = 18
+ABI_VERSION = 19
 MAX_BATCH = 8
 ALGO_DIRECT, ALGO_WINOGRAD, ALGO_WINOGRAD_F4, ALGO_POLYPHASE = 0, 1, 2, 3
 
@@ -55,6 +55,8 @@
                                    c_void_p, c_int, c_void_p]),
     "t2v_conv2d_forward_batch": (c_int, [c_void_p, c_void_p, POINTER(ConvDesc), c_int, c_void_p, c_int, c_void_p, c_void_p,
                                          c_void_p, c_int, c_void_p]),
+    "t2v_conv2d_forward_head_norm": (c_int, [c_void_p, c_void_p, POINTER(ConvDesc), c_void_p, c_int, c_void_p, c_void_p,
+                                             c_void_p, c_int, c_void_p, c_void_p, c_void_p, c_int]),
     "t2v_conv_winograd_supported": (c_int, [POINTER(ConvDesc), c_int]),
     "t2v_conv_polyphase_supported": (c_int, [POINTER(ConvDesc), c_int]),
     "t2v_conv_best_algo": (c_int, [POINTER(ConvDesc), c_int, c_int]),
diff --git a/text2video_amd/csrc/capi.hip b/text2video_amd/csrc/capi.hip
--- a/text2video_amd/csrc/capi.hip
+++ b/text2video_amd/csrc/capi.hip
@@ -346,6 +346,27 @@
     return launch_wino_gemm_sk(s, k);
 }
 
+bool conv_plan_is_head7x7(const ConvPlan& pl) {
+    const ConvKParams& q = pl.kp;
+    return q.nphases == 1 && q.ph[0].ntaps == 49 && q.KW == 7 && q.pad == 3 && q.stride == 1 && q.pad_mode == T2V_PAD_REFLECT &&
+           q.Cout <= 3 && q.Cin_s % 16 == 0 && q.Hin >= 4 && q.Win >= 4;
+}
+int run_head7x7(hipStream_t s, const ConvPlan& pl, const float* x, const float* w, const float* bias, float* y, int y_cs,
+                const LazyNorm* lazy) {
+    const ConvKParams& q = pl.kp;
+    T2V_REQUIRE(conv_plan_is_head7x7(pl), "head7x7: not a 7x7 reflect-padded conv with <= 3 output channels");
+    T2V_REQUIRE(!lazy || (lazy->mean_rstd && (lazy->gamma == nullptr) == (lazy->beta == nullptr) && !lazy->res && !lazy->xout),
+                "head7x7: a pending norm is (mean, rstd), gamma and beta or neither, no residual");
+    HeadParams h;
+    h.x = x; h.w = w; h.bias = bias; h.y = y;
+    h.H = q.Hin; h.W = q.Win; h.Cin_s = q.Cin_s; h.Kp = q.ph[0].Kp; h.Cout = q.Cout; h.Cout_s = y_cs;
+    h.act = q.act; h.act_scale = q.act_scale;
+    if (lazy) {
+        h.mean_rstd = lazy->mean_rstd; h.gamma = lazy->gamma; h.beta = lazy->beta; h.relu = lazy->relu;
+    }
+    return launch_conv_head7x7(s, h);
+}
+
 int run_conv_batch(t2v_ctx* ctx, hipStream_t s, const ConvPlan& pl, int batch, const float* x, long x_stride, const float* w,
                    const float* bias, float* y, int y_cs, long y_stride, float* stats, long stats_stride) {
     T2V_REQUIRE(ctx && x && w && y, "conv: null pointer");
@@ -353,19 +374,9 @@
     T2V_REQUIRE(y_cs >= pl.kp.Cout && y_cs <= pl.Cout_p, "conv: output channel storage %d out of range [%d,%d]", y_cs,
                 pl.kp.Cout, pl.Cout_p);
     T2V_REQUIRE((long)pl.Hout * pl.Wout * y_cs * 4 < 0x7fff0000L, "conv: output tensor too large for 32-bit buffer offsets");
-    {
-        const ConvKParams& q = pl.kp;
-        if (!stats && q.nphases == 1 && q.ph[0].ntaps == 49 && q.KW == 7 && q.pad == 3 && q.stride == 1 &&
-            q.pad_mode == T2V_PAD_REFLECT && q.Cout <= 3 && q.Cin_s % 16 == 0 && q.Hin >= 4 && q.Win >= 4) {
-            for (int b = 0; b < batch; ++b) {
-                HeadParams h;
-                h.x = x + b * x_stride; h.w = w; h.bias = bias; h.y = y + b * y_stride;
-                h.H = q.Hin; h.W = q.Win; h.Cin_s = q.Cin_s; h.Kp = q.ph[0].Kp; h.Cout = q.Cout; h.Cout_s = y_cs;
-                h.act = q.act; h.act_scale = q.act_scale;
-                T2V_TRY(launch_conv_head7x7(s, h));
-            }
-            return T2V_OK;
-        }
+    if (!stats && conv_plan_is_head7x7(pl)) {
+        for (int b = 0; b < batch; ++b) T2V_TRY(run_head7x7(s, pl, x + b * x_stride, w, bias, y + b * y_stride, y_cs, nullptr));
+        return T2V_OK;
     }
     {
         const ConvKParams& q = pl.kp;
@@ -425,6 +436,7 @@
     const bool keep = wb.keep_v != nullptr;
     T2V_REQUIRE(!keep || (f4 && nimg == 1 && wb.keep_slot >= 0 && wb.keep_slot < wb.keep_total),
                 "winograd: V is kept for the weight gradient of single F(4x4,3x3) images only");
+    T2V_REQUIRE(!wb.v_in || (f4 && !keep && !(stages & 1)), "winograd: a borrowed V replaces the input transform (F(4x4,3x3))");
     float* V = keep ? wb.keep_v + (size_t)wb.keep_slot * T * d->Cin : workspace;
     float* Mm = workspace + wino_pos(d->algo) * T * d->Cin;
     if (stages & 1) {
@@ -441,7 +453,7 @@
         g.rows = nimg * wino_tiles_real(d, d->algo);
         g.T = (int)T; g.K = d->Cin; g.N = d->Cout;
         if (keep) g.a_pitch = wb.keep_total * (int)T;
-        T2V_TRY(run_position_gemm(ctx, s, g, V, w_packed, Mm, f4 ? workspace + winograd_vm_floats(d, nimg) : nullptr));
+        T2V_TRY(run_position_gemm(ctx, s, g, wb.v_in ? wb.v_in : V, w_packed, Mm, f4 ? workspace + winograd_vm_floats(d, nimg) : nullptr));
     }
     if (stages & 4) {
         T2V_REQUIRE(d->act == T2V_ACT_NONE || !stats_partial, "winograd: an activation and norm statistics do not combine");
@@ -722,6 +734,21 @@
     ConvPlan pl;
     T2V_TRY(build_conv_plan(d, x_cs, stats_partial != nullptr, &pl));
     return run_conv(ctx, (hipStream_t)stream, pl, x, w_packed, bias, y, y_cs, stats_partial);
+}
+
+int t2v_conv2d_forward_head_norm(t2v_ctx* ctx, void* stream, const t2v_conv_desc* d, const float* x, int x_cs,
+                                 const float* w_packed, const float* bias, float* y, int y_cs, const float* mean_rstd,
+                                 const float* gamma, const float* beta, int relu) {
+    T2V_REQUIRE(ctx && d && x && w_packed && y && mean_rstd, "conv2d_forward_head_norm: null pointer");
+    T2V_REQUIRE(d->algo == T2V_ALGO_DIRECT, "conv2d_forward_head_norm: direct convolutions only");
+    T2V_REQUIRE(relu == 1, "conv2d_forward_head_norm: the pending norm is norm + ReLU (relu must be 1)");
+    ConvPlan pl;
+    T2V_TRY(build_conv_plan(d, x_cs, false, &pl));
+    T2V_REQUIRE(y_cs >= pl.kp.Cout && y_cs <= pl.Cout_p, "conv2d_forward_head_norm: output channel storage %d out of range [%d,%d]",
+                y_cs, pl.kp.Cout, pl.Cout_p);
+    T2V_REQUIRE((long)pl.kp.Hin * pl.kp.Win * x_cs * 4 < 0x7fff0000L, "conv2d_forward_head_norm: input too large for 32-bit buffer offsets");
+    const LazyNorm ln{mean_rstd, gamma, beta, relu};
+    return run_head7x7((hipStream_t)stream, pl, x, w_packed, bias, y, y_cs, &ln);
 }
 
 int t2v_conv2d_forward_batch(t2v_ctx* ctx, void* stream, const t2v_conv_desc* d, int batch, const float* x, int x_cs,
diff --git a/text2video_amd/csrc/conv_head.hip b/text2video_amd/csrc/conv_head.hip
--- a/text2video_amd/csrc/conv_head.hip
+++ b/text2video_amd/csrc/conv_head.hip
@@ -1,6 +1,7 @@
 #include <stdlib.h>
 
 #include "t2v_internal.h"
+#include "transform_common.h"
 
 namespace t2v {
 
@@ -68,6 +69,32 @@
         asm volatile("s_waitcnt vmcnt(0)" ::: "memory");
         typedef float f32x4 __attribute__((ext_vector_type(4)));
         typedef const __attribute__((address_space(4))) f32x4* cf4;
+        if (p.mean_rstd != nullptr) {
+            const f32x4 mr0 = *(cf4)(p.mean_rstd + 2 * c0), mr1 = *(cf4)(p.mean_rstd + 2 * c0 + 4);
+            f32x4 gm = {1.f, 1.f, 1.f, 1.f}, bt = {0.f, 0.f, 0.f, 0.f};
+            auto norm_plane = [&](bool aff) {
+#pragma unroll
+                for (int i = 0; i < 8; ++i) {
+                    float4* q = reinterpret_cast<float4*>(plane + (i * 64 + lane) * 16);
+                    float4 v = *q;
+                    v.x = norm_apply(v.x, mr0.x, mr0.y, aff, gm.x, bt.x, 1);
+                    v.y = norm_apply(v.y, mr0.z, mr0.w, aff, gm.y, bt.y, 1);
+                    v.z = norm_apply(v.z, mr1.x, mr1.y, aff, gm.z, bt.z, 1);
+                    v.w = norm_apply(v.w, mr1.z, mr1.w, aff, gm.w, bt.w, 1);
+                    *q = v;
+                }
+            };
+            if (p.gamma != nullptr) {
+                gm = *(cf4)(p.gamma + c0);
+                bt = *(cf4)(p.beta + c0);
+                norm_plane(true);
+            } else {
+                norm_plane(false);
+            }
+            __builtin_amdgcn_fence(__ATOMIC_RELEASE, "wavefront");
+            __builtin_amdgcn_wave_barrier();
+            __builtin_amdgcn_fence(__ATOMIC_ACQUIRE, "wavefront");
+        }
         f32x4 wa[3][3], wb[2][3], wc[2][3];
         float4 xv[2][10];
         const float* __restrict__ b0 = w0 + c0;
@@ -179,6 +206,7 @@
 }
 
 int launch_conv_head7x7(hipStream_t s, const HeadParams& p) {
+    T2V_REQUIRE(!p.mean_rstd || p.relu == 1, "conv_head7x7: a pending norm is norm + ReLU (what the decoder's last layer carries)");
     constexpr int lds = 4 * kHsPlane;
     const dim3 grid(((p.W + kHdTile - 1) / kHdTile) * ((p.H + kHdTile - 1) / kHdTile));
     if (p.Cin_s == 128) hipLaunchKernelGGL(conv_head7x7_strip_kernel<128>, grid, dim3(256), lds, s, p);
diff --git a/text2video_amd/csrc/conv_plan.h b/text2video_amd/csrc/conv_plan.h
--- a/text2video_amd/csrc/conv_plan.h
+++ b/text2video_amd/csrc/conv_plan.h
@@ -56,12 +56,16 @@
     long img_stride_x = 0;
     float* keep_v = nullptr;
     int keep_total = 1, keep_slot = 0;
+    const float* v_in = nullptr;
 };
 int winograd_forward(t2v_ctx* ctx, hipStream_t s, const t2v_conv_desc* d, const float* x, const float* w_packed,
                      const float* bias, float* y, float* stats_partial, float* workspace, int stages,
                      const WinoBatch* batch = nullptr);
 int run_conv(t2v_ctx* ctx, hipStream_t s, const ConvPlan& pl, const float* x, const float* w, const float* bias,
              float* y, int y_cs, float* stats);
+bool conv_plan_is_head7x7(const ConvPlan& pl);
+int run_head7x7(hipStream_t s, const ConvPlan& pl, const float* x, const float* w, const float* bias, float* y, int y_cs,
+                const LazyNorm* lazy);
 int run_conv_batch(t2v_ctx* ctx, hipStream_t s, const ConvPlan& pl, int batch, const float* x, long x_stride, const float* w,
                    const float* bias, float* y, int y_cs, long y_stride, float* stats, long stats_stride);
 
diff --git a/text2video_amd/csrc/elementwise.hip b/text2video_amd/csrc/elementwise.hip
--- a/text2video_amd/csrc/elementwise.hip
+++ b/text2video_amd/csrc/elementwise.hip
@@ -163,13 +163,33 @@
     return T2V_OK;
 }
 
+__device__ __forceinline__ float4 join_side(const NormJoinSide& s, long im, long n4, int C4, long i, int c4) {
+    const float4* mr = reinterpret_cast<const float4*>(s.mean_rstd) + im * 2 * C4;
+    const float4 a = mr[2 * c4], b = mr[2 * c4 + 1];
+    float4 v = reinterpret_cast<const float4*>(s.y)[im * n4 + i];
+    v.x = norm_scale(v.x, a.x, a.y);
+    v.y = norm_scale(v.y, a.z, a.w);
+    v.z = norm_scale(v.z, b.x, b.y);
+    v.w = norm_scale(v.w, b.z, b.w);
+    if (s.gamma) {
+        const float4 gm = reinterpret_cast<const float4*>(s.gamma)[c4], bt = reinterpret_cast<const float4*>(s.beta)[c4];
+        v.x = norm_affine(v.x, gm.x, bt.x);
+        v.y = norm_affine(v.y, gm.y, bt.y);
+        v.z = norm_affine(v.z, gm.z, bt.z);
+        v.w = norm_affine(v.w, gm.w, bt.w);
+    }
+    const float4 r = reinterpret_cast<const float4*>(s.res)[im * n4 + i];
+    v.x += r.x; v.y += r.y; v.z += r.z; v.w += r.w;
+    return v;
+}
+
 __global__ __launch_bounds__(256) void inorm_apply_kernel(const float4* __restrict__ x,
                                                           const float4* __restrict__ mean_rstd,
                                                           const float4* __restrict__ gamma,
                                                           const float4* __restrict__ beta,
                                                           const float4* __restrict__ res1,
                                                           const float4* __restrict__ res2, float4* __restrict__ y,
-                                                          long n4, int C4, int relu) {
+                                                          long n4, int C4, int relu, const NormJoinSide join) {
     {
         const long im = blockIdx.y;
         x += im * n4;
@@ -213,6 +233,10 @@
             const float4 r = res2[i];
             v.x += r.x; v.y += r.y; v.z += r.z; v.w += r.w;
         }
+        if (join.y) {
+            const float4 r = join_side(join, blockIdx.y, n4, C4, i, c4);
+            v.x += r.x; v.y += r.y; v.z += r.z; v.w += r.w;
+        }
         y[i] = v;
     }
 }
@@ -226,7 +250,21 @@
                        reinterpret_cast<const float4*>(x), reinterpret_cast<const float4*>(mean_rstd),
                        reinterpret_cast<const float4*>(gamma), reinterpret_cast<const float4*>(beta),
                        reinterpret_cast<const float4*>(res1), reinterpret_cast<const float4*>(res2),
-                       reinterpret_cast<float4*>(y), n4, C / 4, relu);
+                       reinterpret_cast<float4*>(y), n4, C / 4, relu, NormJoinSide{});
+    T2V_HIP_CHECK(hipGetLastError());
+    return T2V_OK;
+}
+int launch_inorm_join(hipStream_t s, const NormJoinSide& a, const NormJoinSide& b, float* y, long npix, int C, int nimg) {
+    T2V_REQUIRE(C % 4 == 0, "inorm_join: C=%d must be a multiple of 4", C);
+    T2V_REQUIRE(a.y && a.mean_rstd && a.res && b.y && b.mean_rstd && b.res && y, "inorm_join: null pointer");
+    T2V_REQUIRE((a.gamma == nullptr) == (a.beta == nullptr) && (b.gamma == nullptr) == (b.beta == nullptr),
+                "inorm_join: gamma and beta must both be given or both NULL");
+    const long n4 = npix * (C / 4);
+    hipLaunchKernelGGL(inorm_apply_kernel, dim3(grid_for(n4, 256), nimg), dim3(256), 0, s,
+                       reinterpret_cast<const float4*>(a.y), reinterpret_cast<const float4*>(a.mean_rstd),
+                       reinterpret_cast<const float4*>(a.gamma), reinterpret_cast<const float4*>(a.beta),
+                       reinterpret_cast<const float4*>(a.res), (const float4*)nullptr, reinterpret_cast<float4*>(y), n4, C / 4,
+                       0, b);
     T2V_HIP_CHECK(hipGetLastError());
     return T2V_OK;
 }
diff --git a/text2video_amd/csrc/generator.hip b/text2video_amd/csrc/generator.hip
--- a/text2video_amd/csrc/generator.hip
+++ b/text2video_amd/csrc/generator.hip
@@ -96,6 +96,7 @@
     float* bt[4];
     float* bt2[4];
     float* d;
+    float* vshare;
     float *dimg, *dflow;
     float *decI[8], *decF[8];
     float *raw, *fw;
@@ -121,6 +122,15 @@
     for (int i = 0; i < 4; ++i) b.bt[i] = a.alloc(N * lvl(n));
     for (int i = 0; i < 4; ++i) b.bt2[i] = a.alloc(N * lvl(n));
     b.d = a.alloc(N * lvl(n));
+    {
+        const bool flow_global = !g.no_flow && !g.is_local && g.n_blocks / 2 > 0;
+        b.vshare = nullptr;
+        if (flow_global) {
+            const LayerSpec& L = layers[2 * (1 + n + 2 * (g.n_blocks - g.n_blocks / 2))];
+            if (L.cd.algo == T2V_ALGO_WINOGRAD_F4)
+                b.vshare = a.alloc((size_t)wino_pos(L.cd.algo) * wino_rows_batch(&L.cd, L.cd.algo, nimg) * L.cd.Cin);
+        }
+    }
     b.dimg = a.alloc(N * lvl(n));
     b.dflow = a.alloc(N * lvl(n));
     for (int l = 0; l < n; ++l) {
@@ -218,6 +228,7 @@
             const int wm = wino_m(L.cd.algo);
             WinoBatch wb;
             T2V_TRY(winograd_forward(ctx, s, &L.cd, x, w.w, w.bias, y, stats, b.wino[sc], 7, &wb));
+            T2V_REQUIRE(!lazy_in && !lazy_out, "internal: a Winograd layer outside a chain takes and leaves applied norms");
             T2V_TRY(launch_inorm_finalize_winograd(s, stats, wm, L.cd.H, L.cd.W, Cout, g.eps, mr, 1, fin_of(im)));
             return launch_inorm_apply(s, y, mr, gam, bet, res1, res2, y, (long)M, Cout, relu);
         }
@@ -246,15 +257,43 @@
         ++li;
         return T2V_OK;
     }
-    bool next_takes_raw() const { return options().chain_lazy && specs[li + 1].cd.algo == T2V_ALGO_POLYPHASE; }
-
-    int head(const Ptrs& x, const MutPtrs& y) {
+    bool next_takes_raw() const {
+        if (!options().chain_lazy) return false;
+        const LayerSpec& nx = specs[li + 1];
+        if (nx.cd.algo == T2V_ALGO_POLYPHASE) return true;
+        ConvPlan pl;
+        return !nx.has_norm && build_conv_plan(&nx.cd, nx.x_cs, false, &pl) == T2V_OK && conv_plan_is_head7x7(pl);
+    }
+
+    int head(const Ptrs& x, const MutPtrs& y, bool x_raw) {
         const LayerSpec& L = specs[li];
         const t2v_layer& w = layers[li];
+        const t2v_layer& prev = layers[li - 1];
         ++li;
         ConvPlan pl;
         T2V_TRY(build_conv_plan(&L.cd, L.x_cs, false, &pl));
-        for (int im = 0; im < nimg; ++im) T2V_TRY(run_conv(ctx, s, pl, x.p[im], w.w, w.bias, y.p[im], 4, nullptr));
+        for (int im = 0; im < nimg; ++im) {
+            if (x_raw) {
+                const LazyNorm ln{mr_of(im), g.norm_affine ? prev.gamma : nullptr, g.norm_affine ? prev.beta : nullptr, 1};
+                T2V_TRY(run_head7x7(s, pl, x.p[im], w.w, w.bias, y.p[im], 4, &ln));
+            } else {
+                T2V_TRY(run_conv(ctx, s, pl, x.p[im], w.w, w.bias, y.p[im], 4, nullptr));
+            }
+        }
+        return T2V_OK;
+    }
+    int export_feat(const float* feat, size_t stride, float* const* dst, bool raw) {
+        const LayerSpec& L = specs[li - 2];
+        const t2v_layer& w = layers[li - 2];
+        const size_t floats = (size_t)g.H * g.W * L.cd.Cout;
+        for (int im = 0; im < nimg; ++im) {
+            if (!dst[im]) continue;
+            if (raw)
+                T2V_TRY(launch_inorm_apply(s, feat + im * stride, mr_of(im), g.norm_affine ? w.gamma : nullptr,
+                                           g.norm_affine ? w.beta : nullptr, nullptr, nullptr, dst[im], (long)g.H * g.W, L.cd.Cout, 1));
+            else
+                T2V_HIP_CHECK(hipMemcpyAsync(dst[im], feat + im * stride, floats * sizeof(float), hipMemcpyDeviceToDevice, s));
+        }
         return T2V_OK;
     }
 
@@ -269,7 +308,7 @@
         const float* res;
         float* xout;
     };
-    int wino4_conv_stats(const float* x, const LazyIn* lz, float* y_raw) {
+    int wino4_conv_stats(const float* x, const LazyIn* lz, float* y_raw, const float* v_in = nullptr) {
         const LayerSpec& L = specs[li];
         const t2v_layer& w = layers[li];
         ++li;
@@ -285,7 +324,8 @@
         WinoBatch wb;
         wb.nimg = nimg;
         wb.img_stride_x = (long)b.bott;
-        T2V_TRY(winograd_forward(ctx, s, &cd, x, w.w, w.bias, y_raw, b.stats[sc], b.wino[sc], lz ? 6 : 7, &wb));
+        wb.v_in = lz ? nullptr : v_in;
+        T2V_TRY(winograd_forward(ctx, s, &cd, x, w.w, w.bias, y_raw, b.stats[sc], b.wino[sc], (lz || v_in) ? 6 : 7, &wb));
         const size_t per_img = (size_t)(wino_tiles_padded(&cd, cd.algo) / 8) * cd.Cout * 2;
         for (int im = 0; im < nimg; ++im)
             T2V_TRY(launch_inorm_finalize_winograd(s, b.stats[sc] + im * per_img, 4, cd.H, cd.W, cd.Cout, g.eps, mr_of(im), 1,
@@ -293,12 +333,17 @@
         return T2V_OK;
     }
 
-    int res_chain_lazy(const float* x, int count, float* tmp[4], const float** out) {
+    struct PendingNorm {
+        const float* y;
+        const float* res;
+        const t2v_layer* norm;
+    };
+    int res_chain_lazy(const float* x, int count, float* tmp[4], const float** out, PendingNorm* pend_out, const float* v0) {
         const float* cur = x;
         const t2v_layer* pend = nullptr;
         for (int i = 0; i < count; ++i) {
             if (i == 0) {
-                T2V_TRY(wino4_conv_stats(x, nullptr, tmp[0]));
+                T2V_TRY(wino4_conv_stats(x, nullptr, tmp[0], v0));
             } else {
                 float* xi = tmp[2 + (i & 1)];
                 const LazyIn in{pend, 0, cur, xi};
@@ -309,17 +354,30 @@
             T2V_TRY(wino4_conv_stats(tmp[0], &mid, tmp[1]));
             pend = &layers[li - 1];
         }
+        *out = tmp[1];
+        if (pend_out) {
+            *pend_out = {tmp[1], cur, pend};
+            return T2V_OK;
+        }
         const LayerSpec& L = specs[li - 1];
         T2V_TRY(launch_inorm_apply(s, tmp[1], b.mean_rstd[sc], g.norm_affine ? pend->gamma : nullptr,
                                    g.norm_affine ? pend->beta : nullptr, cur, nullptr, tmp[1], (long)L.cd.H * L.cd.W,
                                    L.cd.Cout, 0, nimg));
-        *out = tmp[1];
-        return T2V_OK;
-    }
-
-    int res_chain(const float* x, int count, float* tmp[4], const float** out) {
-        if (options().chain_lazy && count > 0 && specs[li].cd.algo == T2V_ALGO_WINOGRAD_F4 && b.mr_stride == (size_t)2 * specs[li].cd.Cout)
-            return res_chain_lazy(x, count, tmp, out);
+        return T2V_OK;
+    }
+
+    bool chain_is_lazy(int l, int count) const {
+        return options().chain_lazy && count > 0 && specs[l].cd.algo == T2V_ALGO_WINOGRAD_F4 && b.mr_stride == (size_t)2 * specs[l].cd.Cout;
+    }
+    int share_v(int l, const float* x) {
+        const t2v_conv_desc& cd = specs[l].cd;
+        return launch_winograd4_input(s, x, b.vshare, cd.H, cd.W, cd.Cin, cd.pad, cd.pad_mode == T2V_PAD_REFLECT, nimg, 0, nimg,
+                                      (long)b.bott);
+    }
+    int res_chain(const float* x, int count, float* tmp[4], const float** out, PendingNorm* pend_out = nullptr,
+                  const float* v0 = nullptr) {
+        if (chain_is_lazy(li, count)) return res_chain_lazy(x, count, tmp, out, pend_out, v0);
+        T2V_REQUIRE(!pend_out && !v0, "internal: only the lazy chain leaves its last norm pending / borrows a V");
         const float* cur = x;
         for (int i = 0; i < count; ++i) {
             float* t = tmp[0];
@@ -331,7 +389,7 @@
         return T2V_OK;
     }
 
-    int encoder(const Ptrs& x, float** act, int nb, float* tmp[4], const float** out) {
+    int encoder(const Ptrs& x, float** act, int nb, float* tmp[4], const float** out, PendingNorm* pend_out) {
         const int n = g.is_local ? 1 : g.n_downsample;
         bool raw = n > 0 && next_takes_raw();
         T2V_TRY(conv_norm(x, at(act[0], b.lvl[0]), 1, Ptrs{}, false, raw));
@@ -341,13 +399,14 @@
             raw = raw_out;
         }
         if (nb == 0) {
+            T2V_REQUIRE(!pend_out, "internal: an encoder without blocks ends in an applied norm");
             *out = act[n];
             return T2V_OK;
         }
-        return res_chain(act[n], nb, tmp, out);
-    }
-
-    int decoder(const float* x, float** dec, const float** out) {
+        return res_chain(act[n], nb, tmp, out, pend_out);
+    }
+
+    int decoder(const float* x, float** dec, const float** out, bool* out_raw) {
         const int n = g.is_local ? 1 : g.n_downsample;
         const float* cur = x;
         size_t cur_stride = b.bott;
@@ -355,13 +414,14 @@
         for (int i = 0; i < n; ++i) {
             const int l = n - 1 - i;
             float* y = dec[l];
-            const bool raw_out = i + 1 < n && next_takes_raw();
+            const bool raw_out = next_takes_raw();
             T2V_TRY(conv_norm(at(cur, cur_stride), at(y, b.lvl[l]), 1, Ptrs{}, raw, raw_out));
             raw = raw_out;
             cur = y;
             cur_stride = b.lvl[l];
         }
         *out = cur;
+        *out_raw = raw;
         return T2V_OK;
     }
 };
@@ -455,7 +515,7 @@
     const int branch_layers = 2 * nb_res + n + 1;
     Runner r{ctx, s, *d, specs, layers, b, batch};
     Runner r2{ctx, s2, *d, specs, layers, b, batch};
-    r2.sc = two_streams ? 1 : 0;
+    r2.sc = 1;
 
     Ptrs pose{}, prevp{};
     for (int im = 0; im < batch; ++im) {
@@ -467,10 +527,19 @@
     const float *segout, *imgout;
     T2V_TRY(fork());
     r2.li = enc_layers;
-    T2V_TRY(r2.encoder(prevp, b.encB, nb_enc, tmpB, &imgout));
-    T2V_TRY(r.encoder(pose, b.encA, nb_enc, tmpA, &segout));
+    const bool fused_join = r.chain_is_lazy(1 + n, nb_enc);
+    Runner::PendingNorm pendA{}, pendB{};
+    T2V_TRY(r2.encoder(prevp, b.encB, nb_enc, tmpB, &imgout, fused_join ? &pendB : nullptr));
+    T2V_TRY(r.encoder(pose, b.encA, nb_enc, tmpA, &segout, fused_join ? &pendA : nullptr));
     T2V_TRY(join());
-    T2V_TRY(launch_add(s, imgout, segout, b.d, (long)(batch * bott)));
+    if (fused_join) {
+        const bool aff = d->norm_affine != 0;
+        const NormJoinSide sb{pendB.y, b.mean_rstd[r2.sc], aff ? pendB.norm->gamma : nullptr, aff ? pendB.norm->beta : nullptr, pendB.res};
+        const NormJoinSide sa{pendA.y, b.mean_rstd[r.sc], aff ? pendA.norm->gamma : nullptr, aff ? pendA.norm->beta : nullptr, pendA.res};
+        T2V_TRY(launch_inorm_join(s, sb, sa, b.d, (long)(d->H >> n) * (d->W >> n), G << n, batch));
+    } else {
+        T2V_TRY(launch_add(s, imgout, segout, b.d, (long)(batch * bott)));
+    }
     const float* dsum = b.d;
     r.li = 2 * enc_layers;
 
@@ -493,26 +562,31 @@
         raw.p[im] = ios[im].raw ? ios[im].raw : (blend[im] ? b.raw + im * px4 : ios[im].out);
         fw.p[im] = ios[im].flow_w ? ios[im].flow_w : b.fw + im * px4;
     }
+    float *want_img_feat[kMaxBatch], *want_flow_feat[kMaxBatch];
+    for (int im = 0; im < batch; ++im) {
+        want_img_feat[im] = ios[im].img_feat;
+        want_flow_feat[im] = ios[im].flow_feat;
+    }
+    const float* v0 = nullptr;
+    if (b.vshare && img_in == flow_in && r.chain_is_lazy(2 * enc_layers, nb_res)) {
+        T2V_TRY(r.share_v(2 * enc_layers, dsum));
+        v0 = b.vshare;
+    }
+    bool feat_raw = false;
     if (!d->no_flow) {
         T2V_TRY(fork());
         r2.li = 2 * enc_layers + branch_layers;
         const float *res_flow, *flow_feat;
-        T2V_TRY(r2.res_chain(flow_in, nb_res, tmpB, &res_flow));
-        T2V_TRY(r2.decoder(res_flow, b.decF, &flow_feat));
-        T2V_TRY(r2.head(r2.at(flow_feat, feat), fw));
-        for (int im = 0; im < batch; ++im)
-            if (ios[im].flow_feat)
-                T2V_HIP_CHECK(hipMemcpyAsync(ios[im].flow_feat, flow_feat + im * feat, feat * sizeof(float),
-                                             hipMemcpyDeviceToDevice, s2));
+        T2V_TRY(r2.res_chain(flow_in, nb_res, tmpB, &res_flow, nullptr, v0));
+        T2V_TRY(r2.decoder(res_flow, b.decF, &flow_feat, &feat_raw));
+        T2V_TRY(r2.head(r2.at(flow_feat, feat), fw, feat_raw));
+        T2V_TRY(r2.export_feat(flow_feat, feat, want_flow_feat, feat_raw));
     }
     const float *res_img, *img_feat;
-    T2V_TRY(r.res_chain(img_in, nb_res, tmpA, &res_img));
-    T2V_TRY(r.decoder(res_img, b.decI, &img_feat));
-    T2V_TRY(r.head(r.at(img_feat, feat), raw));
-    for (int im = 0; im < batch; ++im)
-        if (ios[im].img_feat)
-            T2V_HIP_CHECK(hipMemcpyAsync(ios[im].img_feat, img_feat + im * feat, feat * sizeof(float), hipMemcpyDeviceToDevice,
-                                         s));
+    T2V_TRY(r.res_chain(img_in, nb_res, tmpA, &res_img, nullptr, v0));
+    T2V_TRY(r.decoder(res_img, b.decI, &img_feat, &feat_raw));
+    T2V_TRY(r.head(r.at(img_feat, feat), raw, feat_raw));
+    T2V_TRY(r.export_feat(img_feat, feat, want_img_feat, feat_raw));
     if (!d->no_flow) {
         T2V_TRY(join());
         r.li += branch_layers;
diff --git a/text2video_amd/csrc/polyphase.hip b/text2video_amd/csrc/polyphase.hip
--- a/text2video_amd/csrc/polyphase.hip
+++ b/text2video_amd/csrc/polyphase.hip
@@ -57,14 +57,19 @@
                                                              const float2* __restrict__ mean_rstd,
                                                              const float2* __restrict__ gamma,
                                                              const float2* __restrict__ beta, int relu) {
-    const long total = (long)Tt * C2;
+    constexpr int NSUB = UP ? 1 : 4;
+    const long total = (long)Tt * NSUB * C2;
     const long stride = (long)gridDim.x * blockDim.x;
     for (long i = (long)blockIdx.x * blockDim.x + threadIdx.x; i < total; i += stride) {
-        const long tile = i / C2;
-        const int c2 = (int)(i - tile * C2);
+        const long ts = i / C2;
+        const int c2 = (int)(i - ts * C2);
+        const long tile = ts / NSUB;
+        const int sub = (int)(ts - tile * NSUB);
+        auto mine = [&](int s) { return UP || sub == s; };
         if (tile >= T) {
 #pragma unroll 1
-            for (int pos = 0; pos < 81; ++pos) V[((long)pos * Tt + tile) * C2 + c2] = make_float2(0.f, 0.f);
+            for (int pos = 0; pos < 81; ++pos)
+                if (mine((pos / 9 >= 5 ? 2 : 0) + (pos % 9 >= 5 ? 1 : 0))) V[((long)pos * Tt + tile) * C2 + c2] = make_float2(0.f, 0.f);
             continue;
         }
         const int ty = (int)(tile / TW), tx = (int)(tile - (long)ty * TW);
@@ -89,7 +94,7 @@
             return v;
         };
         auto store = [&](int pr, int pc, float vx, float vy) { V[((long)(pr * 9 + pc) * Tt + tile) * C2 + c2] = make_float2(vx, vy); };
-        {
+        if (mine(0)) {
             float rx[5][5], ry[5][5];
 #pragma unroll
             for (int a = 0; a < 5; ++a) {
@@ -118,6 +123,7 @@
                 for (int p = 0; p < 5; ++p) store(p, q, cdot<5>(pp::kBU[p], cx), cdot<5>(pp::kBU[p], cy));
             }
         }
+        if (mine(1))
 #pragma unroll
         for (int b = 0; b < 4; ++b) {
             float cx[5], cy[5];
@@ -130,6 +136,7 @@
 #pragma unroll
             for (int p = 0; p < 5; ++p) store(p, 5 + b, cdot<5>(pp::kBU[p], cx), cdot<5>(pp::kBU[p], cy));
         }
+        if (mine(2))
 #pragma unroll
         for (int a = 0; a < 4; ++a) {
             float dx[5], dy[5];
@@ -142,6 +149,7 @@
 #pragma unroll
             for (int q = 0; q < 5; ++q) store(5 + a, q, cdot<5>(pp::kBU[q], dx), cdot<5>(pp::kBU[q], dy));
         }
+        if (mine(3))
 #pragma unroll
         for (int a = 0; a < 4; ++a)
 #pragma unroll
@@ -157,7 +165,7 @@
     T2V_REQUIRE((ln.gamma == nullptr) == (ln.beta == nullptr) && (ln.relu == 0 || ln.relu == 1) && !ln.res && !ln.xout,
                 "polyphase_input: bad norm arguments");
     const TileGrid tg = up ? tile_grid(H, W, 4) : tile_grid(H / 2, W / 2, 4);
-    const int grid = pp_grid((long)Tt * (C / 2), 256);
+    const int grid = pp_grid((long)Tt * (up ? 1 : 4) * (C / 2), 256);
     auto kern = up ? (ln.mean_rstd ? polyphase_input_kernel<true, true> : polyphase_input_kernel<true, false>)
                    : (ln.mean_rstd ? polyphase_input_kernel<false, true> : polyphase_input_kernel<false, false>);
     hipLaunchKernelGGL(kern, dim3(grid), dim3(256), 0, s, reinterpret_cast<const float2*>(x), reinterpret_cast<float2*>(V), H, W,
diff --git a/text2video_amd/csrc/t2v_internal.h b/text2video_amd/csrc/t2v_internal.h
--- a/text2video_amd/csrc/t2v_internal.h
+++ b/text2video_amd/csrc/t2v_internal.h
@@ -187,6 +187,10 @@
     float* y;
     int H, W, Cin_s, Kp, Cout, Cout_s, act;
     float act_scale;
+    const float* mean_rstd = nullptr;
+    const float* gamma = nullptr;
+    const float* beta = nullptr;
+    int relu = 0;
 };
 int launch_conv_head7x7(hipStream_t s, const HeadParams& p);
 
@@ -265,6 +269,14 @@
 int launch_inorm_apply(hipStream_t s, const float* x, const float* mean_rstd, const float* gamma,
                        const float* beta, const float* res1, const float* res2, float* y, long npix, int C,
                        int relu, int nimg = 1);
+struct NormJoinSide {
+    const float* y = nullptr;
+    const float* mean_rstd = nullptr;
+    const float* gamma = nullptr;
+    const float* beta = nullptr;
+    const float* res = nullptr;
+};
+int launch_inorm_join(hipStream_t s, const NormJoinSide& a, const NormJoinSide& b, float* y, long npix, int C, int nimg);
 int launch_bn_running_update(hipStream_t s, const float* mean_rstd, float* running_mean, float* running_var, long n,
                              float momentum, float eps, int C);
 int launch_pack_conv_weight(hipStream_t s, const float* w, float* packed, int Cout, int Cin, int KH, int KW,
diff --git a/text2video_amd/ops.py b/text2video_amd/ops.py
--- a/text2video_amd/ops.py
+++ b/text2video_amd/ops.py
@@ -197,6 +197,20 @@
     y = out if out is not None else torch.empty(ho, wo, y_cs, dtype=torch.float32, device=x.device)
     check(c.lib.t2v_conv2d_forward(c.handle, _stream(), ctypes.byref(desc), _p(x), x_cs, _p(packed_w), _p(bias),
                                    _p(y), y_cs, _p(stats)), "conv2d_forward")
+    return y
+
+
+def conv2d_head_norm(x, packed_w, bias, desc, mean_rstd, gamma=None, beta=None, relu=True, y_cs=None, out=None):
+    c = context()
+    _chk(x, "x")
+    _chk(mean_rstd, "mean_rstd")
+    x_cs = x.shape[-1]
+    ho, wo = conv_out_dims(desc)
+    y_cs = round_up(desc.Cout, 4) if y_cs is None else y_cs
+    y = out if out is not None else torch.empty(ho, wo, y_cs, dtype=torch.float32, device=x.device)
+    check(c.lib.t2v_conv2d_forward_head_norm(c.handle, _stream(), ctypes.byref(desc), _p(x), x_cs, _p(packed_w), _p(bias),
+                                             _p(y), y_cs, _p(mean_rstd), _p(gamma), _p(beta), int(relu)),
+          "conv2d_forward_head_norm")
     return y
 
 
```
